# Dfam-consortium/RepeatAfterMe

Measured on AMD Instinct MI355X. Metric: flank_bp_aligned_per_sec (extension columns/s x flanks), higher is better.
Workload: dtype int32

## Files before the change

include/ramx.h:

```cpp
#ifndef RAMX_H
#define RAMX_H

#include <stdint.h>
#include <stdio.h>

#ifdef __cplusplus
extern "C" {
#endif

#ifndef RAMX_USE_REFERENCE_STRUCTS
enum CoreBoundFlag { L_BOUNDARY = 0, SEQ_BOUNDARY = 1, CORE_BOUNDARY = 2, EXT_BOUNDARY = 3 };

struct coreAlignment
{
  struct coreAlignment *next;
  int seqIdx;
  uint64_t leftSeqPos;
  uint64_t rightSeqPos;
  char leftExtendable;
  char rightExtendable;
  uint64_t lowerSeqBound;
  uint64_t upperSeqBound;
  enum CoreBoundFlag lowerSeqBoundFlag;
  enum CoreBoundFlag upperSeqBoundFlag;
  int leftExtensionLen;
  int rightExtensionLen;
  int score;
  char orient;
};

struct sequenceLibrary
{
  char *sequence;
  char **identifiers;
  uint64_t *boundaries;
  uint64_t *offsets;
  uint64_t length;
  int count;
  int markov_chain_order;
  uint32_t **markov_chain_prob_tables;
};

struct scoringSystem
{
  char *name;
  int **matrix;
  int msize;
  char *alphabet;
  double m_lambda;
  double m_bg_freqs[4];
  int gapopen;
  int gapextn;
};
#endif

#define RAMX_SYM_N 99


void ramx_set_runtime(int verbose, int when_to_stop, int l);

int ramx_extend_alignment(int direction, struct coreAlignment *coreAlign, int ****score,
                          struct sequenceLibrary *seqLib, char *master, int BANDWIDTH,
                          int CAPPENALTY, int MINIMPROVEMENT, int L, int N,
                          struct scoringSystem *scoreParams, FILE *pathStringFile);

typedef struct ramx_flat_cores
{
  int32_t n;
  const int64_t *left_pos, *right_pos, *lower, *upper;
  const int8_t *orient, *left_ext, *right_ext;
  int32_t *left_len, *right_len, *score;
} ramx_flat_cores;

typedef struct ramx_params
{
  int32_t bandwidth, cappenalty, minimprovement, L, when_to_stop, l, gapopen, gapextn;
  const int32_t *matrix;
} ramx_params;

typedef struct ramx_run_info
{
  int32_t ret;
  int32_t rows_executed;
  int32_t limit_warning;
  int32_t overflow32;
  int32_t n_extendable;
  int32_t launches;
  double  loop_ms;
  double  kernel_ms_avg;
  int32_t kernel_samples;
  double  prep_ms;
  int32_t persistent;
  int32_t lanes_per_flank;
  int32_t respeculated_rows;
  int32_t packed_rows;
  int32_t lean_rows;
} ramx_run_info;

int ramx_extend_flat(int direction, ramx_flat_cores *cores, const int8_t *sequence, uint64_t seq_len,
                     int8_t *master, const ramx_params *p, ramx_run_info *info);

void ramx_invalidate_library(void);
int ramx_preload_library(const int8_t *sequence, uint64_t seq_len);
struct ramx_packed_library;
int ramx_preload_library_packed(const struct sequenceLibrary *seqLib, const struct ramx_packed_library *pl);

typedef struct ramx_dev ramx_dev;

#define RAMX_OK            0
#define RAMX_ERR_NO_DEVICE (-101)
#define RAMX_ERR_HIP       (-102)
#define RAMX_ERR_ARG       (-103)
#define RAMX_ERR_STATE     (-104)
#define RAMX_ERR_COMM      (-105)
#define RAMX_ERR_UNSUPPORTED (-106)

const char *ramx_last_error(void);
int ramx_device_count(void);
int ramx_dev_create(int device_ordinal, ramx_dev **out);
void ramx_dev_destroy(ramx_dev *d);

int ramx_dev_load_library(ramx_dev *d, const int8_t *sequence, uint64_t length);
struct ramx_packed_library;
int ramx_dev_load_library_packed(ramx_dev *d, const struct ramx_packed_library *pl);

typedef struct ramx_flank
{
  int64_t start;
  int32_t t_lo, t_hi;
  int8_t  step;
  int8_t  compl_;
  int8_t  pad_[6];
} ramx_flank;

int ramx_resolve_flanks(int direction, const ramx_flat_cores *cores, int bandwidth, int L,
                        ramx_flank *flanks, int32_t *core_index);

int ramx_dev_begin_direction(ramx_dev *d, const ramx_flank *flanks, int32_t n_flanks, const ramx_params *p);

int ramx_dev_run_direction(ramx_dev *d, ramx_run_info *info);

int ramx_dev_download(ramx_dev *d, int8_t *cons, int32_t cons_cap, int32_t *trim_high, int32_t *trim_pos);

int ramx_dev_peek_state(ramx_dev *d, int32_t flank, int32_t *cells, int32_t *high, int32_t *pos);

int ramx_dev_peek_family_state(ramx_dev *d, int32_t flank, int32_t *cells);

typedef void (*ramx_row_trace_cb)(int32_t row, int32_t besta, const int8_t *codes ,
                                  const int32_t *best_score, const int32_t *best_idx, void *user);
int ramx_dev_set_row_trace(ramx_dev *d, ramx_row_trace_cb cb, void *user);

int ramx_dev_run_families(ramx_dev *d, const ramx_flank *flanks, int32_t n_padded, const int32_t *fam_first,
                          const int32_t *fam_count, int32_t n_families, const ramx_params *p,
                          ramx_run_info *infos, int8_t *cons, int32_t *trim_high, int32_t *trim_pos);

typedef struct ramx_family
{
  ramx_flat_cores cores;
  const int8_t *sequence;
  uint64_t seq_len;
  int8_t *master;
} ramx_family;
int ramx_extend_batch(int direction, ramx_family *families, int32_t n_families, const ramx_params *p, ramx_run_info *infos);

int ramx_comm_unique_id(uint8_t id[128]);
int ramx_dev_comm_init(ramx_dev *d, const uint8_t id[128], int rank, int nranks);
int ramx_dev_comm_size(ramx_dev *d);
int ramx_dev_peer_export(ramx_dev *d, uint8_t handle[64]);
int ramx_dev_peer_import(ramx_dev *d, const uint8_t *handles , int rank, int nranks);
int ramx_dev_peer_selftest(ramx_dev *d, int phase, unsigned long long token);
int ramx_dev_peer_enable(ramx_dev *d, int on);

int ramx_dev_hostbox_attach(ramx_dev *d, const char *shm_name, int rank, int nranks);
int ramx_hostbox_unlink(const char *shm_name);

typedef void (*ramx_allreduce_cb)(long long *vals4, void *user);
int ramx_dev_set_allreduce_cb(ramx_dev *d, ramx_allreduce_cb cb, void *user);

struct scoringSystem *ramx_get_matrix(const char *matrixName);
struct scoringSystem *ramx_get_matrix_using_gap_penalties(const char *matrixName,
                                                          int gapopen, int gapextn);
struct scoringSystem *ramx_get_repeatscout_matrix(int match, int mismatch, int gap);
void ramx_free_scoring_system(struct scoringSystem *s);
double ramx_calculate_lambda(struct scoringSystem *s);

struct sequenceLibrary *ramx_load_sequence_subset_minimal(const char *twoBitName, const char *rangeBEDName,
                                                          struct coreAlignment **core_align,
                                                          int *num_cores, int max_flanking_bp);
void ramx_free_library(struct sequenceLibrary *lib, struct coreAlignment *cores);

typedef struct ramx_packed_library
{
  uint64_t length;
  int32_t n_windows;
  const uint64_t *win_start;
  const uint64_t *win_byte;
  const uint8_t *win_phase;
  const uint8_t *bytes;
  uint64_t n_bytes;
  const uint64_t *n_start;
  const uint32_t *n_len;
  int32_t n_blocks;
} ramx_packed_library;

struct sequenceLibrary *ramx_load_sequence_subset_packed(const char *twoBitName, const char *rangeBEDName,
                                                         struct coreAlignment **core_align, int *num_cores,
                                                         int max_flanking_bp, const ramx_packed_library **packed);
int ramx_packed_decode(const ramx_packed_library *pl, uint64_t from, uint64_t count, char *out);

void ramx_overlap_avoidance(struct coreAlignment *coreAlign, struct sequenceLibrary *seqLib);

void ramx_print_core_edges(struct coreAlignment *coreAlign, struct sequenceLibrary *seqLib,
                           char omitBlanks, char debug);

int ****ramx_allocate_score(int num_align, int bandwidth);
void ramx_free_score(int num_align, int bandwidth, int ****score);

int ramx_cli_main(int argc, char **argv);

#ifdef __cplusplus
}
#endif
#endif
```

repeatafterme_amd/_lib.py:

```python
from __future__ import annotations

import ctypes as C
import os
import subprocess

_PKG = os.path.dirname(os.path.abspath(__file__))
LIB_PATH = os.environ.get("RAMX_LIB") or os.path.join(_PKG, "libramx.so")
CLI_PATH = os.path.join(_PKG, "RAMExtend")

EXPORTS = [
    "ramx_set_runtime", "ramx_extend_alignment", "ramx_extend_flat", "ramx_invalidate_library", "ramx_preload_library", "ramx_resolve_flanks", "ramx_last_error", "ramx_device_count",
    "ramx_dev_create", "ramx_dev_destroy", "ramx_dev_load_library", "ramx_dev_begin_direction",
    "ramx_dev_run_direction", "ramx_dev_download", "ramx_dev_peek_state", "ramx_dev_peek_family_state", "ramx_dev_set_row_trace", "ramx_dev_run_families", "ramx_extend_batch", "ramx_comm_unique_id",
    "ramx_dev_comm_init", "ramx_dev_comm_size", "ramx_dev_set_allreduce_cb", "ramx_dev_peer_export", "ramx_dev_peer_import",
    "ramx_dev_peer_selftest", "ramx_dev_peer_enable", "ramx_dev_hostbox_attach", "ramx_hostbox_unlink", "ramx_get_matrix", "ramx_get_matrix_using_gap_penalties",
    "ramx_get_repeatscout_matrix", "ramx_free_scoring_system", "ramx_calculate_lambda",
    "ramx_load_sequence_subset_minimal", "ramx_load_sequence_subset_packed", "ramx_packed_decode", "ramx_dev_load_library_packed", "ramx_preload_library_packed", "ramx_free_library", "ramx_overlap_avoidance",
    "ramx_print_core_edges", "ramx_allocate_score", "ramx_free_score", "ramx_cli_main",
]


class RamxError(RuntimeError):
    pass


class FlatCores(C.Structure):
    _fields_ = [("n", C.c_int32)] + [(k, C.c_void_p) for k in
                ("left_pos", "right_pos", "lower", "upper", "orient", "left_ext", "right_ext",
                 "left_len", "right_len", "score")]


class Params(C.Structure):
    _fields_ = [(k, C.c_int32) for k in ("bandwidth", "cappenalty", "minimprovement", "L", "when_to_stop",
                                          "l", "gapopen", "gapextn")] + [("matrix", C.c_void_p)]


class RunInfo(C.Structure):
    _fields_ = [("ret", C.c_int32), ("rows_executed", C.c_int32), ("limit_warning", C.c_int32),
                ("overflow32", C.c_int32), ("n_extendable", C.c_int32), ("launches", C.c_int32),
                ("loop_ms", C.c_double), ("kernel_ms_avg", C.c_double), ("kernel_samples", C.c_int32),
                ("prep_ms", C.c_double), ("persistent", C.c_int32), ("lanes_per_flank", C.c_int32),
                ("respeculated_rows", C.c_int32), ("packed_rows", C.c_int32), ("lean_rows", C.c_int32)]


class Family(C.Structure):
    _fields_ = [("cores", FlatCores), ("sequence", C.c_void_p), ("seq_len", C.c_uint64), ("master", C.c_void_p)]


class Flank(C.Structure):
    _fields_ = [("start", C.c_int64), ("t_lo", C.c_int32), ("t_hi", C.c_int32), ("step", C.c_int8),
                ("compl_", C.c_int8), ("pad_", C.c_int8 * 6)]


ALLREDUCE_CB = C.CFUNCTYPE(None, C.POINTER(C.c_longlong), C.c_void_p)


def build(force: bool = False) -> None:
    if force or not os.path.exists(LIB_PATH) or not os.path.exists(CLI_PATH):
        subprocess.check_call(["make", "-s", "-C", os.path.join(_PKG, "csrc"), "all"])


_lib = None


def lib() -> C.CDLL:
    global _lib
    if _lib is None:
        if not os.path.exists(LIB_PATH):
            raise RamxError(f"{LIB_PATH} is missing: build it with `make -C repeatafterme_amd/csrc` "
                            "(there is no CPU fallback)")
        L = C.CDLL(LIB_PATH)
        L.ramx_last_error.restype = C.c_char_p
        L.ramx_set_runtime.argtypes = [C.c_int, C.c_int, C.c_int]
        L.ramx_set_runtime.restype = None
        L.ramx_extend_flat.argtypes = [C.c_int, C.POINTER(FlatCores), C.c_void_p, C.c_uint64, C.c_void_p,
                                       C.POINTER(Params), C.POINTER(RunInfo)]
        L.ramx_extend_flat.restype = C.c_int
        L.ramx_resolve_flanks.argtypes = [C.c_int, C.POINTER(FlatCores), C.c_int, C.c_int, C.c_void_p, C.c_void_p]
        L.ramx_resolve_flanks.restype = C.c_int
        L.ramx_extend_batch.argtypes = [C.c_int, C.POINTER(Family), C.c_int32, C.POINTER(Params), C.POINTER(RunInfo)]
        L.ramx_extend_batch.restype = C.c_int
        L.ramx_device_count.restype = C.c_int
        L.ramx_dev_create.argtypes = [C.c_int, C.POINTER(C.c_void_p)]
        L.ramx_dev_destroy.argtypes = [C.c_void_p]
        L.ramx_dev_destroy.restype = None
        L.ramx_dev_load_library.argtypes = [C.c_void_p, C.c_void_p, C.c_uint64]
        L.ramx_dev_begin_direction.argtypes = [C.c_void_p, C.c_void_p, C.c_int32, C.POINTER(Params)]
        L.ramx_dev_run_direction.argtypes = [C.c_void_p, C.POINTER(RunInfo)]
        L.ramx_dev_download.argtypes = [C.c_void_p, C.c_void_p, C.c_int32, C.c_void_p, C.c_void_p]
        L.ramx_dev_peek_state.argtypes = [C.c_void_p, C.c_int32, C.c_void_p, C.POINTER(C.c_int32),
                                          C.POINTER(C.c_int32)]
        L.ramx_dev_peek_family_state.argtypes = [C.c_void_p, C.c_int32, C.c_void_p]
        L.ramx_comm_unique_id.argtypes = [C.c_void_p]
        L.ramx_dev_comm_init.argtypes = [C.c_void_p, C.c_void_p, C.c_int, C.c_int]
        L.ramx_dev_comm_size.argtypes = [C.c_void_p]
        L.ramx_dev_set_allreduce_cb.argtypes = [C.c_void_p, ALLREDUCE_CB, C.c_void_p]
        L.ramx_dev_peer_export.argtypes = [C.c_void_p, C.c_void_p]
        L.ramx_dev_peer_import.argtypes = [C.c_void_p, C.c_void_p, C.c_int, C.c_int]
        L.ramx_dev_peer_selftest.argtypes = [C.c_void_p, C.c_int, C.c_uint64]
        L.ramx_dev_peer_enable.argtypes = [C.c_void_p, C.c_int]
        L.ramx_dev_hostbox_attach.argtypes = [C.c_void_p, C.c_char_p, C.c_int, C.c_int]
        L.ramx_hostbox_unlink.argtypes = [C.c_char_p]
        if hasattr(L, "ramx_cli_main"):
            L.ramx_cli_main.argtypes = [C.c_int, C.POINTER(C.c_char_p)]
        _lib = L
    return _lib


def check(rc: int, what: str) -> int:
    if rc < 0:
        raise RamxError(f"{what} failed ({rc}): {lib().ramx_last_error().decode()}")
    return rc
```

repeatafterme_amd/csrc/ramx_device.hip:

```cpp

#include <rccl/rccl.h>
#include <errno.h>
#include <fcntl.h>
#include <sys/mman.h>
#include <unistd.h>
#include <stdarg.h>
#include <stdio.h>
#include <stdlib.h>
#include <string.h>
#include <time.h>
#include <vector>


#include "ramx_kernels_common.h"
#include "ramx_kernels_stream.h"
#include "ramx_kernels_resident.h"
#include "ramx_cp_api.h"
#include "ramx_pk_api.h"

static thread_local char g_err[512];

extern "C" void ramx_set_error(const char *fmt, ...)
{
  va_list ap;
  va_start(ap, fmt);
  vsnprintf(g_err, sizeof(g_err), fmt, ap);
  va_end(ap);
}
extern "C" const char *ramx_last_error(void) { return g_err; }

#define HIPCHK(call)                                                                              \
  do {                                                                                            \
    hipError_t e_ = (call);                                                                       \
    if (e_ != hipSuccess) {                                                                       \
      ramx_set_error("HIP error %s at %s:%d (%s)", hipGetErrorString(e_), __FILE__, __LINE__, #call); \
      return RAMX_ERR_HIP;                                                                        \
    }                                                                                             \
  } while (0)

static double now_ms(void);
static void rt_mark(const char *what)
{
  static double last = 0;
  static int on = -1;
  if (on < 0) on = getenv("RAMX_TIMING") != NULL;
  if (!on) return;
  const double t = now_ms();
  if (what) fprintf(stderr, "RAMX_TIMING       run: %-44s %8.3f ms\n", what, t - last);
  last = t;
}
static double now_ms(void)
{
  struct timespec ts;
  clock_gettime(CLOCK_MONOTONIC, &ts);
  return ts.tv_sec * 1e3 + ts.tv_nsec * 1e-6;
}

#define RAMX_NGROUP (RAMX_CP_NCLASS + 4)

struct ramx_dev
{
  int ordinal;
  hipStream_t stream;
  signed char *d_lib; unsigned long long lib_len; unsigned long long lib_cap;
  int lib_packed;
  unsigned char *d_pk_bytes, *d_pk_phase; unsigned long long *d_pk_wstart, *d_pk_wbyte, *d_pk_nstart; unsigned *d_pk_nlen;
  size_t cap_pk_bytes, cap_pk_phase, cap_pk_wstart, cap_pk_wbyte, cap_pk_nstart, cap_pk_nlen, cap_flank_win;
  int pk_windows, pk_nblocks; int *d_flank_win;
  ramx_flank *d_flanks; unsigned *d_bases; int2 *d_bounds; int4 *d_state[2]; int2 *d_trim;
  long long *d_sums; RamxCtl *d_ctl; signed char *d_cons;
  PShard *d_vote; unsigned *d_err;
  int last_persistent;
  size_t cap_flanks, cap_bases, cap_state, cap_cons, cap_bounds, cap_trim, cap_fam, cap_famctl;
  void *d_fam; RamxCtl *d_famctl;
  RamxCtl *h_ctl;
  void *h_stage; size_t cap_stage;
  hipEvent_t ev_chk[2], ev_begin, ev_end, ev_s0[MAX_SAMPLES], ev_s1[MAX_SAMPLES];
  int Nx, Np, KW;
  ramx_params p; int tab[RAMX_NCLASS][4];
  int ready;
  RamxCtl final_ctl;
  ncclComm_t comm; int rank, nranks;
  ramx_allreduce_cb cb; void *cb_user;
  PeerBox *xbox; PeerBox *peer[RAMX_MAX_RANKS]; PeerBox **d_peer; int peer_ready;
  void *peer_ipc[RAMX_MAX_RANKS];
  void *hostbox_map; size_t hostbox_bytes; PeerBox *hostbox_host; int hostbox_registered;
  PeerBox *hostbox_mirror;
  PeerBox *devbox;
  hipStream_t cls_stream[RAMX_NGROUP]; hipEvent_t cls_ready, cls_done[RAMX_NGROUP]; int cls_init;
  int force_chain;
  ramx_row_trace_cb trace_cb; void *trace_user;
  ramx_row_verbose_cb verbose_cb; void *verbose_user;
  signed char *d_dbg_codes; int2 *d_dbg_best; size_t cap_dbg_codes, cap_dbg_best;
  int *d_dbg_cand; int2 *d_dbg_gap; size_t cap_dbg_cand, cap_dbg_gap;
  int *d_dbg_band; size_t cap_dbg_band; int verbose_band;
  CpDevDesc *d_devdesc; size_t cap_devdesc;
  PShard *d_vote_sets; size_t cap_vote_sets; unsigned *d_err_sets; size_t cap_err_sets;
  int packed_kw;
  hipStream_t pack_stream; hipEvent_t pack_done; int pack_busy;
  int pk_r0;
  int last_packed_r0;
  int cp_flanks_ok;
  int2 *d_cpstate; size_t cap_cpstate; int cpstate_W, cpstate_n;
};

extern "C" int ramx_device_count(void)
{
  int n = 0;
  hipError_t e = hipGetDeviceCount(&n);
  if (e != hipSuccess) { ramx_set_error("hipGetDeviceCount: %s", hipGetErrorString(e)); return RAMX_ERR_NO_DEVICE; }
  return n;
}

extern "C" int ramx_dev_create(int ordinal, ramx_dev **out)
{
  int n = ramx_device_count();
  if (n <= 0) { ramx_set_error("no HIP device visible (libramx has no CPU path)"); return RAMX_ERR_NO_DEVICE; }
  if (ordinal < 0 || ordinal >= n) { ramx_set_error("device ordinal %d out of range (%d devices)", ordinal, n); return RAMX_ERR_ARG; }
  HIPCHK(hipSetDevice(ordinal));
  hipDeviceProp_t prop;
  HIPCHK(hipGetDeviceProperties(&prop, ordinal));
  if (strncmp(prop.gcnArchName, "gfx950", 6) != 0)
  {
    ramx_set_error("device %d is %s; libramx carries gfx950 code objects only", ordinal, prop.gcnArchName);
    return RAMX_ERR_NO_DEVICE;
  }
  ramx_dev *d = (ramx_dev *)calloc(1, sizeof(ramx_dev));
  d->ordinal = ordinal;
#define CRCHK(call) do { hipError_t e_ = (call); if (e_ != hipSuccess) { \
    ramx_set_error("HIP error %s at %s:%d (%s)", hipGetErrorString(e_), __FILE__, __LINE__, #call); ramx_dev_destroy(d); return RAMX_ERR_HIP; } } while (0)
  CRCHK(hipStreamCreateWithFlags(&d->stream, hipStreamNonBlocking));
  CRCHK(hipStreamCreateWithFlags(&d->pack_stream, hipStreamNonBlocking));
  CRCHK(hipEventCreateWithFlags(&d->pack_done, hipEventDisableTiming));
  CRCHK(hipHostMalloc((void **)&d->h_ctl, 4 * sizeof(RamxCtl), hipHostMallocDefault));
  CRCHK(hipHostMalloc(&d->h_stage, (size_t)2 << 20, hipHostMallocDefault));
  d->cap_stage = (size_t)2 << 20;
  CRCHK(hipMalloc((void **)&d->d_sums, (3 * NSHARD * 4 + 8) * sizeof(long long)));
  CRCHK(hipMalloc((void **)&d->d_ctl, 2 * sizeof(RamxCtl)));
  CRCHK(hipMalloc((void **)&d->d_vote, PRK_NSETS * NSHARD * sizeof(PShard)));
  CRCHK(hipMalloc((void **)&d->d_err, 64));

  for (int i = 0; i < 2; i++) CRCHK(hipEventCreate(&d->ev_chk[i]));
  CRCHK(hipEventCreate(&d->ev_begin));
  CRCHK(hipEventCreate(&d->ev_end));
  for (int i = 0; i < MAX_SAMPLES; i++) { CRCHK(hipEventCreate(&d->ev_s0[i])); CRCHK(hipEventCreate(&d->ev_s1[i])); }
#undef CRCHK
  const char *eb = getenv("RAMX_FORCE_CHAIN");
  d->force_chain = (eb && atoi(eb) != 0) ? 1 : 0;
  *out = d;
  return RAMX_OK;
}

extern "C" void ramx_dev_destroy(ramx_dev *d)
{
  if (!d) return;
  (void)hipSetDevice(d->ordinal);
  if (d->stream) (void)hipStreamSynchronize(d->stream);
  if (d->pack_stream) { (void)hipStreamSynchronize(d->pack_stream); (void)hipStreamDestroy(d->pack_stream); }
  if (d->pack_done) (void)hipEventDestroy(d->pack_done);
  if (d->comm) (void)ncclCommDestroy(d->comm);
  for (int q = 0; q < RAMX_MAX_RANKS; q++)
    if (d->peer_ipc[q]) { (void)hipIpcCloseMemHandle(d->peer_ipc[q]); d->peer_ipc[q] = NULL; }
  (void)hipFree(d->d_pk_bytes); (void)hipFree(d->d_pk_phase); (void)hipFree(d->d_pk_wstart); (void)hipFree(d->d_pk_wbyte);
  (void)hipFree(d->d_pk_nstart); (void)hipFree(d->d_pk_nlen); (void)hipFree(d->d_flank_win);
  (void)hipFree(d->d_lib); (void)hipFree(d->d_flanks); (void)hipFree(d->d_bases); (void)hipFree(d->d_bounds);
  (void)hipFree(d->d_state[0]); if (d->d_state[1] != d->d_state[0]) (void)hipFree(d->d_state[1]); (void)hipFree(d->d_trim); (void)hipFree(d->d_sums);
  (void)hipFree(d->d_ctl); (void)hipFree(d->d_cons); (void)hipFree(d->d_vote); (void)hipFree(d->d_err);
  if (d->h_ctl) (void)hipHostFree(d->h_ctl);
  if (d->h_stage) (void)hipHostFree(d->h_stage);
  if (d->hostbox_map)
  {
    if (d->hostbox_registered) (void)hipHostUnregister(d->hostbox_map);
    munmap(d->hostbox_map, d->hostbox_bytes);
  }
  if (d->cls_init)
  {
    for (int c = 0; c < RAMX_NGROUP; c++) { (void)hipStreamDestroy(d->cls_stream[c]); (void)hipEventDestroy(d->cls_done[c]); }
    (void)hipEventDestroy(d->cls_ready);
  }
  if (d->devbox) (void)hipFree(d->devbox);
  (void)hipFree(d->d_fam); (void)hipFree(d->d_famctl); (void)hipFree(d->d_cpstate); (void)hipFree(d->d_dbg_codes); (void)hipFree(d->d_dbg_best); (void)hipFree(d->d_dbg_cand); (void)hipFree(d->d_dbg_gap); (void)hipFree(d->d_dbg_band); (void)hipFree(d->d_devdesc); (void)hipFree(d->d_vote_sets); (void)hipFree(d->d_err_sets);
  if (d->hostbox_mirror) (void)hipFree(d->hostbox_mirror);
  if (d->d_peer) (void)hipFree(d->d_peer);
  for (int i = 0; i < 2; i++) if (d->ev_chk[i]) (void)hipEventDestroy(d->ev_chk[i]);
  if (d->ev_begin) (void)hipEventDestroy(d->ev_begin);
  if (d->ev_end) (void)hipEventDestroy(d->ev_end);
  for (int i = 0; i < MAX_SAMPLES; i++) { if (d->ev_s0[i]) (void)hipEventDestroy(d->ev_s0[i]); if (d->ev_s1[i]) (void)hipEventDestroy(d->ev_s1[i]); }
  if (d->stream) (void)hipStreamDestroy(d->stream);
  free(d);
}

extern "C" int ramx_dev_load_library(ramx_dev *d, const int8_t *sequence, uint64_t length)
{
  if (!d || (!sequence && length)) { ramx_set_error("ramx_dev_load_library: bad argument"); return RAMX_ERR_ARG; }
  HIPCHK(hipSetDevice(d->ordinal));
  if (length > d->lib_cap)
  {
    if (d->d_lib) HIPCHK(hipFree(d->d_lib));
    d->d_lib = NULL;
    HIPCHK(hipMalloc((void **)&d->d_lib, length ? length : 1));
    d->lib_cap = length;
  }
  if (length) HIPCHK(hipMemcpyAsync(d->d_lib, sequence, length, hipMemcpyHostToDevice, d->stream));
  HIPCHK(hipStreamSynchronize(d->stream));
  d->lib_len = length;
  d->lib_packed = 0;
  return RAMX_OK;
}

template <typename T>
static int ensure(T **p, size_t *cap, size_t need_bytes);

extern "C" int ramx_dev_load_library_packed(ramx_dev *d, const struct ramx_packed_library *pl)
{
  if (!d || !pl || pl->n_windows < 0 || (pl->n_windows && (!pl->win_start || !pl->win_byte || !pl->win_phase || !pl->bytes)) ||
      pl->n_blocks < 0 || (pl->n_blocks && (!pl->n_start || !pl->n_len)))
  { ramx_set_error("ramx_dev_load_library_packed: bad argument"); return RAMX_ERR_ARG; }
  HIPCHK(hipSetDevice(d->ordinal));
  const size_t nw = (size_t)pl->n_windows, nb = (size_t)pl->n_blocks;
  int rc;
  if ((rc = ensure(&d->d_pk_bytes, &d->cap_pk_bytes, (size_t)pl->n_bytes + 16))) return rc;
  if ((rc = ensure(&d->d_pk_wstart, &d->cap_pk_wstart, (nw + 1) * sizeof(unsigned long long)))) return rc;
  if ((rc = ensure(&d->d_pk_wbyte, &d->cap_pk_wbyte, (nw + 1) * sizeof(unsigned long long)))) return rc;
  if ((rc = ensure(&d->d_pk_phase, &d->cap_pk_phase, nw + 1))) return rc;
  if ((rc = ensure(&d->d_pk_nstart, &d->cap_pk_nstart, (nb + 1) * sizeof(unsigned long long)))) return rc;
  if ((rc = ensure(&d->d_pk_nlen, &d->cap_pk_nlen, (nb + 1) * sizeof(unsigned)))) return rc;
  if (pl->n_bytes) HIPCHK(hipMemcpyAsync(d->d_pk_bytes, pl->bytes, (size_t)pl->n_bytes, hipMemcpyHostToDevice, d->stream));
  if (nw)
  {
    HIPCHK(hipMemcpyAsync(d->d_pk_wstart, pl->win_start, (nw + 1) * sizeof(unsigned long long), hipMemcpyHostToDevice, d->stream));
    HIPCHK(hipMemcpyAsync(d->d_pk_wbyte, pl->win_byte, (nw + 1) * sizeof(unsigned long long), hipMemcpyHostToDevice, d->stream));
    HIPCHK(hipMemcpyAsync(d->d_pk_phase, pl->win_phase, nw, hipMemcpyHostToDevice, d->stream));
  }
  if (nb)
  {
    HIPCHK(hipMemcpyAsync(d->d_pk_nstart, pl->n_start, nb * sizeof(unsigned long long), hipMemcpyHostToDevice, d->stream));
    HIPCHK(hipMemcpyAsync(d->d_pk_nlen, pl->n_len, nb * sizeof(unsigned), hipMemcpyHostToDevice, d->stream));
  }
  HIPCHK(hipStreamSynchronize(d->stream));
  d->lib_len = pl->length; d->pk_windows = pl->n_windows; d->pk_nblocks = pl->n_blocks;
  d->lib_packed = 1;
  return RAMX_OK;
}

static int launch_pack(ramx_dev *d, int Nx, int Np, int W, int k_lo, int k_hi, hipStream_t st)
{
  if (k_hi <= k_lo) return RAMX_OK;
  if (!d->lib_packed)
  {
    dim3 grid((Np + 255) / 256, k_hi - k_lo);
    hipLaunchKernelGGL(ramx_pack_kernel, grid, dim3(256), 0, st, d->d_lib, (unsigned long long)d->lib_len,
                       d->d_flanks, Nx, Np, W, k_lo, d->d_bases, d->d_bounds);
    HIPCHK(hipGetLastError());
    return RAMX_OK;
  }
  PkLib L;
  L.bytes = d->d_pk_bytes; L.win_start = d->d_pk_wstart; L.win_byte = d->d_pk_wbyte; L.win_phase = d->d_pk_phase;
  L.n_start = d->d_pk_nstart; L.n_len = d->d_pk_nlen; L.length = d->lib_len; L.n_windows = d->pk_windows; L.n_blocks = d->pk_nblocks;
  if (k_lo == 0)
  {
    int rc;
    if ((rc = ensure(&d->d_flank_win, &d->cap_flank_win, (size_t)Np * sizeof(int)))) return rc;
    if (Nx > 0)
    {
      hipLaunchKernelGGL(ramx_flank_window_kernel, dim3((Nx + 255) / 256), dim3(256), 0, st, L, d->d_flanks, Nx, d->d_flank_win);
      HIPCHK(hipGetLastError());
    }
  }
  hipLaunchKernelGGL(ramx_pack2_kernel, dim3((Np + 255) / 256, (k_hi - k_lo + RAMX_PK_WORDS - 1) / RAMX_PK_WORDS), dim3(256), 0, st, L, d->d_flanks,
                     d->d_flank_win, Nx, Np, W, k_lo, k_hi, d->d_bases, d->d_bounds);
  HIPCHK(hipGetLastError());
  return RAMX_OK;
}

static int pack_rest(ramx_dev *d)
{
  if (d->packed_kw >= d->KW) return RAMX_OK;
  if (d->pack_busy) { HIPCHK(hipStreamWaitEvent(d->stream, d->pack_done, 0)); d->pack_busy = 0; }
  const int rc = launch_pack(d, d->Nx, d->Np, d->p.bandwidth, d->packed_kw, d->KW, d->stream);
  d->packed_kw = d->KW;
  return rc;
}
static int pk_segment_columns(int L, int when_to_stop)
{
  const char *e = getenv("RAMX_PK_SEGMENT");
  const int v = e ? atoi(e) : (when_to_stop >= L ? 0 : 2048);
  return v < 0 ? 0 : v;
}

template <typename T>
static int ensure(T **p, size_t *cap, size_t need_bytes)
{
  if (need_bytes <= *cap && *p) return RAMX_OK;
  if (*p) HIPCHK(hipFree(*p));
  *p = NULL;
  HIPCHK(hipMalloc((void **)p, need_bytes ? need_bytes : 16));
  *cap = need_bytes;
  return RAMX_OK;
}

extern "C" int ramx_dev_begin_direction(ramx_dev *d, const ramx_flank *flanks, int32_t n_flanks, const ramx_params *p)
{
  if (!d || !p || n_flanks < 0 || (n_flanks && !flanks)) { ramx_set_error("ramx_dev_begin_direction: bad argument"); return RAMX_ERR_ARG; }
  if (p->bandwidth < 0 || p->L < 0) { ramx_set_error("bandwidth and L must be >= 0"); return RAMX_ERR_ARG; }
  if (!p->matrix) { ramx_set_error("scoring matrix missing"); return RAMX_ERR_ARG; }
  HIPCHK(hipSetDevice(d->ordinal));
  rt_mark(NULL);
  const int W = p->bandwidth, Q = W + 1;
  const int Nx = n_flanks;
  const int Np = ((Nx + 63) / 64) * 64 > 0 ? ((Nx + 63) / 64) * 64 : 64;
  const int KW = (p->L + 2 * W + 2) / 8 + 12;
  d->Nx = Nx; d->Np = Np; d->KW = KW; d->p = *p;
  for (int c = 0; c < RAMX_NCLASS; c++)
  {
    const int code = (c == 8) ? RAMX_SYM_N : c;
    for (int k = 0; k < 4; k++) d->tab[c][k] = p->matrix[k * 100 + code];
  }
  int rc;
  if ((rc = ensure(&d->d_flanks, &d->cap_flanks, (size_t)Np * sizeof(ramx_flank)))) return rc;
  if ((rc = ensure(&d->d_bases, &d->cap_bases, (size_t)KW * Np * sizeof(unsigned)))) return rc;
  if ((rc = ensure(&d->d_bounds, &d->cap_bounds, (size_t)Np * sizeof(int2)))) return rc;
  if ((rc = ensure(&d->d_trim, &d->cap_trim, (size_t)Np * sizeof(int2)))) return rc;
  const size_t state_bytes = (size_t)Np * Q * sizeof(int4);
  if (state_bytes > d->cap_state || !d->d_state[0])
  {
    const bool pingpong = getenv("RAMX_PINGPONG") != NULL;
    if (d->d_state[0]) HIPCHK(hipFree(d->d_state[0]));
    if (d->d_state[1] && d->d_state[1] != d->d_state[0]) HIPCHK(hipFree(d->d_state[1]));
    d->d_state[0] = d->d_state[1] = NULL;
    HIPCHK(hipMalloc((void **)&d->d_state[0], state_bytes));
    if (pingpong) HIPCHK(hipMalloc((void **)&d->d_state[1], state_bytes));
    else d->d_state[1] = d->d_state[0];
    d->cap_state = state_bytes;
  }
  if ((rc = ensure(&d->d_cons, &d->cap_cons, (size_t)p->L + 16))) return rc;
  rt_mark("begin: buffers");
  if (Nx) HIPCHK(hipMemcpyAsync(d->d_flanks, flanks, (size_t)Nx * sizeof(ramx_flank), hipMemcpyHostToDevice, d->stream));
  rt_mark("begin: flanks to the device (enqueued)");
  {
    if (d->pack_busy) { HIPCHK(hipStreamWaitEvent(d->stream, d->pack_done, 0)); d->pack_busy = 0; }
    const int seg = pk_segment_columns(p->L, p->when_to_stop);
    const int first = seg > 0 ? ((seg + 8) >> 3) + 28 : KW;
    d->packed_kw = first < KW ? first : KW;
    if ((rc = launch_pack(d, Nx, Np, W, 0, d->packed_kw, d->stream)) != RAMX_OK) return rc;
  }
  HIPCHK(hipMemsetAsync(d->d_sums, 0, 3 * NSHARD * 4 * sizeof(long long), d->stream));
  HIPCHK(hipMemsetAsync(d->d_cons, 0, (size_t)p->L + 16, d->stream));
  rt_mark("begin: pack of the first piece enqueued");
  HIPCHK(hipStreamSynchronize(d->stream));
  rt_mark("begin: synchronised");
  d->cp_flanks_ok = 1;
  for (int i = 0; i < Nx; i++)
    if (flanks[i].t_lo > 0 && flanks[i].t_lo <= flanks[i].t_hi) { d->cp_flanks_ok = 0; break; }
  d->pk_r0 = d->cp_flanks_ok ? 0 : -1;
  if (d->cp_flanks_ok)
    for (int i = 0; i < Nx; i++)
      if (flanks[i].t_lo <= flanks[i].t_hi && flanks[i].t_lo + W > d->pk_r0) d->pk_r0 = flanks[i].t_lo + W;
  d->ready = 1;
  return RAMX_OK;
}

template <bool INIT>
static void launch_column(ramx_dev *d, const KArgs &a)
{
  const int tiles = d->Np / 64;
  const dim3 grid((tiles + 3) / 4), block(256);
  if (a.go <= 0 && a.ge <= 0 && !d->force_chain)
    hipLaunchKernelGGL((ramx_column_kernel<INIT, false, 256>), grid, block, 0, d->stream, a);
  else
    hipLaunchKernelGGL((ramx_column_kernel<INIT, true, 256>), grid, block, 0, d->stream, a);
}

static void launch_column_trace(ramx_dev *d, const KArgs &a, bool init = false)
{
  const int tiles = d->Np / 64;
  const dim3 grid((tiles + 3) / 4), block(256);
  if (init) { hipLaunchKernelGGL((ramx_column_kernel<true, true, 256, true>), grid, block, 0, d->stream, a); return; }
  if (a.dbg_cand != NULL) { hipLaunchKernelGGL((ramx_column_kernel<false, true, 256, true>), grid, block, 0, d->stream, a); return; }
  if (a.go <= 0 && a.ge <= 0 && !d->force_chain)
    hipLaunchKernelGGL((ramx_column_kernel<false, false, 256, true>), grid, block, 0, d->stream, a);
  else
    hipLaunchKernelGGL((ramx_column_kernel<false, true, 256, true>), grid, block, 0, d->stream, a);
}

static bool dev_is_multi(const ramx_dev *d)
{
  return (d->comm != NULL && (d->nranks > 1 || getenv("RAMX_FORCE_COLLECTIVE") != NULL)) || d->cb != NULL;
}

static int host_allreduce_shards(ramx_dev *d, long long *dptr)
{
  if (d->cb)
  {
    long long h[NSHARD * 4], h4[4] = { 0, 0, 0, 0 };
    HIPCHK(hipMemcpyAsync(h, dptr, sizeof(h), hipMemcpyDeviceToHost, d->stream));
    HIPCHK(hipStreamSynchronize(d->stream));
    for (int i = 0; i < NSHARD * 4; i++) h4[i & 3] += h[i];
    d->cb(h4, d->cb_user);
    memset(h, 0, sizeof(h));
    memcpy(h, h4, sizeof(h4));
    HIPCHK(hipMemcpyAsync(dptr, h, sizeof(h), hipMemcpyHostToDevice, d->stream));
    HIPCHK(hipStreamSynchronize(d->stream));
    return RAMX_OK;
  }
  ncclResult_t nr = ncclAllReduce(dptr, dptr, NSHARD * 4, ncclInt64, ncclSum, d->comm, d->stream);
  if (nr != ncclSuccess) { ramx_set_error("ncclAllReduce: %s", ncclGetErrorString(nr)); return RAMX_ERR_COMM; }
  return RAMX_OK;
}

static int host_allreduce_flag(ramx_dev *d, int *flag)
{
  if (d->cb)
  {
    long long h4[4] = { *flag ? 1 : 0, 0, 0, 0 };
    d->cb(h4, d->cb_user);
    *flag = h4[0] != 0;
    return RAMX_OK;
  }
  long long *tmp = d->d_sums + 3 * NSHARD * 4;
  long long h = *flag ? 1 : 0;
  HIPCHK(hipMemcpyAsync(tmp, &h, sizeof(h), hipMemcpyHostToDevice, d->stream));
  ncclResult_t nr = ncclAllReduce(tmp, tmp, 1, ncclInt64, ncclMax, d->comm, d->stream);
  if (nr != ncclSuccess) { ramx_set_error("ncclAllReduce: %s", ncclGetErrorString(nr)); return RAMX_ERR_COMM; }
  HIPCHK(hipMemcpyAsync(&h, tmp, sizeof(h), hipMemcpyDeviceToHost, d->stream));
  HIPCHK(hipStreamSynchronize(d->stream));
  *flag = h != 0;
  return RAMX_OK;
}

extern "C" int ramx_dev_peer_export(ramx_dev *d, uint8_t handle[64])
{
  if (!d || !handle) { ramx_set_error("ramx_dev_peer_export: bad argument"); return RAMX_ERR_ARG; }
  HIPCHK(hipSetDevice(d->ordinal));
  if (!d->devbox)
  {
    hipError_t e = hipExtMallocWithFlags((void **)&d->devbox, sizeof(PeerBox), hipDeviceMallocFinegrained);
    if (e != hipSuccess) { d->devbox = NULL; ramx_set_error("fine-grained allocation for the peer box failed: %s", hipGetErrorString(e)); return RAMX_ERR_HIP; }
    HIPCHK(hipMemset(d->devbox, 0, sizeof(PeerBox)));
  }
  hipIpcMemHandle_t h;
  HIPCHK(hipIpcGetMemHandle(&h, d->devbox));
  static_assert(sizeof(hipIpcMemHandle_t) <= 64, "ipc handle size");
  memset(handle, 0, 64);
  memcpy(handle, &h, sizeof(h));
  return RAMX_OK;
}

__global__ void ramx_peer_token_kernel(PeerBox *const *peers, int rank, int nranks, unsigned long long token)
{
  if (threadIdx.x < nranks)
    __hip_atomic_store(&peers[threadIdx.x]->token[rank], token, __ATOMIC_RELAXED, __HIP_MEMORY_SCOPE_SYSTEM);
}

extern "C" int ramx_dev_peer_import(ramx_dev *d, const uint8_t *handles, int rank, int nranks)
{
  if (!d || !handles || rank < 0 || rank >= nranks || nranks > RAMX_MAX_RANKS || !d->devbox)
  { ramx_set_error("ramx_dev_peer_import: bad argument (export first; at most %d ranks)", RAMX_MAX_RANKS); return RAMX_ERR_ARG; }
  HIPCHK(hipSetDevice(d->ordinal));
  d->peer_ready = 0;
  d->rank = rank; d->nranks = nranks;
  d->xbox = d->devbox; d->hostbox_host = NULL;
  for (int q = 0; q < RAMX_MAX_RANKS; q++)
    if (d->peer_ipc[q]) { (void)hipIpcCloseMemHandle(d->peer_ipc[q]); d->peer_ipc[q] = NULL; }
  for (int q = 0; q < nranks; q++)
  {
    if (q == rank) { d->peer[q] = d->xbox; continue; }
    hipIpcMemHandle_t h;
    memcpy(&h, handles + 64 * q, sizeof(h));
    void *ptr = NULL;
    hipError_t e = hipIpcOpenMemHandle(&ptr, h, hipIpcMemLazyEnablePeerAccess);
    if (e != hipSuccess) { ramx_set_error("hipIpcOpenMemHandle(rank %d): %s", q, hipGetErrorString(e)); return RAMX_ERR_HIP; }
    d->peer[q] = (PeerBox *)ptr;
    d->peer_ipc[q] = ptr;
  }
  if (!d->d_peer) HIPCHK(hipMalloc((void **)&d->d_peer, RAMX_MAX_RANKS * sizeof(PeerBox *)));
  HIPCHK(hipMemcpy(d->d_peer, d->peer, nranks * sizeof(PeerBox *), hipMemcpyHostToDevice));
  return RAMX_OK;
}

extern "C" int ramx_dev_hostbox_attach(ramx_dev *d, const char *shm_name, int rank, int nranks)
{
  if (!d || !shm_name || rank < 0 || rank >= nranks || nranks > RAMX_MAX_RANKS)
  { ramx_set_error("ramx_dev_hostbox_attach: bad argument (at most %d ranks)", RAMX_MAX_RANKS); return RAMX_ERR_ARG; }
  HIPCHK(hipSetDevice(d->ordinal));
  d->peer_ready = 0;
  const size_t bytes = (((size_t)nranks * sizeof(PeerBox)) + 4095) & ~(size_t)4095;
  int fd = rank == 0 ? shm_open(shm_name, O_CREAT | O_EXCL | O_RDWR, 0600) : shm_open(shm_name, O_RDWR, 0600);
  if (fd < 0) { ramx_set_error("shm_open(%s): %s", shm_name, strerror(errno)); return RAMX_ERR_COMM; }
  if (rank == 0 && ftruncate(fd, (off_t)bytes) != 0) { ramx_set_error("ftruncate(%s): %s", shm_name, strerror(errno)); close(fd); shm_unlink(shm_name); return RAMX_ERR_COMM; }
  void *map = mmap(NULL, bytes, PROT_READ | PROT_WRITE, MAP_SHARED, fd, 0);
  close(fd);
  if (map == MAP_FAILED) { ramx_set_error("mmap(%s): %s", shm_name, strerror(errno)); return RAMX_ERR_COMM; }
  hipError_t e = hipHostRegister(map, bytes, hipHostRegisterMapped | hipHostRegisterPortable);
  if (e != hipSuccess) { munmap(map, bytes); ramx_set_error("hipHostRegister(shared boxes): %s", hipGetErrorString(e)); return RAMX_ERR_HIP; }
  void *dptr = NULL;
  e = hipHostGetDevicePointer(&dptr, map, 0);
  if (e != hipSuccess) { (void)hipHostUnregister(map); munmap(map, bytes); ramx_set_error("hipHostGetDevicePointer: %s", hipGetErrorString(e)); return RAMX_ERR_HIP; }
  if (d->hostbox_map) { if (d->hostbox_registered) (void)hipHostUnregister(d->hostbox_map); munmap(d->hostbox_map, d->hostbox_bytes); }
  d->hostbox_map = map; d->hostbox_bytes = bytes; d->hostbox_registered = 1;
  d->hostbox_host = (PeerBox *)map + rank;
  memset(d->hostbox_host, 0, sizeof(PeerBox));
  d->rank = rank; d->nranks = nranks;
  d->xbox = (PeerBox *)dptr + rank;
  for (int q = 0; q < nranks; q++) d->peer[q] = (PeerBox *)dptr + q;
  if (!d->d_peer) HIPCHK(hipMalloc((void **)&d->d_peer, RAMX_MAX_RANKS * sizeof(PeerBox *)));
  HIPCHK(hipMemcpy(d->d_peer, d->peer, nranks * sizeof(PeerBox *), hipMemcpyHostToDevice));
  return RAMX_OK;
}

extern "C" int ramx_hostbox_unlink(const char *shm_name)
{
  if (!shm_name) return RAMX_ERR_ARG;
  return shm_unlink(shm_name) == 0 ? RAMX_OK : RAMX_ERR_COMM;
}

extern "C" int ramx_dev_peer_selftest(ramx_dev *d, int phase, unsigned long long token)
{
  if (!d || !d->d_peer) { ramx_set_error("ramx_dev_peer_selftest: import first"); return RAMX_ERR_ARG; }
  HIPCHK(hipSetDevice(d->ordinal));
  if (phase == 0)
  {
    hipLaunchKernelGGL(ramx_peer_token_kernel, dim3(1), dim3(64), 0, d->stream, (PeerBox *const *)d->d_peer, d->rank, d->nranks, token);
    HIPCHK(hipGetLastError());
    HIPCHK(hipStreamSynchronize(d->stream));
    return RAMX_OK;
  }
  PeerBox h;
  for (int tries = 0; tries < 200; tries++)
  {
    if (d->hostbox_host) memcpy(&h, (const void *)d->hostbox_host, sizeof(h));
    else HIPCHK(hipMemcpy(&h, d->xbox, sizeof(h), hipMemcpyDeviceToHost));
    int ok = 1;
    for (int q = 0; q < d->nranks; q++) ok &= (h.token[q] == token);
    if (ok) return 1;
    struct timespec ts = { 0, 1000000 };
    nanosleep(&ts, NULL);
  }
  return 0;
}

extern "C" int ramx_dev_peer_enable(ramx_dev *d, int on)
{
  if (!d) return RAMX_ERR_ARG;
  d->peer_ready = (on && d->d_peer && d->xbox) ? 1 : 0;
  return RAMX_OK;
}

static int fast_pack_ok(const int (&tab)[RAMX_NCLASS][4], int go, int ge, int L, int W)
{
  long long mx = (long long)(go < 0 ? -go : go) + (long long)(ge < 0 ? -ge : ge);
  for (int c = 0; c < RAMX_NCLASS; c++)
    for (int k = 0; k < 4; k++)
    {
      const long long v = tab[c][k] < 0 ? -(long long)tab[c][k] : (long long)tab[c][k];
      if (v > mx) mx = v;
    }
  for (int c = 0; c < RAMX_NCLASS; c++)
    for (int k = 0; k < 4; k++)
      if (tab[c][k] < -128 || tab[c][k] > 127) return 0;
  return ((long long)L + 2LL * W + 4) * mx < (1LL << 27) ? 1 : 0;
}

static int lean_p_of(const int (&tab)[RAMX_NCLASS][4], int go, int ge)
{
  if (getenv("RAMX_NO_LEAN") != NULL || go > 0 || ge > 0) return -1;
  int mx = 0;
  for (int c = 0; c < RAMX_NCLASS; c++)
    for (int k = 0; k < 4; k++) if (tab[c][k] > mx) mx = tab[c][k];
  return mx;
}

template <int W, int BLOCK>
static int prk_capacity_blocks(int *out)
{
  static int cached = -1;
  if (cached >= 0) { *out = cached; return RAMX_OK; }
  int per_cu = 0, dev = 0, cus = 0;
  HIPCHK(hipGetDevice(&dev));
  HIPCHK(hipDeviceGetAttribute(&cus, hipDeviceAttributeMultiprocessorCount, dev));
  HIPCHK(hipOccupancyMaxActiveBlocksPerMultiprocessor(&per_cu, ramx_persistent_kernel<W, BLOCK>, BLOCK, 0));
  if (per_cu > 1) per_cu = 1;
  *out = per_cu * cus;
  cached = *out;
  return RAMX_OK;
}

static void test_delay_rank(const ramx_dev *d)
{
  const char *e = getenv("RAMX_TEST_DELAY_RANK");
  int r = -1, ms = 0;
  if (e && sscanf(e, "%d:%d", &r, &ms) == 2 && r == d->rank && ms > 0) usleep((useconds_t)ms * 1000);
}

template <int W, int BLOCK>
static int prk_launch(ramx_dev *d, PArgs &pa, int blocks)
{
  if (pa.nranks > 1) test_delay_rank(d);
  if (getenv("RAMX_COOP_LAUNCH") != NULL)
  {
    void *args[] = { (void *)&pa };
    HIPCHK(hipLaunchCooperativeKernel((const void *)ramx_persistent_kernel<W, BLOCK>, dim3(blocks), dim3(BLOCK), args, 0, d->stream));
    return RAMX_OK;
  }
  hipLaunchKernelGGL((ramx_persistent_kernel<W, BLOCK>), dim3(blocks), dim3(BLOCK), 0, d->stream, pa);
  HIPCHK(hipGetLastError());
  return RAMX_OK;
}

template <int W>
static int prk_plan(int tiles, int *block, int *blocks)
{
  int cap = 0, rc;
  *block = 0; *blocks = 0;
  if ((rc = prk_capacity_blocks<W, 256>(&cap)) != RAMX_OK) return rc;
  if ((tiles + 3) / 4 <= cap)
  {
    *block = 256; *blocks = (tiles + 3) / 4;
    return RAMX_OK;
  }
  if constexpr (W <= 40)
  {
    if ((rc = prk_capacity_blocks<W, 512>(&cap)) != RAMX_OK) return rc;
    if ((tiles + 7) / 8 <= cap) { *block = 512; *blocks = (tiles + 7) / 8; }
  }
  return RAMX_OK;
}

static bool prk_has_width(int W) { return W == 14 || W == 20 || W == 40 || W == 80; }
static bool fam_has_width(int W) { return W == 14 || W == 20 || W == 40; }

static int d2h_small(ramx_dev *d, void *dst, const void *src, size_t bytes)
{
  const size_t off = d->cap_stage - ((size_t)64 << 10);
  if (bytes == 0) return RAMX_OK;
  if (bytes > ((size_t)64 << 10) || d->h_stage == NULL || d->cap_stage < ((size_t)128 << 10) || getenv("RAMX_DOWNLOAD_DMA") != NULL)
  {
    HIPCHK(hipStreamSynchronize(d->stream));
    HIPCHK(hipMemcpy(dst, src, bytes, hipMemcpyDeviceToHost));
    return RAMX_OK;
  }
  int2 *stage = (int2 *)((char *)d->h_stage + off);
  const int n = (int)((bytes + 7) / 8);
  hipLaunchKernelGGL(ramx_to_host_kernel, dim3((n + 255) / 256), dim3(256), 0, d->stream, (const int2 *)src, stage, n);
  HIPCHK(hipGetLastError());
  HIPCHK(hipStreamSynchronize(d->stream));
  memcpy(dst, stage, bytes);
  return RAMX_OK;
}

#define RAMX_CP_MIN_K_OVER_PACKED 4
static int prk_local_can(ramx_dev *d, const KArgs &a, int L, bool multi, bool *can_out, int *block, int *blocks)
{
  const int W = a.W;
  const int tiles = d->Np / 64;
  int rc;
  *block = 0; *blocks = 0;
  bool can = !(getenv("RAMX_NO_PERSISTENT") != NULL || d->force_chain || a.go > 0 || a.ge > 0 || a.go + a.ge < -32768 ||
               !prk_has_width(W) || L <= 0);
  if (multi && (!d->peer_ready || d->nranks < 2 || L >= 65536 || getenv("RAMX_NO_PEER") != NULL)) can = false;
  if (can)
  {
    rc = (W == 14) ? prk_plan<14>(tiles, block, blocks) : (W == 20) ? prk_plan<20>(tiles, block, blocks) :
         (W == 40) ? prk_plan<40>(tiles, block, blocks) : prk_plan<80>(tiles, block, blocks);
    if (rc != RAMX_OK) return rc;
    if (*block == 0) can = false;
  }
  *can_out = can;
  return RAMX_OK;
}

static int pk_route(ramx_dev *d, const KArgs &a, int L, bool multi, bool int32_can, bool *pk_out, int *spread, int *rebase, int *pk_block, int *pk_blocks)
{
  *pk_out = false; *pk_block = 0; *pk_blocks = 0;
  const int pk_r0 = (getenv("RAMX_NO_PERSISTENT") != NULL || d->force_chain || L <= 0) ? -1 : d->pk_r0;
  bool pk = pk_r0 >= 0 && pk_r0 < L && ramx_pk_plan(a.W, a.go, a.ge, a.tab, spread, rebase) != 0;
  if (multi && (!d->peer_ready || d->nranks < 2 || L >= 65536 || getenv("RAMX_NO_PEER") != NULL || getenv("RAMX_NO_PK_MULTI") != NULL)) pk = false;
  if (pk)
  {
    if (ramx_pk_shape(a.W, d->Np / 64, pk_block, pk_blocks) != RAMX_OK) { ramx_set_error("packed-row kernel: occupancy query failed"); return RAMX_ERR_HIP; }
    if (*pk_block == 0 || (pk_r0 > 0 && !int32_can)) pk = false;
  }
  *pk_out = pk;
  return RAMX_OK;
}

static int prk_run(ramx_dev *d, const KArgs &a, int L, bool *used)
{
  *used = false;
  const int W = a.W;
  const bool multi = dev_is_multi(d);
  int block = 0, blocks = 0, rc;
  bool can = false;
  if ((rc = prk_local_can(d, a, L, multi, &can, &block, &blocks)) != RAMX_OK) return rc;
  if (multi)
  {
    int cannot = can ? 0 : 1;
    if ((rc = host_allreduce_flag(d, &cannot)) != RAMX_OK) return rc;
    can = !cannot;
  }
  const bool int32_can = can;
  const int pk_r0 = (getenv("RAMX_NO_PERSISTENT") != NULL || d->force_chain || L <= 0) ? -1 : d->pk_r0;
  if (!can && (multi || pk_r0 < 0)) return RAMX_OK;
  *used = true;
  PArgs pa;
  memset(&pa, 0, sizeof(pa));
  pa.S = d->d_state[0]; pa.bases = d->d_bases; pa.bounds = d->d_bounds; pa.trim = d->d_trim;
  pa.sums0 = d->d_sums; pa.vote = d->d_vote; pa.ctl_out = d->d_ctl; pa.cons_out = d->d_cons; pa.err = d->d_err;
  pa.Np = d->Np; pa.Nx = d->Nx; pa.r0 = 0; pa.L = L; pa.go = a.go; pa.ge = a.ge; pa.cap = a.cap; pa.minimp = a.minimp;
  pa.when_to_stop = a.when_to_stop; pa.nblocks = blocks;
  pa.nranks = 1; pa.rank = 0; pa.peers = NULL; pa.box = NULL;
  if (multi)
  {
    pa.nranks = d->nranks; pa.rank = d->rank; pa.peers = (PeerBox *const *)d->d_peer; pa.box = d->xbox;
    pa.mirror = NULL;
    auto local_prep = [&]() -> int
    {
      if (d->hostbox_host)
      {
        if (!d->hostbox_mirror) HIPCHK(hipMalloc((void **)&d->hostbox_mirror, sizeof(PeerBox)));
        HIPCHK(hipMemsetAsync(d->hostbox_mirror, 0, sizeof(PeerBox), d->stream));
        pa.mirror = d->hostbox_mirror;
      }
      if (d->hostbox_host)
      {
        HIPCHK(hipStreamSynchronize(d->stream));
        memset((void *)d->hostbox_host, 0, sizeof(PeerBox));
        __sync_synchronize();
      }
      else
      {
        HIPCHK(hipMemsetAsync(d->xbox, 0, sizeof(PeerBox), d->stream));
        HIPCHK(hipStreamSynchronize(d->stream));
      }
      return RAMX_OK;
    };
    const int lrc = local_prep();
    if ((rc = host_allreduce_shards(d, d->d_sums)) != RAMX_OK) return rc;
    if (lrc != RAMX_OK) return lrc;
    const char *tf = getenv("RAMX_TEST_FAIL_PRK_RANK");
    if (tf && atoi(tf) == d->rank) { ramx_set_error("test hook: forced failure of the persistent launch on rank %d", d->rank); return RAMX_ERR_HIP; }
  }
  memcpy(pa.tab, a.tab, sizeof(pa.tab));
  pa.pack_ok = getenv("RAMX_NO_FASTPACK") ? 0 : fast_pack_ok(pa.tab, a.go, a.ge, L, W);
  if (pa.pack_ok && getenv("RAMX_NO_MASKHI") == NULL) pa.pack_ok = 2;
  pa.lean_p = lean_p_of(pa.tab, a.go, a.ge);
  { const char *lm = getenv("RAMX_LEADER_MAX"); pa.leader_max = lm ? atoi(lm) : 3; if (pa.leader_max < 0) pa.leader_max = 0; if (pa.leader_max > 64) pa.leader_max = 64; }
  PKArgs ka;
  memset(&ka, 0, sizeof(ka));
  int pk_block = 0, pk_blocks = 0;
  bool pk = false;
  if ((rc = pk_route(d, a, L, multi, int32_can, &pk, &ka.spread, &ka.rebase, &pk_block, &pk_blocks)) != RAMX_OK) return rc;
  if (!pk && !int32_can) { *used = false; return RAMX_OK; }
  if (!pk && (rc = pack_rest(d)) != RAMX_OK) return rc;
  HIPCHK(hipMemsetAsync(d->d_vote, 0, PRK_NSETS * NSHARD * sizeof(PShard), d->stream));
  HIPCHK(hipMemsetAsync(d->d_err, 0, 64, d->stream));
  long long *sums_next = d->d_sums + (size_t)NSHARD * 4;
  const bool head = !pk || pk_r0 > 0;
  if (pk && pk_r0 > 0) { pa.L = pk_r0; pa.sums_next = sums_next; }
#ifdef RAMX_PRK_TIMING
  const size_t nw = pk ? (size_t)pk_blocks * (pk_block / 64) : (size_t)blocks * (block / 64);
  unsigned long long *dbgbuf = NULL;
  HIPCHK(hipMalloc((void **)&dbgbuf, nw * 8 * sizeof(unsigned long long)));
  HIPCHK(hipMemset(dbgbuf, 0, nw * 8 * sizeof(unsigned long long)));
  if (pk) ka.dbg = dbgbuf; else pa.dbg = dbgbuf;
#endif
  rc = RAMX_OK;
  const bool tmarks = getenv("RAMX_TIMING") != NULL;
  const double tm0 = now_ms();
  rt_mark("persistent route, memsets");
  if (head)
  {
    if (block == 256)
      rc = (W == 14) ? prk_launch<14, 256>(d, pa, blocks) : (W == 20) ? prk_launch<20, 256>(d, pa, blocks) :
           (W == 40) ? prk_launch<40, 256>(d, pa, blocks) : prk_launch<80, 256>(d, pa, blocks);
    else
      rc = (W == 14) ? prk_launch<14, 512>(d, pa, blocks) : (W == 20) ? prk_launch<20, 512>(d, pa, blocks) : prk_launch<40, 512>(d, pa, blocks);
  }
  rt_mark("first rows launched (int32 kernel)");
  if (rc == RAMX_OK && pk)
  {
    ka.S = d->d_state[0]; ka.bases = d->d_bases; ka.bounds = d->d_bounds; ka.trim = d->d_trim;
    ka.vote = d->d_vote; ka.cons_out = d->d_cons; ka.err = d->d_err;
    ka.peers = pa.peers; ka.box = pa.box; ka.mirror = pa.mirror; ka.rank = pa.rank; ka.nranks = pa.nranks;
    ka.xblock = 0;
    if (ka.nranks > 1 && getenv("RAMX_NO_PK_EXCHANGER") == NULL)
    {
      int cap = 0;
      if (ramx_pk_capacity(W, pk_block, &cap) == RAMX_OK && pk_blocks + 1 <= cap) ka.xblock = pk_blocks;
    }
    ka.Np = d->Np; ka.Nx = d->Nx; ka.L = L; ka.go = a.go; ka.ge = a.ge; ka.cap = a.cap; ka.minimp = a.minimp;
    ka.when_to_stop = a.when_to_stop; ka.nblocks = pk_blocks;
    memcpy(ka.tab, a.tab, sizeof(ka.tab));
    ka.lean_p = pa.lean_p; ka.leader_max = pa.leader_max;
    ka.spec_on = getenv("RAMX_NO_PK_SPEC") == NULL ? 1 : 0;
    { const char *we = getenv("RAMX_TEST_PK_WRONG_EVERY"); ka.test_wrong_every = we ? atoi(we) : 0; }
    { const char *ts = getenv("RAMX_TEST_PK_SPREAD"); if (ts) ka.spread = atoi(ts); }
    ka.spread_rows = ka.spread;
    { const char *ts = getenv("RAMX_TEST_PK_SPREAD_ROWS"); if (ts) ka.spread_rows = atoi(ts); }
    d->last_packed_r0 = pk_r0;
    const int seg = pk_segment_columns(L, a.when_to_stop);
    const int NWw = (2 * W + 1 + 8) / 8 + 2;
    long long *sbuf[2] = { d->d_sums + (size_t)NSHARD * 4, d->d_sums + (size_t)2 * NSHARD * 4 };
    const long long *sums_in = pk_r0 > 0 ? sbuf[0] : d->d_sums;
    int nextbuf = pk_r0 > 0 ? 1 : 0;
    int ctl_i = 0;
    auto words_for = [&](int r_end) { int wn = ((r_end + 7) >> 3) + NWw + 2; return wn < d->KW ? wn : d->KW; };
    if (ka.nranks > 1 && !head) test_delay_rank(d);
    for (int r = pk_r0, s_i = 0; r < L && rc == RAMX_OK; s_i++)
    {
      const int r1 = seg > 0 ? std::min(L, (r / seg + 1) * seg) : L;
      if (d->pack_busy) { HIPCHK(hipStreamWaitEvent(d->stream, d->pack_done, 0)); d->pack_busy = 0; }
      if (d->packed_kw < words_for(r1))
      {
        if ((rc = launch_pack(d, d->Nx, d->Np, W, d->packed_kw, words_for(r1), d->stream)) != RAMX_OK) break;
        d->packed_kw = words_for(r1);
      }
      HIPCHK(hipMemsetAsync(d->d_vote, 0, PRK_NSETS * NSHARD * sizeof(PShard), d->stream));
      ka.r0 = r; ka.Lseg = r1; ka.sums_in = sums_in;
      ka.sums_next = r1 < L ? sbuf[nextbuf] : NULL;
      if (r1 < L) HIPCHK(hipMemsetAsync(sbuf[nextbuf], 0, (size_t)NSHARD * 4 * sizeof(long long), d->stream));
      ka.ctl_in = d->d_ctl + ctl_i; ka.ctl_out = d->d_ctl + (ctl_i ^ 1);
      if (r == 0) ka.ctl_out = d->d_ctl;
      const double tm1 = now_ms();
      rc = ramx_pk_launch(d->stream, W, pk_block, pk_blocks, ka);
      if (rc != RAMX_OK) { ramx_set_error("packed-row kernel: launch failed (W %d, %d workgroups of %d threads)", W, pk_blocks, pk_block); break; }
      if (tmarks) fprintf(stderr, "RAMX_TIMING       run: piece %d (rows %d..%d, %d x %d threads) launched %.3f ms after the first launch (launch call %.3f ms)\n", s_i, r, r1, pk_blocks, pk_block, now_ms() - tm0, now_ms() - tm1);
      const int out_i = (r == 0) ? 0 : (ctl_i ^ 1);
      if (r1 >= L) break;
      const int r2 = std::min(L, (r1 / seg + 1) * seg);
      if (d->packed_kw < words_for(r2))
      {
        if ((rc = launch_pack(d, d->Nx, d->Np, W, d->packed_kw, words_for(r2), d->pack_stream)) != RAMX_OK) break;
        HIPCHK(hipEventRecord(d->pack_done, d->pack_stream));
        d->pack_busy = 1;
        d->packed_kw = words_for(r2);
      }
      RamxCtl hc;
      unsigned errw = 0;
      HIPCHK(hipStreamSynchronize(d->stream));
      if (tmarks) fprintf(stderr, "RAMX_TIMING       run: piece %d complete %.3f ms after the first launch\n", s_i, now_ms() - tm0);
      {
        unsigned long long ew = 0;
        if ((rc = d2h_small(d, &hc, d->d_ctl + out_i, sizeof(hc))) != RAMX_OK) break;
        if ((rc = d2h_small(d, &ew, d->d_err, sizeof(ew))) != RAMX_OK) break;
        errw = (unsigned)ew;
      }
      rt_mark("piece: control block and error word read");
      if (hc.stopped || hc.pad != 0 || errw != 0 || hc.rows_done < r1) break;
      sums_in = sbuf[nextbuf]; nextbuf ^= 1; ctl_i = out_i; r = r1;
    }
    if (pk) { block = pk_block; blocks = pk_blocks; }
  }
  else d->last_packed_r0 = -1;
#ifdef RAMX_PRK_TIMING
  if (rc == RAMX_OK)
  {
    HIPCHK(hipStreamSynchronize(d->stream));
    unsigned long long *h = (unsigned long long *)malloc(nw * 8 * sizeof(unsigned long long));
    HIPCHK(hipMemcpy(h, dbgbuf, nw * 8 * sizeof(unsigned long long), hipMemcpyDeviceToHost));
    static const char *nm[6] = { "wait vote", "block barrier 1", "band", pk ? "early arrival" : "reduce+barrier 2", pk ? "late arrival" : "issue atomics", "loop top" };
    const int wpb = block / 64;
    fprintf(stderr, "PRK_TIMING %s blocks %d x %d threads, L %d, first row %d (ns per column)\n", pk ? "packed rows" : "int32 rows", blocks, block, L, pk ? pk_r0 : 0);
    for (int k = 0; k < 6; k++)
    {
      double s0 = 0, sO = 0, mx = 0, mn = 1e30;
      for (size_t i = 0; i < nw; i++)
      {
        const double v = 10.0 * (double)h[i * 8 + k] / L;
        if ((int)(i % wpb) == 0) s0 += v; else sO += v;
        if (v > mx) mx = v;
        if (v < mn) mn = v;
      }
      fprintf(stderr, "PRK_TIMING %-18s wave0 avg %8.1f  other waves avg %8.1f  min %8.1f  max %8.1f\n", nm[k], s0 / blocks,
              wpb > 1 ? sO / (double)(nw - blocks) : 0.0, mn, mx);
    }
    fprintf(stderr, "PRK_TIMING band by wave index:");
    for (int wv = 0; wv < wpb; wv++)
    {
      double sw = 0;
      for (int b = 0; b < blocks - 1; b++) sw += 10.0 * (double)h[((size_t)b * wpb + wv) * 8 + 2] / L;
      fprintf(stderr, " w%d %.0f", wv, sw / (blocks > 1 ? blocks - 1 : 1));
    }
    fprintf(stderr, "\n");
    {
      int gb = 0;
      for (int b = 1; b < blocks; b++) if (h[(size_t)b * wpb * 8 + 0] < h[(size_t)gb * wpb * 8 + 0]) gb = b;
      fprintf(stderr, "PRK_TIMING workgroup %d (shortest vote wait), per wave: wait vote | barrier | band | early | late | top\n", gb);
      for (int wv = 0; wv < wpb; wv++)
      {
        const unsigned long long *q = h + ((size_t)gb * wpb + wv) * 8;
        fprintf(stderr, "PRK_TIMING   w%d %7.0f %7.0f %7.0f %7.0f %7.0f %7.0f   rows full %llu lean %llu\n", wv, 10.0 * q[0] / L, 10.0 * q[1] / L, 10.0 * q[2] / L,
                10.0 * q[3] / L, 10.0 * q[4] / L, 10.0 * q[5] / L, q[6], q[7]);
      }
    }
    {
      const double half = L - L / 2;
      size_t never = 0, always = 0, wg_any = 0;
      double lanes = 0, cols = 0;
      int hist[6] = { 0, 0, 0, 0, 0, 0 };
      for (int b = 0; b < blocks; b++)
      {
        bool any = false;
        for (int wv = 0; wv < wpb; wv++)
        {
          const size_t i = (size_t)b * wpb + wv;
          const double c = (double)h[i * 8 + 6], l = (double)h[i * 8 + 7];
          if (c == 0) { never++; continue; }
          any = any || c > 0.5 * half;
          if (c > 0.9 * half) always++;
          lanes += l; cols += c;
          const double avg = l / c;
          hist[avg <= 1 ? 0 : avg <= 2 ? 1 : avg <= 4 ? 2 : avg <= 8 ? 3 : avg <= 16 ? 4 : 5]++;
        }
        if (any) wg_any++;
      }
      fprintf(stderr, "PRK_LEANSTAT second half (%.0f columns): %zu of %zu waves always LEAN, %zu non-LEAN in > 90 %% of the columns; workgroups with a wave "
              "non-LEAN in > 50 %%: %zu of %d; lanes per non-LEAN wave-column %.2f; waves by that average <=1: %d <=2: %d <=4: %d <=8: %d <=16: %d more: %d\n",
              half, never, nw, always, wg_any, blocks, cols > 0 ? lanes / cols : 0.0, hist[0], hist[1], hist[2], hist[3], hist[4], hist[5]);
    }
    free(h);
    (void)hipFree(dbgbuf);
  }
#endif
  return rc;
}

static void cp_test_hooks(CPArgs &ca)
{
  const char *we = getenv("RAMX_TEST_CP_WRONG_EVERY"), *vd = getenv("RAMX_TEST_CP_VOTE_DELAY");
  ca.test_wrong_every = we ? atoi(we) : 0;
  ca.test_vote_delay = vd ? atoi(vd) : 0;
  ca.lean_p = lean_p_of(ca.tab, ca.go, ca.ge);
}

template <int W, int BLOCK>
static int fam_launch(ramx_dev *d, const FArgs &fa, int F, hipStream_t st)
{
  (void)d;
  hipLaunchKernelGGL((ramx_family_kernel<W, BLOCK>), dim3(F), dim3(BLOCK), 0, st, fa);
  HIPCHK(hipGetLastError());
  return RAMX_OK;
}

static int run_families_pass(ramx_dev *d, const ramx_flank *flanks, int32_t n_padded, const int32_t *fam_first,
                             const int32_t *fam_count, int32_t n_families, const ramx_params *p,
                             ramx_run_info *infos, int8_t *cons, int32_t *trim_high, int32_t *trim_pos,
                             bool allow_dev, unsigned char *timed_out)
{
  if (!d || !p || !p->matrix || n_families < 0 || n_padded < 0 || (n_padded & 63) || (n_families && (!fam_first || !fam_count || !flanks)))
  { ramx_set_error("ramx_dev_run_families: bad argument"); return RAMX_ERR_ARG; }
  HIPCHK(hipSetDevice(d->ordinal));
  const int W = p->bandwidth, L = p->L;
  if (W < 1 || L < 0) { ramx_set_error("ramx_dev_run_families: bad bandwidth / L"); return RAMX_ERR_ARG; }
  const bool resident = fam_has_width(W) && p->gapopen <= 0 && p->gapextn <= 0 && p->gapopen + p->gapextn >= -32768 &&
                        !d->force_chain && getenv("RAMX_NO_PERSISTENT") == NULL;
  int maxn = 0;
  for (int f = 0; f < n_families; f++)
  {
    if (fam_count[f] < 0 || fam_first[f] < 0 || (fam_first[f] & 63) || (long long)fam_first[f] + fam_count[f] > n_padded) { ramx_set_error("ramx_dev_run_families: bad family layout"); return RAMX_ERR_ARG; }
    if (fam_count[f] > maxn) maxn = fam_count[f];
  }
  if (maxn > 512) { ramx_set_error("batch mode: a family has more than 512 flanks"); return RAMX_ERR_UNSUPPORTED; }
  if (n_families == 0) return RAMX_OK;
  const int Np = n_padded > 0 ? n_padded : 64;
  const int KW = (L + 2 * W + 2) / 8 + 12;
  int rc;
  if ((rc = ensure(&d->d_flanks, &d->cap_flanks, (size_t)Np * sizeof(ramx_flank)))) return rc;
  if ((rc = ensure(&d->d_bases, &d->cap_bases, (size_t)KW * Np * sizeof(unsigned)))) return rc;
  if ((rc = ensure(&d->d_bounds, &d->cap_bounds, (size_t)Np * sizeof(int2)))) return rc;
  if ((rc = ensure(&d->d_trim, &d->cap_trim, (size_t)Np * sizeof(int2)))) return rc;
  if ((rc = ensure(&d->d_cons, &d->cap_cons, (size_t)n_families * (L > 0 ? L : 1) + 16))) return rc;
  int tab9[RAMX_NCLASS][4];
  for (int c = 0; c < RAMX_NCLASS; c++)
  {
    const int code = (c == 8) ? RAMX_SYM_N : c;
    for (int k = 0; k < 4; k++) tab9[c][k] = p->matrix[k * 100 + code];
  }
  const int cp_max = d->force_chain ? 0 : ramx_cp_max_family(W, p->gapopen, p->gapextn, tab9, L);
  FamDesc *hfd = (FamDesc *)malloc(sizeof(FamDesc) * n_families);
  int *grp = (int *)malloc(sizeof(int) * n_families);
  int cls_first[RAMX_NGROUP + 1], cls_count[RAMX_NGROUP], cp_k[RAMX_CP_NCLASS], cp_threads[RAMX_CP_NCLASS];
  memset(cls_count, 0, sizeof(cls_count));
  memset(cp_k, 0, sizeof(cp_k)); memset(cp_threads, 0, sizeof(cp_threads));
  auto cls_of = [](int nx) { return nx <= 64 ? 0 : nx <= 128 ? 1 : nx <= 256 ? 2 : 3; };
  int n_cp = 0, n_dev = 0, dev_k = 0, dev_threads = 0, dev_vw = 0, cus = 0;
  std::vector<CpDevDesc> hdev;
  std::vector<int> dev_round_first, dev_round_blocks;
  {
    int devo = 0;
    if (hipGetDevice(&devo) != hipSuccess || hipDeviceGetAttribute(&cus, hipDeviceAttributeMultiprocessorCount, devo) != hipSuccess) cus = 0;
  }
  const bool dev_route = allow_dev && cp_max > 0 && cus > 0 && getenv("RAMX_NO_CP_DEVICE") == NULL && getenv("RAMX_NO_PERSISTENT") == NULL;
  int dev_wide = 0;
  if (dev_route)
  {
    long long need = 0;
    for (int f = 0; f < n_families; f++)
    {
      if (fam_count[f] <= cp_max) continue;
      int k = 0, th = 0, nb = 0;
      int vwf = 0;
      ramx_cp_device_plan(W, fam_count[f], cus, 0, &k, &th, &nb, &vwf);
      need += k > 0 ? nb : 0;
    }
    dev_wide = need > cus;
  }
  for (int f = 0; f < n_families; f++)
  {
    int g = RAMX_CP_NCLASS + cls_of(fam_count[f]);
    if (fam_count[f] > 0 && cp_max > 0)
    {
      bool ok = true;
      for (int i = 0; i < fam_count[f] && ok; i++)
      {
        const ramx_flank &x = flanks[fam_first[f] + i];
        ok = (x.t_lo <= 0) || (x.t_lo > x.t_hi);
      }
      int k = 0, th = 0;
      const int c = (ok && fam_count[f] <= cp_max) ? ramx_cp_class(W, fam_count[f], &k, &th) : -1;
      if (c >= 0) { g = c; cp_k[c] = k; cp_threads[c] = th; n_cp++; }
      else if (ok && dev_route)
      {
        int nb = 0;
        int vwf = 0;
        ramx_cp_device_plan(W, fam_count[f], cus, dev_wide, &k, &th, &nb, &vwf);
        if (k > 0 && nb <= cus && (dev_k == 0 || (k == dev_k && th == dev_threads && vwf == dev_vw)))
        {
          dev_k = k; dev_threads = th; dev_vw = vwf;
          if (dev_round_first.empty() || dev_round_blocks.back() + nb > cus)
          {
            dev_round_first.push_back((int)hdev.size());
            dev_round_blocks.push_back(0);
          }
          dev_round_blocks.back() += nb;
          for (int b = 0; b < nb; b++)
          {
            CpDevDesc x;
            memset(&x, 0, sizeof(x));
            x.first = fam_first[f]; x.nx = fam_count[f]; x.b = b; x.nb = nb; x.id = f; x.vs = n_dev;
            hdev.push_back(x);
          }
          n_dev++;
          g = -1;
        }
      }
    }
    grp[f] = g;
    if (g >= 0) cls_count[g]++;
  }
  cls_first[0] = 0;
  for (int c = 0; c < RAMX_NGROUP; c++) cls_first[c + 1] = cls_first[c] + cls_count[c];
  {
    int fill[RAMX_NGROUP];
    for (int c = 0; c < RAMX_NGROUP; c++) fill[c] = cls_first[c];
    for (int f = 0; f < n_families; f++)
    {
      if (grp[f] < 0) continue;
      FamDesc &x = hfd[fill[grp[f]]++];
      x.tile0 = fam_first[f] / 64; x.ntiles = (fam_count[f] + 63) / 64; x.nx = fam_count[f]; x.id = f;
    }
  }
  RamxCtl *hctl = NULL;
  int2 *tmp = NULL;
  float ms = 0;
  unsigned long long *cp_dbg = NULL;
#define FAMCHK(call) do { hipError_t e_ = (call); if (e_ != hipSuccess) { \
    ramx_set_error("HIP error %s at %s:%d (%s)", hipGetErrorString(e_), __FILE__, __LINE__, #call); rc = RAMX_ERR_HIP; goto done; } } while (0)
  FamDesc *dfd; RamxCtl *dctl;
  FArgs fa;
  const bool legacy_any = n_cp + n_dev < n_families;
  if ((rc = ensure(&d->d_fam, &d->cap_fam, sizeof(FamDesc) * (size_t)n_families))) goto done;
  if ((rc = ensure(&d->d_famctl, &d->cap_famctl, sizeof(RamxCtl) * (size_t)n_families))) goto done;
  dfd = (FamDesc *)d->d_fam; dctl = d->d_famctl;
  FAMCHK(hipMemcpyAsync(dfd, hfd, sizeof(FamDesc) * n_families, hipMemcpyHostToDevice, d->stream));
  if (n_padded) FAMCHK(hipMemcpyAsync(d->d_flanks, flanks, (size_t)n_padded * sizeof(ramx_flank), hipMemcpyHostToDevice, d->stream));
  if ((rc = launch_pack(d, n_padded, Np, W, 0, KW, d->stream)) != RAMX_OK) goto done;
  d->packed_kw = KW;
  FAMCHK(hipMemsetAsync(d->d_cons, 0, (size_t)n_families * (L > 0 ? L : 1) + 16, d->stream));
  memset(&fa, 0, sizeof(fa));
  fa.bases = d->d_bases; fa.bounds = d->d_bounds; fa.fam = dfd; fa.trim = d->d_trim; fa.ctl_out = dctl; fa.cons_out = d->d_cons;
  fa.Np = Np; fa.L = L; fa.go = p->gapopen; fa.ge = p->gapextn; fa.cap = p->cappenalty; fa.minimp = p->minimprovement;
  fa.when_to_stop = p->when_to_stop;
  memcpy(fa.tab, tab9, sizeof(fa.tab));
  fa.pack_ok = getenv("RAMX_NO_FASTPACK") ? 0 : fast_pack_ok(fa.tab, fa.go, fa.ge, L, W);
  if (fa.pack_ok && getenv("RAMX_NO_MASKHI") == NULL) fa.pack_ok = 2;
  fa.lean_p = lean_p_of(fa.tab, fa.go, fa.ge);
#ifdef RAMX_PRK_TIMING
  FAMCHK(hipMalloc((void **)&fa.dbg, 8 * 8 * sizeof(unsigned long long)));
  FAMCHK(hipMemset(fa.dbg, 0, 8 * 8 * sizeof(unsigned long long)));
#endif
  FAMCHK(hipEventRecord(d->ev_begin, d->stream));
  if (!d->cls_init)
  {
    for (int c = 0; c < RAMX_NGROUP; c++)
    {
      FAMCHK(hipStreamCreateWithFlags(&d->cls_stream[c], hipStreamNonBlocking));
      FAMCHK(hipEventCreateWithFlags(&d->cls_done[c], hipEventDisableTiming));
    }
    FAMCHK(hipEventCreateWithFlags(&d->cls_ready, hipEventDisableTiming));
    d->cls_init = 1;
  }
  if (n_dev > 0)
  {
    if ((rc = ensure(&d->d_devdesc, &d->cap_devdesc, sizeof(CpDevDesc) * hdev.size()))) goto done;
    if ((rc = ensure(&d->d_vote_sets, &d->cap_vote_sets, sizeof(PShard) * RAMX_CP_NSETS * NSHARD * (size_t)n_dev))) goto done;
    if ((rc = ensure(&d->d_err_sets, &d->cap_err_sets, 64 * (size_t)n_dev))) goto done;
    FAMCHK(hipMemcpyAsync(d->d_devdesc, hdev.data(), sizeof(CpDevDesc) * hdev.size(), hipMemcpyHostToDevice, d->stream));
    FAMCHK(hipMemsetAsync(d->d_vote_sets, 0, sizeof(PShard) * RAMX_CP_NSETS * NSHARD * (size_t)n_dev, d->stream));
    FAMCHK(hipMemsetAsync(d->d_err_sets, 0, 64 * (size_t)n_dev, d->stream));
  }
  FAMCHK(hipEventRecord(d->cls_ready, d->stream));
  for (int c = 0; c < RAMX_NGROUP; c++) FAMCHK(hipStreamWaitEvent(d->cls_stream[c], d->cls_ready, 0));
  if (n_dev > 0)
  {
    CPArgs ca;
    memset(&ca, 0, sizeof(ca));
    ca.bases = d->d_bases; ca.bounds = d->d_bounds; ca.trim = d->d_trim; ca.ctl_out = dctl; ca.cons_out = d->d_cons;
    ca.Np = Np; ca.KW = KW; ca.L = L; ca.go = p->gapopen; ca.ge = p->gapextn; ca.cap = p->cappenalty; ca.minimp = p->minimprovement;
    ca.when_to_stop = p->when_to_stop;
    memcpy(ca.tab, tab9, sizeof(ca.tab));
    ca.nranks = 1; ca.rank = 0;
    {
      hipStream_t st = d->cls_stream[RAMX_NGROUP - 1];
      ca.dev = d->d_devdesc; ca.vote = d->d_vote_sets; ca.err = d->d_err_sets; ca.vote_wave = dev_vw;
      { const char *td = getenv("RAMX_TEST_CP_DROP_TICKET"), *tf = getenv("RAMX_TEST_CP_DROP_FAMILY");
        ca.test_drop_row = td ? atoi(td) : 0; ca.test_drop_id = tf ? atoi(tf) : -1; }
      cp_test_hooks(ca);
#ifdef RAMX_CP_TIMING
      if (n_cp == 0)
      {
        FAMCHK(hipMalloc((void **)&ca.dbg, (16 * 16 + 8) * sizeof(unsigned long long)));
        FAMCHK(hipMemset(ca.dbg, 0, (16 * 16 + 8) * sizeof(unsigned long long)));
        cp_dbg = ca.dbg;
      }
#endif
      for (size_t ro = 0; ro < dev_round_first.size(); ro++)
      {
        ca.dev = d->d_devdesc + dev_round_first[ro];
        rc = ramx_cp_launch_device(st, W, dev_k, dev_threads, dev_round_blocks[ro], ca);
        if (rc != RAMX_OK) { ramx_set_error("cell-parallel multi-family device launch failed (W %d, %d workgroups)", W, dev_round_blocks[ro]); goto done; }
      }
    }
  }
  if (n_cp > 0)
  {
    CPArgs ca;
    memset(&ca, 0, sizeof(ca));
    ca.bases = d->d_bases; ca.bounds = d->d_bounds; ca.trim = d->d_trim; ca.ctl_out = dctl; ca.cons_out = d->d_cons;
    ca.state_out = NULL;
    ca.Np = Np; ca.KW = KW; ca.L = L; ca.go = p->gapopen; ca.ge = p->gapextn; ca.cap = p->cappenalty; ca.minimp = p->minimprovement;
    ca.when_to_stop = p->when_to_stop;
    memcpy(ca.tab, tab9, sizeof(ca.tab));
    ca.lean_p = lean_p_of(ca.tab, ca.go, ca.ge);
    if (getenv("RAMX_CP_PEEK") != NULL)
    {
      const size_t need = (size_t)Np * (2 * W + 1) * sizeof(int2);
      if ((rc = ensure(&d->d_cpstate, &d->cap_cpstate, need))) goto done;
      FAMCHK(hipMemsetAsync(d->d_cpstate, 0, need, d->stream));
      FAMCHK(hipEventRecord(d->cls_ready, d->stream));
      for (int c = 0; c < RAMX_CP_NCLASS; c++) FAMCHK(hipStreamWaitEvent(d->cls_stream[c], d->cls_ready, 0));
      ca.state_out = (int2 *)d->d_cpstate;
      d->cpstate_W = W; d->cpstate_n = Np;
    }
#ifdef RAMX_CP_TIMING
    FAMCHK(hipMalloc((void **)&ca.dbg, (16 * 16 + 8) * sizeof(unsigned long long)));
    FAMCHK(hipMemset(ca.dbg, 0, (16 * 16 + 8) * sizeof(unsigned long long)));
    cp_dbg = ca.dbg;
#endif
    for (int c = 0; c < RAMX_CP_NCLASS; c++)
    {
      if (cls_count[c] == 0) continue;
      ca.fam = dfd + cls_first[c];
      rc = ramx_cp_launch_families(d->cls_stream[c], W, cp_k[c], cp_threads[c], cls_count[c], ca);
      if (rc != RAMX_OK) { ramx_set_error("cell-parallel family kernel launch failed (W %d, %d lanes per flank)", W, cp_k[c]); goto done; }
    }
  }
  if (legacy_any && !resident)
  {
    const size_t state_bytes = (size_t)Np * (W + 1) * sizeof(int4);
    if (state_bytes > d->cap_state || !d->d_state[0])
    {
      if (d->d_state[0]) FAMCHK(hipFree(d->d_state[0]));
      if (d->d_state[1] && d->d_state[1] != d->d_state[0]) FAMCHK(hipFree(d->d_state[1]));
      d->d_state[0] = d->d_state[1] = NULL; d->cap_state = 0;
      FAMCHK(hipMalloc((void **)&d->d_state[0], state_bytes));
      d->d_state[1] = d->d_state[0];
      d->cap_state = state_bytes;
    }
    FSArgs fs;
    memset(&fs, 0, sizeof(fs));
    fs.k.bases = d->d_bases; fs.k.bounds = d->d_bounds; fs.k.trim = d->d_trim; fs.k.S_in = d->d_state[0]; fs.k.S_out = d->d_state[0];
    fs.k.Np = Np; fs.k.Nx = Np; fs.k.W = W; fs.k.go = p->gapopen; fs.k.ge = p->gapextn; fs.k.cap = p->cappenalty;
    fs.k.minimp = p->minimprovement; fs.k.when_to_stop = p->when_to_stop;
    memcpy(fs.k.tab, fa.tab, sizeof(fs.k.tab));
    fs.fam = dfd; fs.ctl_out = dctl; fs.cons_out = d->d_cons; fs.L = L;
    const bool chain = p->gapopen > 0 || p->gapextn > 0 || d->force_chain;
#define RAMX_FS_LAUNCH(CH, BL, C) do { const int g_ = RAMX_CP_NCLASS + (C); if (cls_count[g_] > 0) { fs.fam = dfd + cls_first[g_]; \
      hipLaunchKernelGGL((ramx_family_stream_kernel<CH, BL>), dim3(cls_count[g_]), dim3(BL), 0, d->cls_stream[g_], fs); } } while (0)
    if (chain) { RAMX_FS_LAUNCH(true, 64, 0); RAMX_FS_LAUNCH(true, 128, 1); RAMX_FS_LAUNCH(true, 256, 2); RAMX_FS_LAUNCH(true, 512, 3); }
    else { RAMX_FS_LAUNCH(false, 64, 0); RAMX_FS_LAUNCH(false, 128, 1); RAMX_FS_LAUNCH(false, 256, 2); RAMX_FS_LAUNCH(false, 512, 3); }
#undef RAMX_FS_LAUNCH
    FAMCHK(hipGetLastError());
  }
  else if (legacy_any)
  {
    const int g0 = RAMX_CP_NCLASS;
    const int n256 = cls_count[g0] + cls_count[g0 + 1] + cls_count[g0 + 2], n512 = cls_count[g0 + 3];
    if (n256 > 0)
    {
      fa.fam = dfd + cls_first[g0];
      hipStream_t st = d->cls_stream[g0 + 2];
      rc = (W == 14) ? fam_launch<14, 256>(d, fa, n256, st) : (W == 20) ? fam_launch<20, 256>(d, fa, n256, st) : fam_launch<40, 256>(d, fa, n256, st);
      if (rc != RAMX_OK) goto done;
      cls_count[g0 + 2] = n256; cls_count[g0] = cls_count[g0 + 1] = 0;
    }
    if (n512 > 0)
    {
      fa.fam = dfd + cls_first[g0 + 3];
      hipStream_t st = d->cls_stream[g0 + 3];
      rc = (W == 14) ? fam_launch<14, 512>(d, fa, n512, st) : (W == 20) ? fam_launch<20, 512>(d, fa, n512, st) : fam_launch<40, 512>(d, fa, n512, st);
      if (rc != RAMX_OK) goto done;
    }
  }
  for (int c = 0; c < RAMX_NGROUP; c++)
    if (cls_count[c] > 0 || (c == RAMX_NGROUP - 1 && n_dev > 0))
    { FAMCHK(hipEventRecord(d->cls_done[c], d->cls_stream[c])); FAMCHK(hipStreamWaitEvent(d->stream, d->cls_done[c], 0)); }
  FAMCHK(hipEventRecord(d->ev_end, d->stream));
  FAMCHK(hipStreamSynchronize(d->stream));
  FAMCHK(hipEventElapsedTime(&ms, d->ev_begin, d->ev_end));
#ifdef RAMX_PRK_TIMING
  if (resident && legacy_any)
  {
    unsigned long long h[64];
    FAMCHK(hipMemcpy(h, fa.dbg, sizeof(h), hipMemcpyDeviceToHost));
    static const char *nm[6] = { "vote + stop rule", "winner table+barrier", "band + contrib", "wave reduce", "end barrier", "loop top" };
    const double cols = h[6] ? (double)h[6] : 1.0;
    fprintf(stderr, "FAM_TIMING family 0 (block 0), %.0f columns, ns per column per wave:\n", cols);
    for (int k = 0; k < 6; k++)
      fprintf(stderr, "FAM_TIMING %-22s w0 %7.1f  w1 %7.1f  w2 %7.1f  w3 %7.1f\n", nm[k], 10.0 * h[k] / cols, 10.0 * h[8 + k] / cols,
              10.0 * h[16 + k] / cols, 10.0 * h[24 + k] / cols);
  }
  if (fa.dbg) (void)hipFree(fa.dbg);
#endif
#ifdef RAMX_CP_TIMING
  if (cp_dbg)
  {
    unsigned long long h[16 * 16 + 8];
    FAMCHK(hipMemcpy(h, cp_dbg, sizeof(h), hipMemcpyDeviceToHost));
    static const char *nm[12] = { "vote read + stop rule", "(after speculative band)", "row update", "reductions", "records/slide/window",
                                  "sum+atomics+barrier", "-", "loop top", "wait: drain", "wait: samples + polling", "wait: fold",
                                  "wait: LDS + barrier" };
    const double cols = h[16 * 16] ? (double)h[16 * 16] : 1.0;
    fprintf(stderr, "CP_TIMING block 0, %.0f columns, shader clocks per column (waves 0, 1, last two):\n", cols);
    int nw = 0;
    for (int w = 0; w < 16; w++) if (h[w * 16 + 0]) nw = w + 1;
    for (int k = 0; k < 12; k++)
      if (k == 6) fprintf(stderr, "CP_TIMING mispredicted columns: %.0f of %.0f\n", (double)h[6], cols);
      else fprintf(stderr, "CP_TIMING %-24s w0 %7.1f  w1 %7.1f  w%d %7.1f  w%d %7.1f\n", nm[k], h[k] / cols, h[16 + k] / cols,
                          nw > 1 ? nw - 2 : 0, h[(nw > 1 ? nw - 2 : 0) * 16 + k] / cols, nw > 0 ? nw - 1 : 0, h[(nw > 0 ? nw - 1 : 0) * 16 + k] / cols);
  }
#endif
  hctl = (RamxCtl *)malloc(sizeof(RamxCtl) * n_families);
  FAMCHK(hipMemcpy(hctl, dctl, sizeof(RamxCtl) * n_families, hipMemcpyDeviceToHost));
  if (cons && L > 0) FAMCHK(hipMemcpy(cons, d->d_cons, (size_t)n_families * L, hipMemcpyDeviceToHost));
  if ((trim_high || trim_pos) && n_padded)
  {
    tmp = (int2 *)malloc((size_t)n_padded * sizeof(int2));
    FAMCHK(hipMemcpy(tmp, d->d_trim, (size_t)n_padded * sizeof(int2), hipMemcpyDeviceToHost));
    for (int i = 0; i < n_padded; i++) { if (trim_high) trim_high[i] = tmp[i].x; if (trim_pos) trim_pos[i] = tmp[i].y; }
  }
  for (int f = 0; f < n_families; f++)
  {
    const bool gave_up = grp[f] < 0 && hctl[f].pad != 0;
    if (timed_out) timed_out[f] = gave_up ? 1 : 0;
    if (gave_up && !timed_out) { ramx_set_error("batch mode: the vote of a multi-workgroup family timed out (bounded spin gave up)"); rc = RAMX_ERR_STATE; goto done; }
    if (!infos) continue;
    memset(&infos[f], 0, sizeof(ramx_run_info));
    infos[f].ret = hctl[f].max_row + 1;
    infos[f].rows_executed = hctl[f].rows_done;
    infos[f].limit_warning = (hctl[f].stopped && hctl[f].rows_done - 1 == L - 1) ? 1 : 0;
    infos[f].overflow32 = hctl[f].overflow;
    infos[f].n_extendable = fam_count[f];
    infos[f].launches = 1;
    infos[f].loop_ms = ms;
    infos[f].persistent = grp[f] < RAMX_CP_NCLASS ? 1 : (resident ? 1 : 2);
    infos[f].lanes_per_flank = grp[f] < 0 ? dev_k : (grp[f] < RAMX_CP_NCLASS ? cp_k[grp[f]] : 1);
    infos[f].respeculated_rows = grp[f] < 0 ? hctl[f].besta : 0;
  }
  rc = RAMX_OK;
done:
#undef FAMCHK
  if (cp_dbg) (void)hipFree(cp_dbg);
  free(hctl); free(tmp); free(hfd); free(grp);
  d->ready = 0;
  return rc;
}

extern "C" int ramx_dev_run_families(ramx_dev *d, const ramx_flank *flanks, int32_t n_padded, const int32_t *fam_first,
                                     const int32_t *fam_count, int32_t n_families, const ramx_params *p,
                                     ramx_run_info *infos, int8_t *cons, int32_t *trim_high, int32_t *trim_pos)
{
  std::vector<unsigned char> to((size_t)(n_families > 0 ? n_families : 1), 0);
  int rc = run_families_pass(d, flanks, n_padded, fam_first, fam_count, n_families, p, infos, cons, trim_high, trim_pos, true, to.data());
  if (rc != RAMX_OK) return rc;
  std::vector<int> redo;
  for (int f = 0; f < n_families; f++) if (to[f]) redo.push_back(f);
  if (redo.empty()) return RAMX_OK;
  fprintf(stderr, "ramx: batch mode: the device-wide vote of %zu multi-workgroup famil%s timed out (bounded spin); repeating "
                  "%s on the lane-per-flank route\n", redo.size(), redo.size() == 1 ? "y" : "ies", redo.size() == 1 ? "it" : "them");
  const int L = p->L;
  std::vector<ramx_flank> fl2;
  std::vector<int32_t> first2, count2;
  for (int f : redo)
  {
    first2.push_back((int32_t)fl2.size());
    count2.push_back(fam_count[f]);
    const int padded = ((fam_count[f] + 63) / 64) * 64;
    for (int i = 0; i < padded; i++)
    {
      ramx_flank x;
      if (i < fam_count[f]) x = flanks[fam_first[f] + i];
      else { memset(&x, 0, sizeof(x)); x.t_lo = 1; x.t_hi = 0; x.step = 1; }
      fl2.push_back(x);
    }
  }
  const int n2 = (int)redo.size(), np2 = (int)fl2.size();
  std::vector<ramx_run_info> inf2((size_t)n2);
  std::vector<int8_t> cons2((size_t)n2 * (L > 0 ? L : 1));
  std::vector<int32_t> th2((size_t)np2 + 1), tp2((size_t)np2 + 1);
  rc = run_families_pass(d, fl2.data(), np2, first2.data(), count2.data(), n2, p, inf2.data(), cons2.data(), th2.data(), tp2.data(), false, NULL);
  if (rc != RAMX_OK) return rc;
  for (int k = 0; k < n2; k++)
  {
    const int f = redo[k];
    if (infos) infos[f] = inf2[k];
    if (cons && L > 0) memcpy(cons + (size_t)f * L, cons2.data() + (size_t)k * L, (size_t)L);
    for (int i = 0; i < fam_count[f]; i++)
    {
      if (trim_high) trim_high[fam_first[f] + i] = th2[first2[k] + i];
      if (trim_pos) trim_pos[fam_first[f] + i] = tp2[first2[k] + i];
    }
  }
  return RAMX_OK;
}

extern "C" int ramx_dev_run_direction(ramx_dev *d, ramx_run_info *info)
{
  if (!d || !d->ready) { ramx_set_error("ramx_dev_run_direction: begin_direction has not been called"); return RAMX_ERR_STATE; }
  HIPCHK(hipSetDevice(d->ordinal));
  const ramx_params &p = d->p;
  const int L = p.L;
  KArgs a;
  memset(&a, 0, sizeof(a));
  a.bases = d->d_bases; a.bounds = d->d_bounds; a.trim = d->d_trim; a.cons_out = d->d_cons;
  a.Np = d->Np; a.Nx = d->Nx; a.W = p.bandwidth; a.go = p.gapopen; a.ge = p.gapextn; a.cap = p.cappenalty;
  a.minimp = p.minimprovement; a.when_to_stop = p.when_to_stop;
  memcpy(a.tab, d->tab, sizeof(a.tab));
  const bool multi = dev_is_multi(d);

  auto slot = [&](int r) { return d->d_sums + (size_t)(((r % 3) + 3) % 3) * NSHARD * 4; };
  int launches = 0, nsamp = 0, pending = -1, chk = 0, lanes = 1, prk_local_rc = RAMX_OK;
  bool persistent = false;
  const bool tracing = d->trace_cb != NULL || d->verbose_cb != NULL;
  const bool verbose_trace = d->verbose_cb != NULL;
  const int Bt = 2 * p.bandwidth + 1;
  auto deliver_trace = [&](int r, int besta) -> int
  {
    std::vector<int8_t> codes;
    std::vector<int2> best((size_t)d->Nx + 1), gaps((size_t)d->Nx + 1);
    std::vector<int32_t> bs((size_t)d->Nx + 1), bi((size_t)d->Nx + 1), gfl(2 * (size_t)d->Nx + 2), cand(16 * (size_t)d->Nx + 16);
    if (d->Nx && r >= 0) HIPCHK(hipMemcpy(best.data(), d->d_dbg_best, (size_t)d->Nx * sizeof(int2), hipMemcpyDeviceToHost));
    for (int i = 0; i < d->Nx; i++) { bs[i] = best[i].x; bi[i] = best[i].y; }
    if (d->trace_cb && r >= 0)
    {
      codes.resize((size_t)d->Nx * Bt + 1);
      if (d->Nx) HIPCHK(hipMemcpy(codes.data(), d->d_dbg_codes, (size_t)d->Nx * Bt, hipMemcpyDeviceToHost));
      d->trace_cb(r, besta, codes.data(), bs.data(), bi.data(), d->trace_user);
    }
    if (d->verbose_cb)
    {
      if (d->Nx)
      {
        HIPCHK(hipMemcpy(cand.data(), d->d_dbg_cand, (size_t)d->Nx * 16 * sizeof(int), hipMemcpyDeviceToHost));
        HIPCHK(hipMemcpy(gaps.data(), d->d_dbg_gap, (size_t)d->Nx * sizeof(int2), hipMemcpyDeviceToHost));
      }
      for (int i = 0; i < d->Nx; i++) { gfl[2 * i] = gaps[i].x; gfl[2 * i + 1] = gaps[i].y; }
      std::vector<int32_t> band;
      if (d->verbose_band && d->Nx)
      {
        band.resize((size_t)d->Nx * 8 * Bt);
        HIPCHK(hipMemcpy(band.data(), d->d_dbg_band, band.size() * sizeof(int32_t), hipMemcpyDeviceToHost));
      }
      d->verbose_cb(r, besta, d->Nx, bs.data(), bi.data(), gfl.data(), cand.data(), band.empty() ? NULL : band.data(), d->verbose_user);
    }
    return RAMX_OK;
  };
  auto trace_buffers = [&](KArgs &ka) -> int
  {
    int trc;
    if ((trc = ensure(&d->d_dbg_best, &d->cap_dbg_best, (size_t)d->Np * sizeof(int2))) != RAMX_OK) return trc;
    ka.dbg_best = d->d_dbg_best;
    ka.dbg_codes = NULL; ka.dbg_cand = NULL; ka.dbg_gap = NULL; ka.dbg_band = NULL;
    if (d->trace_cb)
    {
      if ((trc = ensure(&d->d_dbg_codes, &d->cap_dbg_codes, (size_t)d->Np * Bt)) != RAMX_OK) return trc;
      ka.dbg_codes = d->d_dbg_codes;
    }
    if (verbose_trace)
    {
      if ((trc = ensure(&d->d_dbg_cand, &d->cap_dbg_cand, (size_t)d->Np * 16 * sizeof(int))) != RAMX_OK) return trc;
      if ((trc = ensure(&d->d_dbg_gap, &d->cap_dbg_gap, (size_t)d->Np * sizeof(int2))) != RAMX_OK) return trc;
      ka.dbg_cand = d->d_dbg_cand; ka.dbg_gap = d->d_dbg_gap;
      if (d->verbose_band)
      {
        if ((trc = ensure(&d->d_dbg_band, &d->cap_dbg_band, (size_t)d->Np * 8 * Bt * sizeof(int))) != RAMX_OK) return trc;
        ka.dbg_band = d->d_dbg_band;
      }
    }
    return RAMX_OK;
  };
  rt_mark(NULL);
  {
    bool lazy = false;
    if (!tracing && d->Nx > 0)
    {
      int blk = 0, blks = 0, sp = 0, rb = 0, pb = 0, pbs = 0;
      bool can32 = false;
      int lrc = prk_local_can(d, a, L, multi, &can32, &blk, &blks);
      if (lrc != RAMX_OK) return lrc;
      if ((lrc = pk_route(d, a, L, multi, can32, &lazy, &sp, &rb, &pb, &pbs)) != RAMX_OK) return lrc;
      if (lazy && !multi && d->cp_flanks_ok && getenv("RAMX_NO_CP_DEVICE") == NULL && ramx_cp_max_family(a.W, a.go, a.ge, d->tab, L) > 0)
      {
        int dev = 0, cus = 0, k = 0, th = 0, nb = 0, vwf = 0;
        HIPCHK(hipGetDevice(&dev));
        HIPCHK(hipDeviceGetAttribute(&cus, hipDeviceAttributeMultiprocessorCount, dev));
        const char *mx = getenv("RAMX_CP_DEVICE_MAXN");
        if (mx == NULL || d->Nx <= atoi(mx)) ramx_cp_device_plan(a.W, d->Nx, cus, 0, &k, &th, &nb, &vwf);
        if (k > 0 && k < RAMX_CP_MIN_K_OVER_PACKED && getenv("RAMX_CP_K") == NULL) k = 0;
        if (k > 0) lazy = false;
      }
    }
    if (!lazy) { const int prc = pack_rest(d); if (prc != RAMX_OK) return prc; }
  }
  rt_mark("route (occupancy answers)");
  const bool cp_multi_ok = !multi || (d->peer_ready && d->nranks >= 2 && L < 65536 && getenv("RAMX_NO_PEER") == NULL);
  if (!tracing && cp_multi_ok && !d->force_chain && L > 0 && getenv("RAMX_NO_PERSISTENT") == NULL && getenv("RAMX_NO_CP_DEVICE") == NULL &&
      (multi || d->Nx > 0))
  {
    int dev = 0, cus = 0, k = 0, th = 0, nb = 0, vwf = 0;
    HIPCHK(hipGetDevice(&dev));
    HIPCHK(hipDeviceGetAttribute(&cus, hipDeviceAttributeMultiprocessorCount, dev));
    const char *mx = getenv("RAMX_CP_DEVICE_MAXN");
    if (d->cp_flanks_ok && ramx_cp_max_family(a.W, a.go, a.ge, d->tab, L) > 0 && (mx == NULL || d->Nx <= atoi(mx)))
      ramx_cp_device_plan(a.W, d->Nx > 0 ? d->Nx : 1, cus, 0, &k, &th, &nb, &vwf);
    if (k > 0 && k < RAMX_CP_MIN_K_OVER_PACKED && getenv("RAMX_CP_K") == NULL)
    {
      int blk = 0, blks = 0, sp = 0, rb = 0, pb = 0, pbs = 0;
      bool can32 = false, pkq = false;
      int lrc = prk_local_can(d, a, L, multi, &can32, &blk, &blks);
      if (lrc != RAMX_OK) return lrc;
      if ((lrc = pk_route(d, a, L, multi, can32, &pkq, &sp, &rb, &pb, &pbs)) != RAMX_OK) return lrc;
      if (pkq) k = 0;
    }
    if (multi)
    {
      if (d->hostbox_host)
      {
        HIPCHK(hipStreamSynchronize(d->stream));
        memset((void *)d->hostbox_host, 0, sizeof(PeerBox));
        __sync_synchronize();
      }
      else
      {
        HIPCHK(hipMemsetAsync(d->xbox, 0, sizeof(PeerBox), d->stream));
        HIPCHK(hipStreamSynchronize(d->stream));
      }
      int cannot = k > 0 ? 0 : 1;
      int arc = host_allreduce_flag(d, &cannot);
      if (arc != RAMX_OK) return arc;
      if (cannot) k = 0;
    }
    if (k > 0)
    {
      int lrc = RAMX_OK;
      bool accepted = false;
      auto launch = [&]() -> int
      {
        { const int prc = pack_rest(d); if (prc != RAMX_OK) return prc; }
        CPArgs ca;
        memset(&ca, 0, sizeof(ca));
        ca.bases = d->d_bases; ca.bounds = d->d_bounds; ca.trim = d->d_trim; ca.ctl_out = d->d_ctl; ca.cons_out = d->d_cons;
        ca.Np = d->Np; ca.KW = d->KW; ca.L = L; ca.go = a.go; ca.ge = a.ge; ca.cap = a.cap; ca.minimp = a.minimp; ca.when_to_stop = a.when_to_stop;
        memcpy(ca.tab, d->tab, sizeof(ca.tab));
        {
          std::vector<CpDevDesc> hd((size_t)nb);
          for (int i = 0; i < nb; i++) { memset(&hd[i], 0, sizeof(CpDevDesc)); hd[i].first = 0; hd[i].nx = d->Nx; hd[i].b = i; hd[i].nb = nb; hd[i].id = 0; }
          int drc = ensure(&d->d_devdesc, &d->cap_devdesc, sizeof(CpDevDesc) * (size_t)nb);
          if (drc != RAMX_OK) return drc;
          HIPCHK(hipMemcpyAsync(d->d_devdesc, hd.data(), sizeof(CpDevDesc) * (size_t)nb, hipMemcpyHostToDevice, d->stream));
          HIPCHK(hipStreamSynchronize(d->stream));
        }
        ca.dev = d->d_devdesc; ca.vote = d->d_vote; ca.err = d->d_err; ca.S = d->d_state[0]; ca.vote_wave = vwf;
        { const char *td = getenv("RAMX_TEST_CP_DROP_TICKET"); ca.test_drop_row = td ? atoi(td) : 0; ca.test_drop_id = -1; }
        cp_test_hooks(ca);
        ca.nranks = 1; ca.rank = 0;
        if (multi)
        {
          ca.nranks = d->nranks; ca.rank = d->rank; ca.peers = (PeerBox *const *)d->d_peer; ca.box = d->xbox; ca.mirror = NULL;
          if (d->hostbox_host)
          {
            if (!d->hostbox_mirror) HIPCHK(hipMalloc((void **)&d->hostbox_mirror, sizeof(PeerBox)));
            HIPCHK(hipMemsetAsync(d->hostbox_mirror, 0, sizeof(PeerBox), d->stream));
            ca.mirror = d->hostbox_mirror;
          }
          const char *tf = getenv("RAMX_TEST_FAIL_PRK_RANK");
          if (tf && atoi(tf) == d->rank) { ramx_set_error("test hook: forced failure of the cell-parallel launch on rank %d", d->rank); return RAMX_ERR_HIP; }
        }
        HIPCHK(hipMemsetAsync(d->d_vote, 0, RAMX_CP_NSETS * NSHARD * sizeof(PShard), d->stream));
        HIPCHK(hipMemsetAsync(d->d_err, 0, 64, d->stream));
        HIPCHK(hipMemsetAsync(d->d_ctl, 0, 2 * sizeof(RamxCtl), d->stream));
#ifdef RAMX_CP_TIMING
        HIPCHK(hipMalloc((void **)&ca.dbg, (16 * 16 + 8) * sizeof(unsigned long long)));
        HIPCHK(hipMemset(ca.dbg, 0, (16 * 16 + 8) * sizeof(unsigned long long)));
#endif
        HIPCHK(hipEventRecord(d->ev_begin, d->stream));
        if (multi) test_delay_rank(d);
        int crc = ramx_cp_launch_device(d->stream, a.W, k, th, nb, ca);
        if (crc != RAMX_OK)
        {
#ifdef RAMX_CP_TIMING
          (void)hipFree(ca.dbg);
#endif
          ramx_set_error("cell-parallel device launch failed (W %d, %d lanes per flank, %d workgroups)", a.W, k, nb);
          return crc;
        }
        accepted = true;
        HIPCHK(hipEventRecord(d->ev_end, d->stream));
        HIPCHK(hipStreamSynchronize(d->stream));
#ifdef RAMX_CP_TIMING
        if (vwf)
        {
          unsigned long long h[16 * 16 + 8];
          HIPCHK(hipMemcpy(h, ca.dbg, sizeof(h), hipMemcpyDeviceToHost));
          const double cols = h[16 * 16] ? (double)h[16 * 16] : 1.0;
          fprintf(stderr, "SP_TIMING workgroup 0, %d workgroups x %d threads, K %d, %.0f rows; shader clocks (100 MHz) per row\n", nb, th, k, cols);
          fprintf(stderr, "SP_TIMING vote wave: tickets wait+fold %.1f | winner+forward %.1f | stop rule, decision %.1f | loop %.1f | waiting for band sums %.1f | forwarded at once %.0f %%\n",
                  h[0] / cols, h[1] / cols, h[2] / cols, h[3] / cols, h[4] / cols, 100.0 * h[5] / cols);
          for (int wv = 1; wv < th / 64; wv++)
            fprintf(stderr, "SP_TIMING band wave %d: idle %.1f | planning %.1f | rows %.1f\n", wv, h[wv * 16 + 0] / cols, h[wv * 16 + 1] / cols, h[wv * 16 + 2] / cols);
        }
        (void)hipFree(ca.dbg);
#endif
        return RAMX_OK;
      };
      lrc = launch();
      RamxCtl c0;
      memset(&c0, 0, sizeof(c0));
      int bad = lrc != RAMX_OK;
      if (!bad && hipMemcpy(&c0, d->d_ctl, sizeof(c0), hipMemcpyDeviceToHost) != hipSuccess) bad = 1;
      bad = bad || c0.pad != 0;
      if (multi)
      {
        if (lrc != RAMX_OK) (void)hipStreamSynchronize(d->stream);
        int frc = host_allreduce_flag(d, &bad);
        if (frc != RAMX_OK) return frc;
        if (bad)
        {
          fprintf(stderr, "ramx: cross-device cell-parallel launch gave up or failed on some rank; repeating the direction with per-column "
                          "launches and leaving the mailbox path off for the rest of this process\n");
          d->peer_ready = 0;
        }
      }
      else if (lrc != RAMX_OK && accepted)
        return lrc;
      else if (lrc != RAMX_OK)
      {
        (void)hipStreamSynchronize(d->stream);
        (void)hipGetLastError();
        fprintf(stderr, "ramx: cell-parallel device launch not possible (%s); continuing on the lane-per-flank route\n", ramx_last_error());
      }
      else if (bad)
        fprintf(stderr, "ramx: device-wide vote of the cell-parallel launch timed out (bounded spin); repeating the direction with "
                        "per-column launches\n");
      if (!bad) { persistent = true; lanes = k; launches = 1; }
    }
  }
  const bool cp_done = persistent;
  rt_mark("cell-parallel plan / launch");
  if (!cp_done)
  {
  HIPCHK(hipMemsetAsync(d->d_sums, 0, 3 * NSHARD * 4 * sizeof(long long), d->stream));
  HIPCHK(hipEventRecord(d->ev_begin, d->stream));
  a.r = -1; a.S_in = d->d_state[0]; a.S_out = d->d_state[1]; a.ctl_in = d->d_ctl; a.ctl_out = d->d_ctl + 1;
  a.sums_in = slot(0); a.sums_out = slot(0); a.sums_zero = slot(1); a.nshards_in = NSHARD;
  if (verbose_trace)
  {
    int trc = trace_buffers(a);
    if (trc != RAMX_OK) return trc;
    launch_column_trace(d, a, true);
    HIPCHK(hipGetLastError());
    HIPCHK(hipStreamSynchronize(d->stream));
    if ((trc = deliver_trace(-1, 0)) != RAMX_OK) return trc;
  }
  else launch_column<true>(d, a);
  HIPCHK(hipGetLastError());
  rt_mark("boundary row launched");
  {
    if (d->d_state[0] != d->d_state[1]) { ramx_set_error("persistent path needs the in-place row buffer"); }
    else if (!tracing)
    {
      prk_local_rc = prk_run(d, a, L, &persistent);
      if (prk_local_rc != RAMX_OK && !(multi && persistent)) return prk_local_rc;
    }
  }
  if (persistent && multi)
  {
    int bad = prk_local_rc != RAMX_OK;
    RamxCtl c0[2];
    unsigned errw = 0;
    memset(c0, 0, sizeof(c0));
    if (!bad)
    {
      if (hipStreamSynchronize(d->stream) != hipSuccess || hipMemcpy(c0, d->d_ctl, sizeof(c0), hipMemcpyDeviceToHost) != hipSuccess ||
          hipMemcpy(&errw, d->d_err, sizeof(errw), hipMemcpyDeviceToHost) != hipSuccess) bad = 1;
    }
    else (void)hipStreamSynchronize(d->stream);
    bad = bad || c0[0].pad != 0 || c0[1].pad != 0 || errw != 0;
    int frc = host_allreduce_flag(d, &bad);
    if (frc != RAMX_OK) return frc;
    if (bad)
    {
      fprintf(stderr, "ramx: cross-device persistent launch gave up on some rank; repeating the direction with per-column launches "
                      "and leaving the mailbox path off for the rest of this process\n");
      persistent = false;
      d->peer_ready = 0;
      HIPCHK(hipMemsetAsync(d->d_sums, 0, 3 * NSHARD * 4 * sizeof(long long), d->stream));
      a.r = -1; a.S_in = d->d_state[0]; a.S_out = d->d_state[1]; a.ctl_in = d->d_ctl; a.ctl_out = d->d_ctl + 1;
      a.sums_in = slot(0); a.sums_out = slot(0); a.sums_zero = slot(1); a.nshards_in = NSHARD;
      launch_column<true>(d, a);
      HIPCHK(hipMemsetAsync(d->d_ctl, 0, sizeof(RamxCtl), d->stream));
    }
  }
  else if (persistent)
  {
    HIPCHK(hipStreamSynchronize(d->stream));
    RamxCtl c0[2];
    unsigned errw = 0;
    {
      unsigned long long ew = 0;
      int drc;
      if ((drc = d2h_small(d, c0, d->d_ctl, sizeof(c0))) != RAMX_OK) return drc;
      if ((drc = d2h_small(d, &ew, d->d_err, sizeof(ew))) != RAMX_OK) return drc;
      errw = (unsigned)ew;
    }
    rt_mark("after the launch: control blocks, error word");
    if (c0[0].pad != 0 || c0[1].pad != 0 || errw != 0)
    {
      if (errw == 2 || errw == 3)
        fprintf(stderr, "ramx: the packed-row kernel refused %s (a cell outside the span computed for this scoring system); repeating "
                        "the direction with per-column launches\n", errw == 3 ? "the rows it was handed" : "a row it computed");
      else
      fprintf(stderr, "ramx: device-wide barrier of the persistent launch timed out (bounded spin); repeating the direction with "
                      "per-column launches\n");
      persistent = false;
      HIPCHK(hipMemsetAsync(d->d_sums, 0, 3 * NSHARD * 4 * sizeof(long long), d->stream));
      a.r = -1; a.S_in = d->d_state[0]; a.S_out = d->d_state[1]; a.ctl_in = d->d_ctl; a.ctl_out = d->d_ctl + 1;
      a.sums_in = slot(0); a.sums_out = slot(0); a.sums_zero = slot(1); a.nshards_in = NSHARD;
      launch_column<true>(d, a);
      HIPCHK(hipMemsetAsync(d->d_ctl, 0, sizeof(RamxCtl), d->stream));
    }
  }
  }
  d->last_persistent = persistent ? 1 : 0;
  if (!persistent) { const int prc = pack_rest(d); if (prc != RAMX_OK) return prc; }
  const int CHUNK = 64;
  const int stride = L > MAX_SAMPLES * 4 ? L / MAX_SAMPLES : 4;
  bool stopped = false;
  memset(d->h_ctl, 0, 4 * sizeof(RamxCtl));
  for (int r = 0; r < L && !stopped && !persistent; r++)
  {
    if (multi)
    {
      int hrc = host_allreduce_shards(d, slot(r));
      if (hrc != RAMX_OK) return hrc;
    }
    a.sums_in = slot(r); a.nshards_in = NSHARD;
    a.r = r; a.S_in = d->d_state[(r + 1) & 1]; a.S_out = d->d_state[r & 1];
    a.ctl_in = d->d_ctl + ((r + 1) & 1); a.ctl_out = d->d_ctl + (r & 1);
    a.sums_out = slot(r + 1); a.sums_zero = slot(r + 2);
    if (tracing)
    {
      int trc = trace_buffers(a);
      if (trc != RAMX_OK) return trc;
      launch_column_trace(d, a);
      launches++;
      HIPCHK(hipGetLastError());
      HIPCHK(hipStreamSynchronize(d->stream));
      RamxCtl c;
      HIPCHK(hipMemcpy(&c, a.ctl_out, sizeof(c), hipMemcpyDeviceToHost));
      if (c.rows_done == r + 1)
        if ((trc = deliver_trace(r, c.besta)) != RAMX_OK) return trc;
      if (c.stopped) stopped = true;
      continue;
    }
    const bool sample = (r % stride) == (stride / 2) && nsamp < MAX_SAMPLES;
    if (sample) HIPCHK(hipEventRecord(d->ev_s0[nsamp], d->stream));
    launch_column<false>(d, a);
    if (sample) { HIPCHK(hipEventRecord(d->ev_s1[nsamp], d->stream)); nsamp++; }
    launches++;
    if (((r + 1) % CHUNK) == 0 || r == L - 1)
    {
      HIPCHK(hipGetLastError());
      HIPCHK(hipMemcpyAsync(d->h_ctl + 2 * chk, d->d_ctl, 2 * sizeof(RamxCtl), hipMemcpyDeviceToHost, d->stream));
      HIPCHK(hipEventRecord(d->ev_chk[chk], d->stream));
      if (pending >= 0)
      {
        HIPCHK(hipEventSynchronize(d->ev_chk[pending]));
        const RamxCtl *h = d->h_ctl + 2 * pending;
        if (h[0].stopped || h[1].stopped) stopped = true;
      }
      pending = chk;
      chk ^= 1;
    }
  }
  if (!cp_done) HIPCHK(hipEventRecord(d->ev_end, d->stream));
  rt_mark("loop enqueued / pieces run");
  HIPCHK(hipStreamSynchronize(d->stream));
  RamxCtl h[2];
  { const int drc = d2h_small(d, h, d->d_ctl, sizeof(h)); if (drc != RAMX_OK) return drc; }
  rt_mark("final synchronisation, control blocks");
  const RamxCtl &f = (L == 0) ? h[1] : ((h[0].rows_done > h[1].rows_done) ? h[0] : h[1]);
  d->final_ctl = f;
  if (persistent)
  {
    launches = 1;
    if (f.pad != 0) { ramx_set_error("persistent kernel: device-wide barrier timed out (bounded spin gave up)"); return RAMX_ERR_STATE; }
  }
  if (info)
  {
    info->ret = f.max_row + 1;
    info->rows_executed = f.rows_done;
    info->limit_warning = (f.stopped && f.rows_done - 1 == L - 1) ? 1 : 0;
    info->overflow32 = f.overflow;
    info->n_extendable = d->Nx;
    info->launches = launches;
    float ms = 0;
    HIPCHK(hipEventElapsedTime(&ms, d->ev_begin, d->ev_end));
    info->loop_ms = ms;
    double acc = 0; int cnt = 0;
    for (int i = 0; i < nsamp; i++)
    {
      float t = 0;
      if (hipEventElapsedTime(&t, d->ev_s0[i], d->ev_s1[i]) == hipSuccess) { acc += t; cnt++; }
    }
    info->kernel_ms_avg = cnt ? acc / cnt : 0.0;
    info->kernel_samples = cnt;
    info->persistent = persistent ? 1 : 0;
    info->lanes_per_flank = lanes;
    info->respeculated_rows = cp_done ? f.besta : 0;
    info->packed_rows = (persistent && !cp_done && d->last_packed_r0 >= 0 && f.rows_done > d->last_packed_r0) ? f.rows_done - d->last_packed_r0 : 0;
    info->lean_rows = (persistent && !cp_done && d->last_packed_r0 >= 0) ? (f.besta & 0xffff) : 0;
    if (persistent && !cp_done && d->last_packed_r0 >= 0) info->respeculated_rows = (f.besta >> 16) & 0xffff;
  }
  return RAMX_OK;
}

extern "C" int ramx_dev_download(ramx_dev *d, int8_t *cons, int32_t cons_cap, int32_t *trim_high, int32_t *trim_pos)
{
  if (!d || !d->ready) { ramx_set_error("ramx_dev_download: nothing to download"); return RAMX_ERR_STATE; }
  HIPCHK(hipSetDevice(d->ordinal));
  const int rows = d->final_ctl.rows_done;
  const bool timing = getenv("RAMX_TIMING") != NULL;
  const double td0 = now_ms();
  if (cons)
  {
    if (cons_cap < rows) { ramx_set_error("cons buffer too small (%d < %d)", cons_cap, rows); return RAMX_ERR_ARG; }
    if (rows) { const int drc = d2h_small(d, cons, d->d_cons, (size_t)rows); if (drc != RAMX_OK) return drc; }
  }
  if ((trim_high || trim_pos) && d->Nx)
  {
    const size_t need = (size_t)d->Nx * sizeof(int2);
    if (need > d->cap_stage)
    {
      if (d->h_stage) HIPCHK(hipHostFree(d->h_stage));
      d->h_stage = NULL; d->cap_stage = 0;
      HIPCHK(hipHostMalloc(&d->h_stage, need + need / 2, hipHostMallocDefault));
      d->cap_stage = need + need / 2;
    }
    int2 *tmp = (int2 *)d->h_stage;
    const double td1 = now_ms();
    if (getenv("RAMX_DOWNLOAD_DMA"))
      HIPCHK(hipMemcpyAsync(tmp, d->d_trim, need, hipMemcpyDeviceToHost, d->stream));
    else
    {
      hipLaunchKernelGGL(ramx_to_host_kernel, dim3((d->Nx + 255) / 256), dim3(256), 0, d->stream, (const int2 *)d->d_trim, tmp, d->Nx);
      HIPCHK(hipGetLastError());
    }
    HIPCHK(hipStreamSynchronize(d->stream));
    if (timing) fprintf(stderr, "RAMX_TIMING       download: consensus %.3f ms, trim copy %.3f ms\n", td1 - td0, now_ms() - td1);
    for (int i = 0; i < d->Nx; i++)
    {
      if (trim_high) trim_high[i] = tmp[i].x;
      if (trim_pos) trim_pos[i] = tmp[i].y;
    }
  }
  return RAMX_OK;
}

extern "C" int ramx_dev_peek_state(ramx_dev *d, int32_t flank, int32_t *cells, int32_t *high, int32_t *pos)
{
  if (!d || !d->ready || flank < 0 || flank >= d->Nx) { ramx_set_error("ramx_dev_peek_state: bad argument"); return RAMX_ERR_ARG; }
  HIPCHK(hipSetDevice(d->ordinal));
  const int W = d->p.bandwidth, Q = W + 1, B = 2 * W + 1;
  const int rows = d->final_ctl.rows_done;
  const int4 *S = d->d_state[(rows - 1) & 1];
  const int tile = flank / 64, lane = flank % 64;
  for (int q = 0; q < Q; q++)
  {
    int4 v;
    HIPCHK(hipMemcpy(&v, S + ((size_t)tile * Q + q) * 64 + lane, sizeof(v), hipMemcpyDeviceToHost));
    cells[4 * q] = v.x; cells[4 * q + 1] = v.y;
    if (2 * q + 1 < B) { cells[4 * q + 2] = v.z; cells[4 * q + 3] = v.w; }
    else { if (high) *high = v.z; if (pos) *pos = v.w; }
  }
  return RAMX_OK;
}

extern "C" int ramx_dev_peek_family_state(ramx_dev *d, int32_t flank, int32_t *cells)
{
  if (!d) d = ramx_default_device();
  if (!d || !d->d_cpstate || flank < 0 || flank >= d->cpstate_n || !cells)
  { ramx_set_error("ramx_dev_peek_family_state: nothing kept (set RAMX_CP_PEEK=1 before the batch call)"); return RAMX_ERR_ARG; }
  HIPCHK(hipSetDevice(d->ordinal));
  const int B = 2 * d->cpstate_W + 1;
  HIPCHK(hipMemcpy(cells, d->d_cpstate + (size_t)flank * B, (size_t)B * sizeof(int2), hipMemcpyDeviceToHost));
  return RAMX_OK;
}

extern "C" int ramx_dev_family_route_max(ramx_dev *d, const ramx_params *p)
{
  if (!d || !p || !p->matrix) return 512;
  int tab9[RAMX_NCLASS][4];
  for (int c = 0; c < RAMX_NCLASS; c++)
  {
    const int code = (c == 8) ? RAMX_SYM_N : c;
    for (int k = 0; k < 4; k++) tab9[c][k] = p->matrix[k * 100 + code];
  }
  if (d->force_chain || getenv("RAMX_NO_CP_DEVICE") != NULL || getenv("RAMX_NO_PERSISTENT") != NULL) return 512;
  const int m = ramx_cp_max_family(p->bandwidth, p->gapopen, p->gapextn, tab9, p->L);
  if (m <= 0) return 512;
  const int s1 = ramx_cp_single_family_max(p->bandwidth);
  return s1 < m ? s1 : m;
}

extern "C" int ramx_dev_set_row_trace(ramx_dev *d, ramx_row_trace_cb cb, void *user)
{
  if (!d) d = ramx_default_device();
  if (!d) return RAMX_ERR_NO_DEVICE;
  d->trace_cb = cb;
  d->trace_user = user;
  return RAMX_OK;
}

extern "C" int ramx_dev_set_row_verbose(ramx_dev *d, ramx_row_verbose_cb cb, void *user)
{
  if (!d) d = ramx_default_device();
  if (!d) return RAMX_ERR_NO_DEVICE;
  d->verbose_cb = cb;
  d->verbose_user = user;
  return RAMX_OK;
}

extern "C" int ramx_dev_set_verbose_band(ramx_dev *d, int on)
{
  if (!d) d = ramx_default_device();
  if (!d) return RAMX_ERR_NO_DEVICE;
  d->verbose_band = on ? 1 : 0;
  return RAMX_OK;
}

extern "C" int ramx_dev_set_allreduce_cb(ramx_dev *d, ramx_allreduce_cb cb, void *user)
{
  if (!d) { ramx_set_error("ramx_dev_set_allreduce_cb: bad argument"); return RAMX_ERR_ARG; }
  d->cb = cb;
  d->cb_user = user;
  return RAMX_OK;
}

extern "C" int ramx_comm_unique_id(uint8_t id[128])
{
  ncclUniqueId u;
  ncclResult_t r = ncclGetUniqueId(&u);
  if (r != ncclSuccess) { ramx_set_error("ncclGetUniqueId: %s", ncclGetErrorString(r)); return RAMX_ERR_COMM; }
  memcpy(id, &u, 128);
  return RAMX_OK;
}

extern "C" int ramx_dev_comm_init(ramx_dev *d, const uint8_t id[128], int rank, int nranks)
{
  if (!d || rank < 0 || rank >= nranks) { ramx_set_error("ramx_dev_comm_init: bad argument"); return RAMX_ERR_ARG; }
  HIPCHK(hipSetDevice(d->ordinal));
  d->rank = rank; d->nranks = nranks;
  if (nranks == 1 && getenv("RAMX_COMM_SINGLE") == NULL) return RAMX_OK;
  ncclUniqueId u;
  memcpy(&u, id, 128);
  ncclResult_t r = ncclCommInitRank(&d->comm, nranks, u, rank);
  if (r != ncclSuccess) { ramx_set_error("ncclCommInitRank: %s", ncclGetErrorString(r)); d->comm = NULL; return RAMX_ERR_COMM; }
  return RAMX_OK;
}

extern "C" int ramx_dev_comm_size(ramx_dev *d)
{
  if (!d) { ramx_set_error("ramx_dev_comm_size: bad argument"); return RAMX_ERR_ARG; }
  if (!d->comm) return 1;
  int n = 0;
  ncclResult_t r = ncclCommCount(d->comm, &n);
  if (r != ncclSuccess) { ramx_set_error("ncclCommCount: %s", ncclGetErrorString(r)); return RAMX_ERR_COMM; }
  return n;
}
```

repeatafterme_amd/csrc/ramx_kernels_packed.h:

```cpp
#pragma once

#include "ramx_kernels_vote.h"
#include "ramx_pk_api.h"

template <int W>
struct PkCfg
{
  static constexpr int B = 2 * W + 1, NP = W + 1, NW = (B + 8) / 8 + 2, NG = (B + 31) / 32, Q = W + 1;
};

#define PKB_NEG2 ((int)0x80008000u)
#ifndef PKB_GROUP
#define PKB_GROUP 2
#endif
#ifndef PKB_PT
#define PKB_PT 2
#endif

__device__ __forceinline__ int pkb_add_sat(int a, int b) { return pk_i(__builtin_elementwise_add_sat(pk_v(a), pk_v(b))); }
__device__ __forceinline__ int pkb_sub_sat(int a, int b) { return pk_i(__builtin_elementwise_sub_sat(pk_v(a), pk_v(b))); }
__device__ __forceinline__ int pkb_max(int a, int b) { return pk_i(__builtin_elementwise_max(pk_v(a), pk_v(b))); }
__device__ __forceinline__ void pkb_add_to_hi(int &dst, int a, int b) { asm("v_add_i16 %0, %1, %2 op_sel:[0,0,1] clamp" : "+v"(dst) : "v"(a), "v"(b)); }
__device__ __forceinline__ int pkb_add_lo(int a, int b) { int d; asm("v_add_i16 %0, %1, %2 clamp" : "=v"(d) : "v"(a), "v"(b)); return d; }
__device__ __forceinline__ int pkb_hmax(int p) { const pk_s2 q = pk_v(p); return q.x > q.y ? (int)q.x : (int)q.y; }
__device__ __forceinline__ unsigned pkb_lds_off(const void *p) { return (unsigned)(size_t)(__attribute__((address_space(3))) const void *)p; }

__device__ __forceinline__ unsigned pkb_mask_word(unsigned wv, int kb, int bdy9x4 )
{
  int s = bdy9x4 - 32 * kb;
  s = s < 0 ? 0 : s;
  const unsigned m = s >= 32 ? 0u : (0xffffffffu << s);
  return wv | m;
}

struct PkTabs
{
  int4 t4[4][256];
  int tp[4][256];
};

template <int BLOCK>
__device__ __forceinline__ void pkb_tabs_init(PkTabs &pt, const int (&tab)[RAMX_NCLASS][4])
{
  for (int i = threadIdx.x; i < 256; i += BLOCK)
  {
    const int hi = i >> 4, lo = (i & 15) ^ ((hi & 3) << 2);
    int q[4];
#pragma unroll
    for (int c = 0; c < 4; c++)
    {
      const int sl = lo < RAMX_NCLASS ? tab[lo][c] : (lo == 15 ? -32768 : 0);
      const int sh = hi < RAMX_NCLASS ? tab[hi][c] : (hi == 15 ? -32768 : 0);
      q[c] = (sl & 0xffff) | (sh << 16);
      pt.tp[c][i] = q[c];
    }
#pragma unroll
    for (int wv = 0; wv < 4; wv++) pt.t4[wv][i] = make_int4(q[wv], q[(wv + 1) & 3], q[(wv + 2) & 3], q[(wv + 3) & 3]);
  }
}

template <int W, int BLOCK, bool FULL>
__device__ __forceinline__ void pkb_band(const int go2, const int ge2, const PkTabs &pt, const int wsel, const int ph4, const unsigned (&w)[PkCfg<W>::NW],
                                         int (&R)[PkCfg<W>::NP], int (&E)[PkCfg<W>::NP], int &best, int (&kg)[PkCfg<W>::NG], int (&bA)[4], int &maxE)
{
  constexpr int B = PkCfg<W>::B, NP = PkCfg<W>::NP, NG = PkCfg<W>::NG, PT = PKB_PT;
  const char *tb = FULL ? reinterpret_cast<const char *>(&pt.t4[0][0]) : reinterpret_cast<const char *>(&pt.tp[0][0]);
  const unsigned wrep = (unsigned)wsel * 0x01010101u;
  const int hmask = (int)0xffff0000u;
  int C = PKB_NEG2, Rprev = PKB_NEG2;
  best = PKB_NEG2; maxE = PKB_NEG2;
#pragma unroll
  for (int c = 0; c < 4; c++) bA[c] = PKB_NEG2;
#pragma unroll
  for (int g = 0; g < NG; g++) kg[g] = -2147483647 - 1;
  unsigned Alo = 0, Ahi = 0;
  int tQ[PT];
  int cQ[FULL ? PT : 1][4];
  auto lookup = [&](auto kc, auto qc) __attribute__((always_inline))
  {
    constexpr int k = decltype(kc)::value, qi = decltype(qc)::value;
    if constexpr ((k & 3) == 0)
    {
      unsigned A = __builtin_amdgcn_alignbit(w[(k >> 2) + 1], w[k >> 2], ph4);
      A ^= (A >> 2) & 0x0c0c0c0cu;
      Alo = __builtin_amdgcn_perm(wrep, A, 0x04010400u);
      Ahi = __builtin_amdgcn_perm(wrep, A, 0x04030402u);
    }
    const unsigned Aw = (k & 2) ? Ahi : Alo;
    if constexpr (FULL)
    {
      const int4 v4 = *reinterpret_cast<const int4 *>(tb + pk_word_shl<(k & 1), 4>(Aw));
      cQ[qi][0] = v4.x; cQ[qi][1] = v4.y; cQ[qi][2] = v4.z; cQ[qi][3] = v4.w;
      tQ[qi] = v4.x;
    }
    else tQ[qi] = *reinterpret_cast<const int *>(tb + pk_word_shl<(k & 1), 2>(Aw));
  };
  static_for([&](auto kc) __attribute__((always_inline)) { lookup(kc, kc); }, std::make_integer_sequence<int, PT>{});
  static_for([&](auto kc) __attribute__((always_inline))
  {
    constexpr int k = decltype(kc)::value;
    if constexpr ((k % PKB_GROUP) == 0)
    {
      if constexpr (FULL) asm volatile("" ::"v"(C), "v"(bA[0]), "v"(bA[1]), "v"(bA[2]), "v"(bA[3]), "v"(maxE), "v"(kg[(k > 0 ? 2 * k - 1 : 0) >> 5]));
      else asm volatile("" ::"v"(best), "v"(C));
      __builtin_amdgcn_sched_barrier(0);
    }
    const int S = tQ[0];
    int sc[4] = { 0, 0, 0, 0 };
    if constexpr (FULL) { sc[0] = cQ[0][0]; sc[1] = cQ[0][1]; sc[2] = cQ[0][2]; sc[3] = cQ[0][3]; }
#pragma unroll
    for (int q = 0; q + 1 < PT; q++)
    {
      tQ[q] = tQ[q + 1];
      if constexpr (FULL) { cQ[q][0] = cQ[q + 1][0]; cQ[q][1] = cQ[q + 1][1]; cQ[q][2] = cQ[q + 1][2]; cQ[q][3] = cQ[q + 1][3]; }
    }
    if constexpr (k + PT < NP) lookup(std::integral_constant<int, (k + PT < NP ? k + PT : 0)>{}, std::integral_constant<int, PT - 1>{});
    const int PeP = k + 1 < NP ? E[k + 1 < NP ? k + 1 : 0] : PKB_NEG2;
    const int sub = pkb_add_sat(R[k], S);
    const int sg = pkb_add_sat(sub, go2);
    const int t = pk_max3_lll(sg, PeP, C);
    pkb_add_to_hi(C, t, ge2);
    int m = pkb_max(pkb_max(sub, PeP), C);
    E[k] = C;
    if constexpr (FULL) { if constexpr (k > 0) maxE = pkb_max(maxE, C); }
    if constexpr (2 * k + 1 < B)
    {
      const int t2 = pk_max3_hhh(sg, PeP, C);
      C = pkb_add_lo(t2, ge2);
    }
    else m = (m & 0xffff) | (int)0x80000000u;
    R[k] = m;
    if constexpr (FULL)
    {
      constexpr int g = (2 * k) >> 5;
      const int klo = (int)(((unsigned)m << 16) | (unsigned)(31 - ((2 * k) & 31)));
      if constexpr (2 * k + 1 < B)
      {
        const int khi = (m & hmask) | (31 - ((2 * k + 1) & 31));
        kg[g] = imax3(kg[g], klo, khi);
      }
      else kg[g] = imax(kg[g], klo);
      const int ms = (int)__builtin_amdgcn_alignbit((unsigned)m, (unsigned)Rprev, 16);
#pragma unroll
      for (int c = 0; c < 4; c++) bA[c] = pkb_max(bA[c], pkb_add_sat(ms, sc[c]));
      Rprev = m;
    }
    else best = pkb_max(best, m);
  }, std::make_integer_sequence<int, NP>{});
}

template <int W, int BLOCK>
__device__ __forceinline__ void pkb_leader_rows(const PkTabs &pt, int *scr , const int ph, const int leader,
                                                const int pbase, const int jhi, const int bestF,
                                                const unsigned (&w)[PkCfg<W>::NW], const int (&R)[PkCfg<W>::NP], const int (&E)[PkCfg<W>::NP],
                                                int (&bestA)[4], int &jbest)
{
  constexpr int B = PkCfg<W>::B, NW = PkCfg<W>::NW, NP = PkCfg<W>::NP;
  constexpr int NH = (B + 63) / 64;
  const int lane = threadIdx.x & 63;
  if (lane == leader)
  {
    static_for([&](auto kc) __attribute__((always_inline)) { constexpr int k = decltype(kc)::value; scr[k] = R[k]; scr[NP + k] = E[k]; },
               std::make_integer_sequence<int, NP>{});
    static_for([&](auto kc) __attribute__((always_inline)) { constexpr int k = decltype(kc)::value; scr[2 * NP + k] = (int)w[k]; },
               std::make_integer_sequence<int, NW>{});
  }
  __builtin_amdgcn_wave_barrier();
  const int bf = __builtin_amdgcn_readlane(bestF, leader);
  const int lbase = __builtin_amdgcn_readlane(pbase, leader);
  const int ljhi = __builtin_amdgcn_readlane(jhi, leader);
  int ta[4] = { NEG, NEG, NEG, NEG }, me = NEG;
  unsigned long long hit[NH];
#pragma unroll
  for (int h = 0; h < NH; h++)
  {
    const int k = lane + 64 * h;
    const bool ok = k < B && k <= ljhi;
    const int kk = k < B ? k : 0;
    const int mw = scr[kk >> 1];
    const int m = lbase + ((kk & 1) ? (mw >> 16) : (int)(short)mw);
    const int g = kk + 1 + ph;
    const unsigned cls = ((unsigned)scr[2 * NP + (g >> 3)] >> (4 * (g & 7))) & 15u;
    if (ok && k + 1 <= ljhi)
    {
#pragma unroll
      for (int c = 0; c < 4; c++) ta[c] = imax(ta[c], m + (int)(short)pt.tp[c][cls]);
    }
    if (ok && k >= 1)
    {
      const int cw = scr[NP + ((kk + 1) >> 1)];
      me = imax(me, lbase + ((kk & 1) ? (int)(short)cw : (cw >> 16)));
    }
    hit[h] = __ballot(ok && m == bf);
  }
  const int mx = wave_max_i32_dpp(me);
  int best[4];
#pragma unroll
  for (int c = 0; c < 4; c++) best[c] = imax(wave_max_i32_dpp(ta[c]), mx);
  int jb = 0;
#pragma unroll
  for (int h = NH - 1; h >= 0; h--)
    if (hit[h]) jb = 64 * h + __builtin_ctzll(hit[h]);
  if (lane == leader)
  {
#pragma unroll
    for (int c = 0; c < 4; c++) bestA[c] = best[c];
    jbest = jb;
  }
}

template <class A>
__device__ __forceinline__ int pkb_stop_rule(const A &a, const int r, const long long (&v)[4], const int fl, int *st, const int lane)
{
  long long mx = ((long long)__builtin_amdgcn_readfirstlane(st[1]) << 32) | (long long)(unsigned)__builtin_amdgcn_readfirstlane(st[0]);
  int mr = __builtin_amdgcn_readfirstlane(st[2]), ov = __builtin_amdgcn_readfirstlane(st[3]);
  long long cw = 0;
  int bw = 0;
#pragma unroll
  for (int k = 0; k < 4; k++)
  {
    const long long vk = ((long long)__builtin_amdgcn_readfirstlane((int)(v[k] >> 32)) << 32) |
                         (long long)(unsigned)__builtin_amdgcn_readfirstlane((int)v[k]);
    if (vk > 2147483647LL || vk < -2147483648LL) ov = 1;
    if (vk > cw) { cw = vk; bw = k; }
  }
  int dist = mr - r;
  dist = dist < 0 ? -dist : dist;
  const int nm = cw >= mx + (long long)dist * a.minimp ? 1 : 0;
  if (nm && !fl) { mr = r; mx = cw; }
  int d2 = r - mr;
  d2 = d2 < 0 ? -d2 : d2;
  const int stp = d2 >= a.when_to_stop ? 1 : 0;
  if (lane == 0) { st[0] = (int)mx; st[1] = (int)(mx >> 32); st[2] = mr; st[3] = ov; }
  return bw | (nm << 2) | (stp << 3) | (fl << 4);
}

#ifdef RAMX_PRK_TIMING
#ifdef RAMX_PRK_TIMING_TAIL
#define PKB_TICK_ON (2 * r >= a.L)
#else
#define PKB_TICK_ON true
#endif
#define PKB_TICK(k) do { const unsigned long long t_ = wall_clock64(); if (PKB_TICK_ON) tsum[k] += t_ - tlast; tlast = t_; } while (0)
#else
#define PKB_TICK(k) do { } while (0)
#endif

template <int W, int BLOCK>
__global__ __launch_bounds__(BLOCK, BLOCK / 256) void ramx_packed_kernel(const PKArgs a)
{
  constexpr int NP = PkCfg<W>::NP, NW = PkCfg<W>::NW, NG = PkCfg<W>::NG, Q = PkCfg<W>::Q, WPB = BLOCK / 64;
  constexpr bool VW = (BLOCK % 256) != 0;
  constexpr int BW = VW ? WPB - 1 : WPB, VOTER = VW ? BW : 0;
  constexpr bool SPEC = W <= 40;
  struct Smem
  {
    PkTabs pt;
    long long tot[2][2][4];
    int word[2][2];
    int cnt[2][2];
    int st[4];
    int lead[WPB][2 * NP + NW + 1];
    int eb[SPEC ? BLOCK * NP : 1];
  };
  __shared__ __attribute__((aligned(16))) Smem sm;
  const int lane = threadIdx.x & 63, wave = threadIdx.x >> 6;
  const int tile = blockIdx.x * BW + wave;
  const bool live = wave < BW && tile < (a.Np >> 6);
  const int n = (live ? tile : 0) * 64 + lane;
  int4 *S = a.S + (size_t)(live ? tile : 0) * Q * 64 + lane;
  const int2 bd = a.bounds[n];
  const int bdy = (n >= a.Nx) ? 0x3fffffff : (bd.x > bd.y ? -0x40000000 : bd.y);
#define PKB_BDY9X4(b) ((b) > 0x07ffffff ? 0x3fffffff : ((b) < -0x08000000 ? -0x40000000 : 4 * ((b) + 9)))
  const int shard = blockIdx.x % NSHARD;
  const int go2 = pk_two(a.go), ge2 = pk_two(a.ge);

  pkb_tabs_init<BLOCK>(sm.pt, a.tab);
  if (threadIdx.x < 16) (&sm.tot[0][0][0])[threadIdx.x] = 0;
  if (threadIdx.x < 4) (&sm.cnt[0][0])[threadIdx.x] = 0;
  if (threadIdx.x < 4) (&sm.word[0][0])[threadIdx.x] = 0;

  long long max_ext = 0;
  int max_row = -1, rows_done = a.r0, ovf = 0, stopped = 0, failed = 0, carried = 0;
  if (a.r0 > 0)
  {
    const RamxCtl *cp = a.ctl_in;
    const long long me = cp->max_ext;
    max_ext = ((long long)__builtin_amdgcn_readfirstlane((int)(me >> 32)) << 32) | (long long)(unsigned)__builtin_amdgcn_readfirstlane((int)me);
    max_row = __builtin_amdgcn_readfirstlane(cp->max_row);
    rows_done = __builtin_amdgcn_readfirstlane(cp->rows_done);
    ovf = __builtin_amdgcn_readfirstlane(cp->overflow);
    stopped = (__builtin_amdgcn_readfirstlane(cp->stopped) || rows_done < a.r0) ? 1 : 0;
    const int cpad = __builtin_amdgcn_readfirstlane(cp->pad);
    failed = cpad;
    carried = __builtin_amdgcn_readfirstlane(cp->besta);
  }
  else if (live) a.trim[n] = make_int2(0, 0);
  stopped = __builtin_amdgcn_readfirstlane(stopped); max_row = __builtin_amdgcn_readfirstlane(max_row);
  rows_done = __builtin_amdgcn_readfirstlane(rows_done); carried = __builtin_amdgcn_readfirstlane(carried);
  const bool skip = stopped || failed || a.r0 >= a.Lseg;
  if (threadIdx.x == 0) { sm.st[0] = (int)max_ext; sm.st[1] = (int)(max_ext >> 32); sm.st[2] = max_row; sm.st[3] = ovf; }

  if (blockIdx.x == a.nblocks)
  {
    if (wave != 0 || stopped || failed || a.r0 >= a.Lseg) return;
    for (int r = a.r0; r < a.Lseg; r++)
    {
      PShard *vb = a.vote;
      asm volatile("" : "+s"(vb));
      long long v[4];
      prk_wait_vote(a, vb, a.sums_in, r == a.r0 ? (a.r0 == 0 ? 1 : 2) : 0, r, lane, (a.nblocks - (lane & (NSHARD - 1)) + NSHARD - 1) / NSHARD, failed, v, true);
      const int fl = __any(failed) ? 1 : 0;
      const int dword = pkb_stop_rule(a, r, v, fl, sm.st, lane);
      if (fl) { if (lane == 0) __hip_atomic_fetch_max(a.err, 1u, __ATOMIC_RELAXED, __HIP_MEMORY_SCOPE_AGENT); break; }
      if (lane == 0) a.cons_out[r] = (signed char)(dword & 3);
      if (lane < NSHARD)
      {
        PShard *z = vb + (size_t)((r + 3) & (PRK_NSETS - 1)) * NSHARD + lane;
#pragma unroll
        for (int k = 0; k < 4; k++) __hip_atomic_store(&z->word[k], 0ULL, __ATOMIC_RELAXED, __HIP_MEMORY_SCOPE_AGENT);
      }
      if ((dword & 8) || r == a.L - 1) break;
    }
    return;
  }

  int R[NP], E[NP];
  int high, pos, pbase = 0;
  {
    const int jcut = bdy - (a.r0 - 1);
    int bmax = -2147483647 - 1, bmin = 2147483647;
    const int4 *S1 = S;
    asm volatile("" : "+v"(S1));
    static_for([&](auto qc) __attribute__((always_inline))
    {
      constexpr int q = decltype(qc)::value;
      if constexpr ((q & 7) == 0) __builtin_amdgcn_sched_barrier(0);
      const int4 v = S1[(size_t)q * 64];
      const int x0 = 2 * q <= jcut ? v.x : -2147483647 - 1, n0 = 2 * q <= jcut ? v.x : 2147483647;
      bmax = imax(bmax, x0); bmin = n0 < bmin ? n0 : bmin;
      if constexpr (q < W)
      {
        const int x1 = 2 * q + 1 <= jcut ? v.z : -2147483647 - 1, n1 = 2 * q + 1 <= jcut ? v.z : 2147483647;
        bmax = imax(bmax, x1); bmin = n1 < bmin ? n1 : bmin;
      }
      asm volatile("" : "+v"(bmax), "+v"(bmin));
    }, std::make_integer_sequence<int, Q>{});
    __builtin_amdgcn_sched_barrier(0);
    const bool none = bmax == -2147483647 - 1;
    pbase = none ? 0 : bmax;
    if (live && !skip && n < a.Nx && !none && (long long)bmax - (long long)bmin > (long long)a.spread)
      __hip_atomic_fetch_max(a.err, 3u, __ATOMIC_RELAXED, __HIP_MEMORY_SCOPE_AGENT);
    int jcut2 = jcut;
    const int4 *S2 = S;
    asm volatile("" : "+v"(jcut2), "+v"(S2));
    auto rel16 = [&](int x, bool inb) __attribute__((always_inline)) -> int
    {
      int d = x - pbase;
      d = d < -32768 ? -32768 : (d > 32767 ? 32767 : d);
      return inb ? d : -32768;
    };
    int eprev = -32768;
    static_for([&](auto qc) __attribute__((always_inline))
    {
      constexpr int q = decltype(qc)::value;
      if constexpr ((q & 7) == 0) __builtin_amdgcn_sched_barrier(0);
      const int4 v = S2[(size_t)q * 64];
      const bool in0 = 2 * q <= jcut2, in1 = q < W && 2 * q + 1 <= jcut2;
      const int m0 = rel16(v.x, in0), e0 = rel16(v.y, in0);
      const int m1 = q < W ? rel16(v.z, in1) : -32768, e1 = q < W ? rel16(v.w, in1) : -32768;
      R[q] = (m0 & 0xffff) | (m1 << 16);
      E[q] = (eprev & 0xffff) | (e0 << 16);
      eprev = e1;
      if constexpr (q == W) { high = v.z; pos = v.w; }
    }, std::make_integer_sequence<int, Q>{});
    __builtin_amdgcn_sched_barrier(0);
  }
  if (skip)
  {
    if (blockIdx.x == 0 && threadIdx.x == 0)
    {
      RamxCtl o;
      o.max_ext = max_ext; o.max_row = max_row; o.stopped = stopped; o.rows_done = rows_done; o.overflow = ovf; o.besta = carried; o.pad = failed;
      *a.ctl_out = o;
    }
    return;
  }

  unsigned w[NW], wnext;
  {
    const int k0 = (a.r0 + 8) >> 3;
    const unsigned *bp = a.bases + (size_t)k0 * a.Np + n;
    static_for([&](auto kc) __attribute__((always_inline)) { constexpr int k = decltype(kc)::value; w[k] = pkb_mask_word(bp[(size_t)k * a.Np], k0 + k, PKB_BDY9X4(bdy)); },
               std::make_integer_sequence<int, NW>{});
    wnext = bp[(size_t)NW * a.Np];
  }
  __syncthreads();

  int prevBest = 0x3fffffff;
  int full_rows = 0, lean_rows = 0, wrong_rows = 0;
#ifdef RAMX_PRK_TIMING
  unsigned long long tsum[6] = { 0, 0, 0, 0, 0, 0 }, tlast = wall_clock64();
#endif
  int spec = 0, guess = 0;
  for (int r = a.r0; r < a.Lseg; r++)
  {
    PKB_TICK(5);
    PShard *vb = a.vote;
    asm volatile("" : "+s"(vb));
    if (((r + 8) & 7) == 0 && r > a.r0)
    {
      static_for([&](auto kc) __attribute__((always_inline)) { constexpr int k = decltype(kc)::value; w[k] = w[k + 1]; }, std::make_integer_sequence<int, NW - 1>{});
      const int kn = ((r + 8) >> 3) + NW;
      int nn = n, bb = bdy;
      asm volatile("" : "+v"(nn), "+v"(bb));
      w[NW - 1] = pkb_mask_word(wnext, kn - 1, PKB_BDY9X4(bb));
      wnext = a.bases[(size_t)kn * a.Np + nn];
    }
    const int par = r & 1, npar = (r + 1) & 1;
    const bool hand_over = r == a.Lseg - 1 && a.Lseg < a.L;
    int besta = 0, next_guess = 0;
    long long dgw = 0;
    bool new_max = false, last_col = false;

    auto decide = [&]() __attribute__((always_inline)) -> bool
    {
      if (wave == VOTER)
      {
        long long v[4];
        int lv = lane;
        asm volatile("" : "+v"(lv));
        prk_wait_vote(a, vb, a.sums_in, r == a.r0 ? (a.r0 == 0 ? 1 : 2) : 0, r, lv, (a.nblocks - (lv & (NSHARD - 1)) + NSHARD - 1) / NSHARD, failed, v, blockIdx.x == a.xblock);
        const int fl = __any(failed) ? 1 : 0;
        const int dword = pkb_stop_rule(a, r, v, fl, sm.st, lane);
        const int bw = dword & 3;
        if (lane == 0)
        {
          sm.word[par][0] = dword;
          if (fl) __hip_atomic_fetch_max(a.err, 1u, __ATOMIC_RELAXED, __HIP_MEMORY_SCOPE_AGENT);
        }
        if (blockIdx.x == a.xblock && !fl)
        {
          if (lane == 0) a.cons_out[r] = (signed char)bw;
          if (lane < NSHARD)
          {
            PShard *z = vb + (size_t)((r + 3) & (PRK_NSETS - 1)) * NSHARD + lane;
#pragma unroll
            for (int k = 0; k < 4; k++) __hip_atomic_store(&z->word[k], 0ULL, __ATOMIC_RELAXED, __HIP_MEMORY_SCOPE_AGENT);
          }
        }
      }
      PKB_TICK(0);
      asm volatile("s_waitcnt lgkmcnt(0)\n\ts_barrier" ::: "memory");
      PKB_TICK(1);
      int dw, gw;
      asm volatile("ds_read_b64 %0, %1\n\ts_waitcnt lgkmcnt(0)" : "=v"(dgw) : "v"(pkb_lds_off(&sm.word[par][0])) : "memory");
      dw = __builtin_amdgcn_readfirstlane((int)dgw); gw = __builtin_amdgcn_readfirstlane((int)(dgw >> 32));
      next_guess = gw;
      if (dw & 16) { failed = 1; return false; }
      besta = dw & 3;
      new_max = (dw & 4) != 0;
      stopped = (dw >> 3) & 1;
      rows_done = r + 1;
      last_col = stopped || r == a.L - 1;
      return true;
    };

    auto arrive = [&](const int set, const long long t0, const long long t1, const long long t2, const long long t3) __attribute__((always_inline))
    {
      const long long mine = lane == 0 ? t0 : lane == 1 ? t1 : lane == 2 ? t2 : t3;
      int old = 0;
      if (lane < 4) asm volatile("ds_add_u64 %0, %1" : : "v"(pkb_lds_off(&sm.tot[set][npar][lane])), "v"(mine) : "memory");
      if (lane == 0) asm volatile("ds_add_rtn_u32 %0, %1, %2\n\ts_waitcnt lgkmcnt(0)" : "=v"(old) : "v"(pkb_lds_off(&sm.cnt[set][npar])), "v"(1) : "memory");
      old = __builtin_amdgcn_readfirstlane(old);
      if (old == WPB - 1)
      {
        long long t = 0;
        if (lane < 4)
        {
          asm volatile("ds_read_b64 %0, %1\n\ts_waitcnt lgkmcnt(0)" : "=v"(t) : "v"(pkb_lds_off(&sm.tot[set][npar][lane])) : "memory");
          if (set == 1)
          {
            asm volatile("ds_write_b64 %0, %1" : : "v"(pkb_lds_off(&sm.tot[set][npar][lane])), "v"(0LL) : "memory");
            if (hand_over)
            {
              int lq = lane;
              asm volatile("" : "+v"(lq));
              __hip_atomic_fetch_add(&a.sums_next[shard * 4 + lq], t, __ATOMIC_RELAXED, __HIP_MEMORY_SCOPE_AGENT);
            }
            else
            {
              PShard *sh = vb + (size_t)((r + 1) & (PRK_NSETS - 1)) * NSHARD + shard;
              __hip_atomic_fetch_add(&sh->word[lane], (unsigned long long)t + PRK_BIAS + PRK_TICKET, __ATOMIC_RELAXED, __HIP_MEMORY_SCOPE_AGENT);
            }
          }
        }
        if (set == 1 && lane == 0) asm volatile("ds_write_b32 %0, %1" : : "v"(pkb_lds_off(&sm.cnt[set][npar])), "v"(0) : "memory");
        if constexpr (SPEC)
        {
          const long long q0 = prk_readlane_u64((unsigned long long)t, 0), q1 = prk_readlane_u64((unsigned long long)t, 1);
          const long long q2 = prk_readlane_u64((unsigned long long)t, 2), q3 = prk_readlane_u64((unsigned long long)t, 3);
          long long c = 0;
          int g = 0;
          if (q0 > c) { c = q0; g = 0; }
          if (q1 > c) { c = q1; g = 1; }
          if (q2 > c) { c = q2; g = 2; }
          if (q3 > c) { c = q3; g = 3; }
          const int informative = !(q0 == q1 && q1 == q2 && q2 == q3) && a.spec_on;
          if (lane == 0) sm.word[par][1] = (informative << 8) | g;
        }
      }
    };

    int Rb[SPEC ? NP : 1], high_b = 0, pos_b = 0, prev_b = 0, pbase_b = 0;
    int *myEb = sm.eb + (SPEC ? threadIdx.x * NP : 0);
    bool pass_spec = false;
    int wsel = 0;
    if (spec)
    {
      if constexpr (SPEC)
      {
#ifndef PKB_PROBE_NO_BACKUP
        if (live)
        static_for([&](auto kc) __attribute__((always_inline)) { constexpr int k = decltype(kc)::value; Rb[k] = R[k]; myEb[k] = E[k]; }, std::make_integer_sequence<int, NP>{});
#else
        Rb[0] = R[0];
#endif
        high_b = high; pos_b = pos; prev_b = prevBest; pbase_b = pbase;
      }
      pass_spec = true;
      wsel = guess;
      if (a.test_wrong_every > 0 && (r % a.test_wrong_every) == 0) wsel = (guess + 1) & 3;
    }
    else
    {
      if (!decide()) break;
      wsel = besta;
    }
    bool confirmed_arrival = false;
    bool gave_up = false;
    for (;;)
    {
      const int set = pass_spec ? 0 : 1;
      const int jhi = bdy - r;
      const int capfloor = (high + a.cap) > 0 ? (high + a.cap) : 0;
      bool lean = false, early = false;
      unsigned long long leaders = 0;
      if (live && a.lean_p >= 0)
      {
        const unsigned long long keep = __ballot((n < a.Nx) && !((prevBest + 2 * a.lean_p <= capfloor) && (prevBest + a.lean_p <= high)));
        if (keep == 0) { lean = true; early = true; }
        else if (__popcll(keep) <= a.leader_max) { lean = true; leaders = keep; }
      }
      if (!live) early = true;
      const bool send = pass_spec || !last_col;
      if (early && send)
      {
        const long long t = wave_sum_nonneg31((live && n < a.Nx) ? capfloor : 0);
        arrive(set, t, t, t, t);
      }
      PKB_TICK(3);
      if (__builtin_amdgcn_readfirstlane(early ? 1 : 0) == 0) __builtin_amdgcn_s_setprio(2);

      int contrib[4] = { 0, 0, 0, 0 };
      if (live)
      {
        const int ph4 = 4 * ((r + 8) & 7);
        int best, kg[NG], bA[4], maxE;
        if (lean) pkb_band<W, BLOCK, false>(go2, ge2, sm.pt, wsel, ph4, w, R, E, best, kg, bA, maxE);
        else pkb_band<W, BLOCK, true>(go2, ge2, sm.pt, wsel, ph4, w, R, E, best, kg, bA, maxE);
        int rel, jbest = 0, bestA[4] = { NEG, NEG, NEG, NEG };
        if (lean) rel = pkb_hmax(best);
        else
        {
          int bkey = kg[NG - 1], bg = NG - 1;
          rel = kg[NG - 1] >> 16;
#pragma unroll
          for (int g = NG - 2; g >= 0; g--)
          {
            const int v = kg[g] >> 16;
            const bool take = v >= rel;
            rel = take ? v : rel;
            bkey = take ? kg[g] : bkey;
            bg = take ? g : bg;
          }
          jbest = 32 * bg + 31 - (bkey & 31);
          const int mE = pkb_hmax(maxE);
          int rot[4];
#pragma unroll
          for (int i = 0; i < 4; i++) rot[i] = jhi < 1 ? NEG : pbase + imax(pkb_hmax(bA[i]), mE);
#pragma unroll
          for (int c = 0; c < 4; c++)
          {
            const int i = (c - wsel) & 3;
            bestA[c] = i == 0 ? rot[0] : i == 1 ? rot[1] : i == 2 ? rot[2] : rot[3];
          }
        }
        const int bestF = jhi < 0 ? SENT : pbase + rel;
        for (unsigned long long rest = leaders; rest != 0; rest &= rest - 1)
          pkb_leader_rows<W, BLOCK>(sm.pt, sm.lead[wave], (r + 8) & 7, __builtin_ctzll(rest), pbase, jhi, bestF, w, R, E, bestA, jbest);
        if ((r & 63) == 63)
        {
          int mn = 0x7fff7fff, jj = jhi;
          asm volatile("" : "+v"(jj));
          static_for([&](auto kc) __attribute__((always_inline))
          {
            constexpr int k = decltype(kc)::value;
            int v = R[k];
            const bool in_hi = 2 * k + 1 < PkCfg<W>::B && 2 * k + 1 <= jj;
            v = in_hi ? v : ((v & 0xffff) | 0x7fff0000);
            v = 2 * k <= jj ? v : 0x7fff7fff;
            mn = pk_i(__builtin_elementwise_min(pk_v(mn), pk_v(v)));
          }, std::make_integer_sequence<int, NP>{});
          const pk_s2 q = pk_v(mn);
          const int lowest = q.x < q.y ? (int)q.x : (int)q.y;
          if (n < a.Nx && jhi >= 0 && rel - lowest > a.spread_rows) __hip_atomic_fetch_max(a.err, 2u, __ATOMIC_RELAXED, __HIP_MEMORY_SCOPE_AGENT);
        }
        if ((r & 15) == 15 && __any(jhi >= 0 && (rel > a.rebase || rel < -a.rebase)))
        {
          const int mv = jhi >= 0 ? rel : 0;
          const int bb = pk_two(mv);
          static_for([&](auto kc) __attribute__((always_inline)) { constexpr int k = decltype(kc)::value; R[k] = pkb_sub_sat(R[k], bb); E[k] = pkb_sub_sat(E[k], bb); },
                     std::make_integer_sequence<int, NP>{});
          pbase += mv;
        }
        prevBest = bestF;
        if (bestF > high) { high = bestF; pos = r + jbest - W; }
        if (n < a.Nx)
        {
          const int capv = high + a.cap;
#pragma unroll
          for (int c = 0; c < 4; c++)
          {
            const int b = bestA[c] < 0 ? 0 : bestA[c];
            contrib[c] = (b >= capv) ? b : capv;
          }
        }
        if (!pass_spec) { if (lean) lean_rows++; else full_rows++; }
      }
      PKB_TICK(2);
      if (!early && send)
      {
#ifndef PKB_PROBE_NO_REDUCE
        const long long t0 = wave_sum_nonneg31(contrib[0]), t1 = wave_sum_nonneg31(contrib[1]);
        const long long t2 = wave_sum_nonneg31(contrib[2]), t3 = wave_sum_nonneg31(contrib[3]);
#else
        const long long t0 = __builtin_amdgcn_readfirstlane(contrib[0]), t1 = __builtin_amdgcn_readfirstlane(contrib[1]);
        const long long t2 = __builtin_amdgcn_readfirstlane(contrib[2]), t3 = __builtin_amdgcn_readfirstlane(contrib[3]);
#endif
        arrive(set, t0, t1, t2, t3);
      }
      PKB_TICK(4);
      __builtin_amdgcn_s_setprio(0);
      if (!pass_spec) { confirmed_arrival = send; break; }
      if (!decide()) { gave_up = true; break; }
      const bool right = besta == wsel;
      if (wave == VOTER)
      {
        if (lane < 4)
        {
          long long t;
          asm volatile("ds_read_b64 %0, %1\n\ts_waitcnt lgkmcnt(0)" : "=v"(t) : "v"(pkb_lds_off(&sm.tot[0][npar][lane])) : "memory");
          asm volatile("ds_write_b64 %0, %1" : : "v"(pkb_lds_off(&sm.tot[0][npar][lane])), "v"(0LL) : "memory");
          if (right && !last_col)
          {
            if (hand_over)
            {
              int lq = lane;
              asm volatile("" : "+v"(lq));
              __hip_atomic_fetch_add(&a.sums_next[shard * 4 + lq], t, __ATOMIC_RELAXED, __HIP_MEMORY_SCOPE_AGENT);
            }
            else
            {
              PShard *sh = vb + (size_t)((r + 1) & (PRK_NSETS - 1)) * NSHARD + shard;
              __hip_atomic_fetch_add(&sh->word[lane], (unsigned long long)t + PRK_BIAS + PRK_TICKET, __ATOMIC_RELAXED, __HIP_MEMORY_SCOPE_AGENT);
            }
          }
        }
        if (lane == 0) asm volatile("ds_write_b32 %0, %1" : : "v"(pkb_lds_off(&sm.cnt[0][npar])), "v"(0) : "memory");
      }
      if (right) break;
      if constexpr (SPEC)
      {
        if (live)
        static_for([&](auto kc) __attribute__((always_inline)) { constexpr int k = decltype(kc)::value; R[k] = Rb[k]; E[k] = myEb[k]; }, std::make_integer_sequence<int, NP>{});
        high = high_b; pos = pos_b; prevBest = prev_b; pbase = pbase_b;
      }
      wrong_rows++;
      pass_spec = false;
      wsel = besta;
    }
    if (gave_up) break;
#ifndef PKB_PROBE_NO_TRIM
    if (new_max && live)
#else
    if (new_max && live && r < 0)
#endif
    {
      int nn = n;
      asm volatile("" : "+v"(nn));
      a.trim[nn] = make_int2(high, pos);
    }
    if (last_col || hand_over) break;
    if constexpr (SPEC)
    {
      if (confirmed_arrival)
      {
        asm volatile("s_waitcnt lgkmcnt(0)\n\ts_barrier" ::: "memory");
        int gw;
        asm volatile("ds_read_b32 %0, %1\n\ts_waitcnt lgkmcnt(0)" : "=v"(gw) : "v"(pkb_lds_off(&sm.word[par][1])) : "memory");
        next_guess = __builtin_amdgcn_readfirstlane(gw);
      }
      spec = next_guess >> 8; guess = next_guess & 3;
    }
  }
#ifdef RAMX_PRK_TIMING
  if (a.dbg != NULL && (threadIdx.x & 63) == 0)
  {
#pragma unroll
    for (int k = 0; k < 6; k++) a.dbg[((size_t)blockIdx.x * WPB + wave) * 8 + k] += tsum[k];
    a.dbg[((size_t)blockIdx.x * WPB + wave) * 8 + 6] += (unsigned long long)full_rows;
    a.dbg[((size_t)blockIdx.x * WPB + wave) * 8 + 7] += (unsigned long long)lean_rows;
  }
#endif

  if (live && rows_done > a.r0)
  {
    int bz = bdy;
    asm volatile("" : "+v"(bz));
    const int rl = rows_done - 1, jh = bz - rl;
    const int edge = rl < W ? a.go + (rl + 1) * a.ge : SENT;
    int tid = threadIdx.x;
    asm volatile("" : "+v"(tid));
    int4 *S3 = a.S + (size_t)(blockIdx.x * BW + (tid >> 6)) * Q * 64 + (tid & 63);
    auto val = [&](int half, int j, bool is_e) __attribute__((always_inline)) -> int
    {
      if (j > jh) { const int f = j < W ? edge : SENT; return is_e ? f + a.ge : f; }
      return pbase + half;
    };
    static_for([&](auto qc) __attribute__((always_inline))
    {
      constexpr int q = decltype(qc)::value;
      const int m0 = val((int)(short)R[q], 2 * q, false), e0 = val(E[q] >> 16, 2 * q, true);
      if constexpr (q < W)
      {
        const int m1 = val(R[q] >> 16, 2 * q + 1, false), e1 = val((int)(short)E[q + 1 < NP ? q + 1 : 0], 2 * q + 1, true);
        S3[(size_t)q * 64] = make_int4(m0, e0, m1, e1);
      }
      else S3[(size_t)q * 64] = make_int4(m0, e0, high, pos);
    }, std::make_integer_sequence<int, Q>{});
  }
  if (blockIdx.x == 0 && threadIdx.x == 0)
  {
    RamxCtl o;
    o.max_ext = ((long long)sm.st[1] << 32) | (long long)(unsigned)sm.st[0]; o.max_row = sm.st[2]; o.stopped = stopped; o.rows_done = rows_done;
    o.overflow = sm.st[3];
    o.besta = ((carried & 0xffff) + lean_rows) | ((((carried >> 16) & 0xffff) + wrong_rows) << 16);
    o.pad = failed;
    *a.ctl_out = o;
  }
}
```

repeatafterme_amd/csrc/ramx_packed.hip:

```cpp
#define RAMX_SECONDARY_TU 1
#include "ramx_kernels_packed.h"

#include <stdlib.h>

#define PK_REBASE 6000

int ramx_pk_plan(int W, int go, int ge, const int (&tab)[RAMX_NCLASS][4], int *spread, int *rebase)
{
  *spread = 0; *rebase = 0;
  if (!(W == 14 || W == 20 || W == 40 || W == 80) || go > 0 || ge > 0 || getenv("RAMX_NO_PK") != NULL) return 0;
  long long P = 0, mn = 0;
  for (int c = 0; c < RAMX_NCLASS; c++)
    for (int k = 0; k < 4; k++)
    {
      if (tab[c][k] > P) P = tab[c][k];
      if (-(long long)tab[c][k] > mn) mn = -(long long)tab[c][k];
    }
  const long long GO = -(long long)go, GE = -(long long)ge;
  const long long sp = 3LL * W * (P + mn + GE) + GO + (long long)W * GE;
  const long long lag = PK_REBASE + 16 * (P > mn ? P : mn);
  if (sp + lag + mn + GO + GE + 64 > 32000) return 0;
  if (lag + P + 64 > 32000) return 0;
  *spread = (int)sp; *rebase = PK_REBASE;
  return 1;
}

template <int W, int BLOCK>
static int pk_capacity(int *out)
{
  static int cached = -1;
  if (cached >= 0) { *out = cached; return RAMX_OK; }
  int per_cu = 0, dev = 0, cus = 0;
  if (hipGetDevice(&dev) != hipSuccess) return RAMX_ERR_HIP;
  if (hipDeviceGetAttribute(&cus, hipDeviceAttributeMultiprocessorCount, dev) != hipSuccess) return RAMX_ERR_HIP;
  if (hipOccupancyMaxActiveBlocksPerMultiprocessor(&per_cu, ramx_packed_kernel<W, BLOCK>, BLOCK, 0) != hipSuccess) return RAMX_ERR_HIP;
  int lim = 1;
  if (const char *e = getenv("RAMX_PK_WG_PER_CU")) lim = atoi(e) >= 2 && BLOCK == 256 ? 2 : 1;
  if (per_cu > lim) per_cu = lim;
  *out = per_cu * cus;
  cached = *out;
  return RAMX_OK;
}

template <int W>
static int pk_shape(int tiles, int *block, int *blocks)
{
  int cap = 0, rc;
  *block = 0; *blocks = 0;
  const bool vw = W <= 40 && getenv("RAMX_PK_NO_VW") == NULL;
  if constexpr (W <= 40) rc = vw ? pk_capacity<W, 320>(&cap) : pk_capacity<W, 256>(&cap);
  else rc = pk_capacity<W, 256>(&cap);
  if (rc != RAMX_OK) return rc;
  if (getenv("RAMX_PK_NO_256") != NULL) cap = 0;
  if ((tiles + 3) / 4 <= cap) { *block = vw ? 320 : 256; *blocks = (tiles + 3) / 4; return RAMX_OK; }
  if constexpr (W <= 40)
  {
    if ((rc = pk_capacity<W, 512>(&cap)) != RAMX_OK) return rc;
    if ((tiles + 7) / 8 <= cap) { *block = 512; *blocks = (tiles + 7) / 8; }
  }
  return RAMX_OK;
}

int ramx_pk_capacity(int W, int block, int *cap)
{
  *cap = 0;
  if (block == 256)
    switch (W) { case 14: return pk_capacity<14, 256>(cap); case 20: return pk_capacity<20, 256>(cap); case 40: return pk_capacity<40, 256>(cap); case 80: return pk_capacity<80, 256>(cap); }
  if (block == 320)
    switch (W) { case 14: return pk_capacity<14, 320>(cap); case 20: return pk_capacity<20, 320>(cap); case 40: return pk_capacity<40, 320>(cap); }
  if (block == 512)
    switch (W) { case 14: return pk_capacity<14, 512>(cap); case 20: return pk_capacity<20, 512>(cap); case 40: return pk_capacity<40, 512>(cap); }
  return RAMX_OK;
}

int ramx_pk_shape(int W, int tiles, int *block, int *blocks)
{
  switch (W)
  {
    case 14: return pk_shape<14>(tiles, block, blocks);
    case 20: return pk_shape<20>(tiles, block, blocks);
    case 40: return pk_shape<40>(tiles, block, blocks);
    case 80: return pk_shape<80>(tiles, block, blocks);
  }
  *block = 0; *blocks = 0;
  return RAMX_OK;
}

template <int W>
static int pk_launch(hipStream_t st, int block, int blocks, const PKArgs &a)
{
  const int grid = blocks + (a.xblock != 0 ? 1 : 0);
  if (block == 256) hipLaunchKernelGGL((ramx_packed_kernel<W, 256>), dim3(grid), dim3(256), 0, st, a);
  else if (block == 320)
  {
    if constexpr (W <= 40) hipLaunchKernelGGL((ramx_packed_kernel<W, 320>), dim3(grid), dim3(320), 0, st, a);
    else return RAMX_ERR_ARG;
  }
  else if (block == 512)
  {
    if constexpr (W <= 40) hipLaunchKernelGGL((ramx_packed_kernel<W, 512>), dim3(grid), dim3(512), 0, st, a);
    else return RAMX_ERR_ARG;
  }
  else return RAMX_ERR_ARG;
  return hipGetLastError() == hipSuccess ? RAMX_OK : RAMX_ERR_HIP;
}

int ramx_pk_launch(hipStream_t st, int W, int block, int blocks, const PKArgs &a)
{
  switch (W)
  {
    case 14: return pk_launch<14>(st, block, blocks, a);
    case 20: return pk_launch<20>(st, block, blocks, a);
    case 40: return pk_launch<40>(st, block, blocks, a);
    case 80: return pk_launch<80>(st, block, blocks, a);
  }
  return RAMX_ERR_UNSUPPORTED;
}
```

repeatafterme_amd/csrc/ramx_pk_api.h:

```cpp
#pragma once

#include <hip/hip_runtime.h>

#include "ramx_kernels_common.h"

struct PShard;
struct PeerBox;

struct PKArgs
{
  int4 *S;
  const unsigned *bases;
  const int2 *bounds;
  int2 *trim;
  const long long *sums_in;
  PShard *vote;
  const RamxCtl *ctl_in;
  RamxCtl *ctl_out;
  signed char *cons_out;
  unsigned *err;
  PeerBox *const *peers;
  PeerBox *box;
  PeerBox *mirror;
  int rank, nranks;
  int xblock;
  long long *sums_next;
  int Np, Nx, r0, Lseg, L, go, ge, cap, minimp, when_to_stop, nblocks;
  int tab[RAMX_NCLASS][4];
  int lean_p;
  int leader_max;
  int spread;
  int spread_rows;
  int rebase;
  int spec_on;
  int test_wrong_every;
  unsigned long long *dbg;
};

int ramx_pk_plan(int W, int go, int ge, const int (&tab)[RAMX_NCLASS][4], int *spread, int *rebase);
int ramx_pk_capacity(int W, int block, int *cap);
int ramx_pk_shape(int W, int tiles, int *block, int *blocks);
int ramx_pk_launch(hipStream_t st, int W, int block, int blocks, const PKArgs &a);
```

repeatafterme_amd/device.py:

```python
from __future__ import annotations

import ctypes as C

import numpy as np

from . import _lib
from .datamodel import CoreSet, ExtendParams
from .extend import RunInfo, _info, _params


def resolve_flanks(direction: int, cores: CoreSet, bandwidth: int, L: int):
    L_ = _lib.lib()
    fc = _lib.FlatCores(cores.n, *[getattr(cores, k).ctypes.data for k in
                                   ("left_pos", "right_pos", "lower", "upper", "orient", "left_ext",
                                    "right_ext", "left_len", "right_len", "score")])
    flanks = (_lib.Flank * max(cores.n, 1))()
    idx = np.zeros(max(cores.n, 1), np.int32)
    nx = L_.ramx_resolve_flanks(int(direction), C.byref(fc), bandwidth, L, flanks, idx.ctypes.data)
    return (flanks, nx), idx[:nx].copy()


class Device:
    def __init__(self, ordinal: int = 0):
        self._L = _lib.lib()
        h = C.c_void_p()
        _lib.check(self._L.ramx_dev_create(ordinal, C.byref(h)), "ramx_dev_create")
        self._h = h
        self._keep = None
        self.nx = 0
        self.p = None

    def close(self):
        if self._h:
            self._L.ramx_dev_destroy(self._h)
            self._h = None

    def __del__(self):
        try:
            self.close()
        except Exception:
            pass

    def load_library(self, sequence: np.ndarray):
        assert sequence.dtype == np.int8 and sequence.flags.c_contiguous
        _lib.check(self._L.ramx_dev_load_library(self._h, sequence.ctypes.data, len(sequence)), "ramx_dev_load_library")

    def begin_direction(self, flanks, p: ExtendParams):
        arr, nx = flanks
        cp, keep = _params(p)
        self._keep = keep
        _lib.check(self._L.ramx_dev_begin_direction(self._h, arr, nx, C.byref(cp)), "ramx_dev_begin_direction")
        self.nx, self.p = nx, p

    def run_direction(self) -> RunInfo:
        ci = _lib.RunInfo()
        _lib.check(self._L.ramx_dev_run_direction(self._h, C.byref(ci)), "ramx_dev_run_direction")
        self.last = _info(ci)
        return self.last

    def download(self):
        rows = self.last.rows_executed
        cons = np.zeros(max(rows, 1), np.int8)
        th = np.zeros(max(self.nx, 1), np.int32)
        tp = np.zeros(max(self.nx, 1), np.int32)
        _lib.check(self._L.ramx_dev_download(self._h, cons.ctypes.data, len(cons), th.ctypes.data, tp.ctypes.data),
                   "ramx_dev_download")
        return cons[:rows], th[:self.nx], tp[:self.nx]

    def peek_state(self, flank: int):
        B = 2 * self.p.bandwidth + 1
        cells = np.zeros(4 * (self.p.bandwidth + 1), np.int32)
        hi, po = C.c_int32(), C.c_int32()
        _lib.check(self._L.ramx_dev_peek_state(self._h, flank, cells.ctypes.data, C.byref(hi), C.byref(po)),
                   "ramx_dev_peek_state")
        return cells[:2 * B].reshape(B, 2).copy(), hi.value, po.value

    def unique_id(self) -> np.ndarray:
        uid = np.zeros(128, np.uint8)
        _lib.check(self._L.ramx_comm_unique_id(uid.ctypes.data), "ramx_comm_unique_id")
        return uid

    def comm_init(self, uid: np.ndarray, rank: int, nranks: int):
        uid = np.ascontiguousarray(uid, dtype=np.uint8)
        _lib.check(self._L.ramx_dev_comm_init(self._h, uid.ctypes.data, rank, nranks), "ramx_dev_comm_init")

    def comm_size(self) -> int:
        return _lib.check(self._L.ramx_dev_comm_size(self._h), "ramx_dev_comm_size")

    def set_allreduce_callback(self, fn):
        def _cb(ptr, _user):
            vals = fn([ptr[i] for i in range(4)])
            for i in range(4):
                ptr[i] = int(vals[i])
        self._cb = _lib.ALLREDUCE_CB(_cb)
        _lib.check(self._L.ramx_dev_set_allreduce_cb(self._h, self._cb, None), "ramx_dev_set_allreduce_cb")

    def peer_setup(self, rank: int, world: int, all_gather_bytes, all_reduce_min, barrier) -> bool:
        import os
        only = os.environ.get("RAMX_PEER_KIND", "")
        token = 0x52414D58000000 + world
        self.peer_kind = None

        def selftest(ok):
            if all_reduce_min(ok) == 1:
                if self._L.ramx_dev_peer_selftest(self._h, 0, token) < 0:
                    ok = 0
                barrier()
                if ok and self._L.ramx_dev_peer_selftest(self._h, 1, token) != 1:
                    ok = 0
            return all_reduce_min(ok)

        if only in ("", "device"):
            ok = 1
            h = np.zeros(64, np.uint8)
            if self._L.ramx_dev_peer_export(self._h, h.ctypes.data) < 0:
                ok = 0
            handles = all_gather_bytes(h.tobytes())
            if all_reduce_min(ok) == 1:
                allh = np.frombuffer(b"".join(handles), np.uint8).copy()
                if self._L.ramx_dev_peer_import(self._h, allh.ctypes.data, rank, world) < 0:
                    ok = 0
            if selftest(ok) == 1:
                self._L.ramx_dev_peer_enable(self._h, 1)
                self.peer_kind = "device"
                return True
        if only in ("", "host"):
            mine = np.zeros(64, np.uint8)
            tag = (b"/ramx_box_%d_%s" % (os.getpid(), os.urandom(8).hex().encode()))[:63]
            mine[:len(tag)] = np.frombuffer(tag, np.uint8)
            name = bytes(all_gather_bytes(mine.tobytes())[0]).split(b"\0", 1)[0]
            ok = 1
            try:
                if rank == 0:
                    ok = 1 if self._L.ramx_dev_hostbox_attach(self._h, name, rank, world) >= 0 else 0
                barrier()
                if rank != 0:
                    ok = 1 if self._L.ramx_dev_hostbox_attach(self._h, name, rank, world) >= 0 else 0
                barrier()
                ok = selftest(ok)
            finally:
                if rank == 0:
                    self._L.ramx_hostbox_unlink(name)
            if ok == 1:
                self._L.ramx_dev_peer_enable(self._h, 1)
                self.peer_kind = "host"
                return True
        self._L.ramx_dev_peer_enable(self._h, 0)
        return False
```

Measured before the change: 17.75 billion.

## Offload long-running leader flanks to a dedicated service block via handoff slots

Adds a service block to the persistent packed kernel. A flank that stays a lean-mode leader for many consecutive rows can be handed to this block through atomic claim, answer, ready and release slots. The service block then computes that flank's band rows with wave-wide DPP scans, and the owning block drops it from its own work and vote contributions. The aim is to stop one straggler flank from keeping a whole block in non-lean mode. The cost is an extra block in the grid, more cross-block handshakes and spin waits, extra slot memsets per segment, and correctness risk in the handoff protocol.

```diff
diff --git a/include/ramx.h b/include/ramx.h
--- a/include/ramx.h
+++ b/include/ramx.h
@@ -144,6 +144,8 @@
 
 int ramx_dev_peek_state(ramx_dev *d, int32_t flank, int32_t *cells, int32_t *high, int32_t *pos);
 
+int ramx_dev_served_rows(ramx_dev *d);
+
 int ramx_dev_peek_family_state(ramx_dev *d, int32_t flank, int32_t *cells);
 
 typedef void (*ramx_row_trace_cb)(int32_t row, int32_t besta, const int8_t *codes ,
diff --git a/repeatafterme_amd/_lib.py b/repeatafterme_amd/_lib.py
--- a/repeatafterme_amd/_lib.py
+++ b/repeatafterme_amd/_lib.py
@@ -11,7 +11,7 @@
 EXPORTS = [
     "ramx_set_runtime", "ramx_extend_alignment", "ramx_extend_flat", "ramx_invalidate_library", "ramx_preload_library", "ramx_resolve_flanks", "ramx_last_error", "ramx_device_count",
     "ramx_dev_create", "ramx_dev_destroy", "ramx_dev_load_library", "ramx_dev_begin_direction",
-    "ramx_dev_run_direction", "ramx_dev_download", "ramx_dev_peek_state", "ramx_dev_peek_family_state", "ramx_dev_set_row_trace", "ramx_dev_run_families", "ramx_extend_batch", "ramx_comm_unique_id",
+    "ramx_dev_run_direction", "ramx_dev_download", "ramx_dev_peek_state", "ramx_dev_served_rows", "ramx_dev_peek_family_state", "ramx_dev_set_row_trace", "ramx_dev_run_families", "ramx_extend_batch", "ramx_comm_unique_id",
     "ramx_dev_comm_init", "ramx_dev_comm_size", "ramx_dev_set_allreduce_cb", "ramx_dev_peer_export", "ramx_dev_peer_import",
     "ramx_dev_peer_selftest", "ramx_dev_peer_enable", "ramx_dev_hostbox_attach", "ramx_hostbox_unlink", "ramx_get_matrix", "ramx_get_matrix_using_gap_penalties",
     "ramx_get_repeatscout_matrix", "ramx_free_scoring_system", "ramx_calculate_lambda",
@@ -90,6 +90,9 @@
         L.ramx_dev_download.argtypes = [C.c_void_p, C.c_void_p, C.c_int32, C.c_void_p, C.c_void_p]
         L.ramx_dev_peek_state.argtypes = [C.c_void_p, C.c_int32, C.c_void_p, C.POINTER(C.c_int32),
                                           C.POINTER(C.c_int32)]
+        if hasattr(L, "ramx_dev_served_rows"):
+            L.ramx_dev_served_rows.argtypes = [C.c_void_p]
+            L.ramx_dev_served_rows.restype = C.c_int
         L.ramx_dev_peek_family_state.argtypes = [C.c_void_p, C.c_int32, C.c_void_p]
         L.ramx_comm_unique_id.argtypes = [C.c_void_p]
         L.ramx_dev_comm_init.argtypes = [C.c_void_p, C.c_void_p, C.c_int, C.c_int]
diff --git a/repeatafterme_amd/csrc/ramx_device.hip b/repeatafterme_amd/csrc/ramx_device.hip
--- a/repeatafterme_amd/csrc/ramx_device.hip
+++ b/repeatafterme_amd/csrc/ramx_device.hip
@@ -70,7 +70,9 @@
   ramx_flank *d_flanks; unsigned *d_bases; int2 *d_bounds; int4 *d_state[2]; int2 *d_trim;
   long long *d_sums; RamxCtl *d_ctl; signed char *d_cons;
   PShard *d_vote; unsigned *d_err;
+  PkSlot *d_slots;
   int last_persistent;
+  unsigned last_served;
   size_t cap_flanks, cap_bases, cap_state, cap_cons, cap_bounds, cap_trim, cap_fam, cap_famctl;
   void *d_fam; RamxCtl *d_famctl;
   RamxCtl *h_ctl;
@@ -139,6 +141,7 @@
   CRCHK(hipMalloc((void **)&d->d_ctl, 2 * sizeof(RamxCtl)));
   CRCHK(hipMalloc((void **)&d->d_vote, PRK_NSETS * NSHARD * sizeof(PShard)));
   CRCHK(hipMalloc((void **)&d->d_err, 64));
+  CRCHK(hipMalloc((void **)&d->d_slots, PK_NSLOT * sizeof(PkSlot)));
 
   for (int i = 0; i < 2; i++) CRCHK(hipEventCreate(&d->ev_chk[i]));
   CRCHK(hipEventCreate(&d->ev_begin));
@@ -165,7 +168,7 @@
   (void)hipFree(d->d_pk_nstart); (void)hipFree(d->d_pk_nlen); (void)hipFree(d->d_flank_win);
   (void)hipFree(d->d_lib); (void)hipFree(d->d_flanks); (void)hipFree(d->d_bases); (void)hipFree(d->d_bounds);
   (void)hipFree(d->d_state[0]); if (d->d_state[1] != d->d_state[0]) (void)hipFree(d->d_state[1]); (void)hipFree(d->d_trim); (void)hipFree(d->d_sums);
-  (void)hipFree(d->d_ctl); (void)hipFree(d->d_cons); (void)hipFree(d->d_vote); (void)hipFree(d->d_err);
+  (void)hipFree(d->d_ctl); (void)hipFree(d->d_cons); (void)hipFree(d->d_vote); (void)hipFree(d->d_err); (void)hipFree(d->d_slots);
   if (d->h_ctl) (void)hipHostFree(d->h_ctl);
   if (d->h_stage) (void)hipHostFree(d->h_stage);
   if (d->hostbox_map)
@@ -788,6 +791,12 @@
       int cap = 0;
       if (ramx_pk_capacity(W, pk_block, &cap) == RAMX_OK && pk_blocks + 1 <= cap) ka.xblock = pk_blocks;
     }
+    ka.slots = d->d_slots; ka.served = d->d_err + 1; ka.svc = 0;
+    if (ka.nranks <= 1 && W <= 40 && pa.lean_p >= 0 && pa.leader_max > 0 && getenv("RAMX_NO_PK_SERVICE") == NULL)
+    {
+      int cap = 0;
+      if (ramx_pk_capacity(W, pk_block, &cap) == RAMX_OK && pk_blocks + 1 <= cap) ka.svc = 1;
+    }
     ka.Np = d->Np; ka.Nx = d->Nx; ka.L = L; ka.go = a.go; ka.ge = a.ge; ka.cap = a.cap; ka.minimp = a.minimp;
     ka.when_to_stop = a.when_to_stop; ka.nblocks = pk_blocks;
     memcpy(ka.tab, a.tab, sizeof(ka.tab));
@@ -816,6 +825,7 @@
         d->packed_kw = words_for(r1);
       }
       HIPCHK(hipMemsetAsync(d->d_vote, 0, PRK_NSETS * NSHARD * sizeof(PShard), d->stream));
+      if (ka.svc) HIPCHK(hipMemsetAsync(d->d_slots, 0, PK_NSLOT * sizeof(PkSlot), d->stream));
       ka.r0 = r; ka.Lseg = r1; ka.sums_in = sums_in;
       ka.sums_next = r1 < L ? sbuf[nextbuf] : NULL;
       if (r1 < L) HIPCHK(hipMemsetAsync(sbuf[nextbuf], 0, (size_t)NSHARD * 4 * sizeof(long long), d->stream));
@@ -1348,6 +1358,7 @@
 {
   if (!d || !d->ready) { ramx_set_error("ramx_dev_run_direction: begin_direction has not been called"); return RAMX_ERR_STATE; }
   HIPCHK(hipSetDevice(d->ordinal));
+  d->last_served = 0;
   const ramx_params &p = d->p;
   const int L = p.L;
   KArgs a;
@@ -1652,6 +1663,7 @@
       if ((drc = d2h_small(d, c0, d->d_ctl, sizeof(c0))) != RAMX_OK) return drc;
       if ((drc = d2h_small(d, &ew, d->d_err, sizeof(ew))) != RAMX_OK) return drc;
       errw = (unsigned)ew;
+      d->last_served = (unsigned)(ew >> 32);
     }
     rt_mark("after the launch: control blocks, error word");
     if (c0[0].pad != 0 || c0[1].pad != 0 || errw != 0)
@@ -1663,6 +1675,7 @@
       fprintf(stderr, "ramx: device-wide barrier of the persistent launch timed out (bounded spin); repeating the direction with "
                       "per-column launches\n");
       persistent = false;
+      d->last_served = 0;
       HIPCHK(hipMemsetAsync(d->d_sums, 0, 3 * NSHARD * 4 * sizeof(long long), d->stream));
       a.r = -1; a.S_in = d->d_state[0]; a.S_out = d->d_state[1]; a.ctl_in = d->d_ctl; a.ctl_out = d->d_ctl + 1;
       a.sums_in = slot(0); a.sums_out = slot(0); a.sums_zero = slot(1); a.nshards_in = NSHARD;
@@ -1807,6 +1820,12 @@
   return RAMX_OK;
 }
 
+extern "C" int ramx_dev_served_rows(ramx_dev *d)
+{
+  if (!d) { ramx_set_error("ramx_dev_served_rows: bad argument"); return RAMX_ERR_ARG; }
+  return d->last_served > 0x7fffffffu ? 0x7fffffff : (int)d->last_served;
+}
+
 extern "C" int ramx_dev_peek_state(ramx_dev *d, int32_t flank, int32_t *cells, int32_t *high, int32_t *pos)
 {
   if (!d || !d->ready || flank < 0 || flank >= d->Nx) { ramx_set_error("ramx_dev_peek_state: bad argument"); return RAMX_ERR_ARG; }
diff --git a/repeatafterme_amd/csrc/ramx_kernels_packed.h b/repeatafterme_amd/csrc/ramx_kernels_packed.h
--- a/repeatafterme_amd/csrc/ramx_kernels_packed.h
+++ b/repeatafterme_amd/csrc/ramx_kernels_packed.h
@@ -233,6 +233,220 @@
   const int stp = d2 >= a.when_to_stop ? 1 : 0;
   if (lane == 0) { st[0] = (int)mx; st[1] = (int)(mx >> 32); st[2] = mr; st[3] = ov; }
   return bw | (nm << 2) | (stp << 3) | (fl << 4);
+}
+
+#ifndef PK_ADOPT_RUN
+#define PK_ADOPT_RUN 64
+#endif
+#define PK_RELEASE_MARGIN 6
+
+__device__ __forceinline__ int pkb_scan_max64(int v)
+{
+#define PKB_SCAN_STEP(ctrl) asm("s_nop 1\n\tv_max_i32_dpp %0, %0, %0 " ctrl : "+v"(v))
+  PKB_SCAN_STEP("row_shr:1 row_mask:0xf bank_mask:0xf"); PKB_SCAN_STEP("row_shr:2 row_mask:0xf bank_mask:0xf");
+  PKB_SCAN_STEP("row_shr:4 row_mask:0xf bank_mask:0xf"); PKB_SCAN_STEP("row_shr:8 row_mask:0xf bank_mask:0xf");
+  PKB_SCAN_STEP("row_bcast:15 row_mask:0xa bank_mask:0xf"); PKB_SCAN_STEP("row_bcast:31 row_mask:0xc bank_mask:0xf");
+#undef PKB_SCAN_STEP
+  return v;
+}
+
+template <int W, int BLOCK>
+__device__ __forceinline__ void pkb_service(const PKArgs &a, const PkTabs &pt, long long (&tot)[2][4], int (&word)[2][2], int *st)
+{
+  constexpr int B = PkCfg<W>::B, NP = PkCfg<W>::NP;
+  const int lane = threadIdx.x & 63, wave = threadIdx.x >> 6;
+  const int shard = blockIdx.x % NSHARD;
+  const bool has_slot = wave < PK_NSLOT;
+  PkSlot *sl = a.slots + (has_slot ? wave : 0);
+  const int j0 = lane, j1 = lane + 64;
+  int state = 0;
+  int T = 0, T2 = 0, fn = 0, bdy = 0, high = 0, pos = 0, failed = 0;
+  int m0 = NEG, m1 = NEG, e0 = NEG, e1 = NEG;
+  int cls0 = 0, cls1 = 0;
+  unsigned rows = 0;
+  auto cls_of = [&](int rr, int j) __attribute__((always_inline)) -> int
+  {
+    const int g = rr + 8 + j;
+    return (int)((a.bases[(size_t)(g >> 3) * a.Np + fn] >> (4 * (g & 7))) & 15u);
+  };
+  __syncthreads();
+  for (int r = a.r0; r < a.Lseg; r++)
+  {
+    PShard *vb = a.vote;
+    asm volatile("" : "+s"(vb));
+    const int par = r & 1, npar = (r + 1) & 1;
+    const bool hand_over = r == a.Lseg - 1 && a.Lseg < a.L;
+    if (state == 2 && T2 != 0 && r == T2)
+    {
+      if (lane == 0)
+      {
+        __hip_atomic_store(&sl->answer, 0u, __ATOMIC_RELAXED, __HIP_MEMORY_SCOPE_AGENT);
+        __hip_atomic_store(&sl->ready, 0u, __ATOMIC_RELAXED, __HIP_MEMORY_SCOPE_AGENT);
+        __hip_atomic_store(&sl->release, 0u, __ATOMIC_RELAXED, __HIP_MEMORY_SCOPE_AGENT);
+        __hip_atomic_store(&sl->claim, 0u, __ATOMIC_RELEASE, __HIP_MEMORY_SCOPE_AGENT);
+      }
+      state = 0; T2 = 0;
+    }
+    if (has_slot && state == 0)
+    {
+      unsigned c = 0;
+      if (lane == 0) c = __hip_atomic_load(&sl->claim, __ATOMIC_RELAXED, __HIP_MEMORY_SCOPE_AGENT);
+      c = (unsigned)__builtin_amdgcn_readfirstlane((int)c);
+      if (c != 0)
+      {
+        fn = (int)c - 1; T = r + 3; state = 1;
+        const int2 bd = a.bounds[fn];
+        bdy = bd.x > bd.y ? -0x40000000 : bd.y;
+        if (lane == 0) __hip_atomic_store(&sl->answer, (unsigned)(T + 1), __ATOMIC_RELAXED, __HIP_MEMORY_SCOPE_AGENT);
+        __builtin_amdgcn_fence(__ATOMIC_RELEASE, "agent");
+      }
+    }
+    if (state == 1 && r == T)
+    {
+      unsigned spins = 0;
+      int ok = 0;
+      for (;;)
+      {
+        unsigned f = 0;
+        if (lane == 0) f = __hip_atomic_load(&sl->ready, __ATOMIC_RELAXED, __HIP_MEMORY_SCOPE_AGENT);
+        if (__builtin_amdgcn_readfirstlane((int)f) != 0) { ok = 1; break; }
+        if (++spins > PRK_SPIN_LIMIT || ((spins & 1023u) == 0 && __hip_atomic_load(a.err, __ATOMIC_RELAXED, __HIP_MEMORY_SCOPE_AGENT) != 0)) break;
+        __builtin_amdgcn_s_sleep(1);
+      }
+      __builtin_amdgcn_fence(__ATOMIC_ACQUIRE, "agent");
+      if (!ok)
+      {
+        if (lane == 0) __hip_atomic_fetch_max(a.err, 1u, __ATOMIC_RELAXED, __HIP_MEMORY_SCOPE_AGENT);
+        state = 3;
+      }
+      else
+      {
+        const int lbase = __hip_atomic_load(&sl->pbase, __ATOMIC_RELAXED, __HIP_MEMORY_SCOPE_AGENT);
+        high = __hip_atomic_load(&sl->high, __ATOMIC_RELAXED, __HIP_MEMORY_SCOPE_AGENT);
+        pos = __hip_atomic_load(&sl->pos, __ATOMIC_RELAXED, __HIP_MEMORY_SCOPE_AGENT);
+        const int jprev = bdy - (r - 1);
+        auto cell = [&](int j, int &m, int &e) __attribute__((always_inline))
+        {
+          m = NEG; e = NEG;
+          if (j < B && j <= jprev)
+          {
+            const int mw = __hip_atomic_load(&sl->row[j >> 1], __ATOMIC_RELAXED, __HIP_MEMORY_SCOPE_AGENT);
+            const int ew = __hip_atomic_load(&sl->row[NP + ((j + 1) >> 1)], __ATOMIC_RELAXED, __HIP_MEMORY_SCOPE_AGENT);
+            m = lbase + ((j & 1) ? (mw >> 16) : (int)(short)mw);
+            e = lbase + ((j & 1) ? (int)(short)ew : (ew >> 16));
+          }
+        };
+        cell(j0, m0, e0); cell(j1, m1, e1);
+        cls0 = j0 < B ? cls_of(r, j0) : 0; cls1 = j1 < B ? cls_of(r, j1) : 0;
+        state = 2;
+      }
+    }
+    state = __builtin_amdgcn_readfirstlane(state);
+    int ncls0 = 0, ncls1 = 0;
+    if (state == 2) { ncls0 = j0 < B ? cls_of(r + 1, j0) : 0; ncls1 = j1 < B ? cls_of(r + 1, j1) : 0; }
+
+    if (wave == 0)
+    {
+      long long v[4];
+      const int nv = a.nblocks + 1;
+      prk_wait_vote(a, vb, a.sums_in, r == a.r0 ? (a.r0 == 0 ? 1 : 2) : 0, r, lane, (nv - (lane & (NSHARD - 1)) + NSHARD - 1) / NSHARD, failed, v, false);
+      const int fl = __any(failed) ? 1 : 0;
+      const int dword = pkb_stop_rule(a, r, v, fl, st, lane);
+      if (lane == 0)
+      {
+        word[par][0] = dword;
+        if (fl) __hip_atomic_fetch_max(a.err, 1u, __ATOMIC_RELAXED, __HIP_MEMORY_SCOPE_AGENT);
+      }
+    }
+    __syncthreads();
+    const int dw = __builtin_amdgcn_readfirstlane(word[par][0]);
+    if (dw & 16) break;
+    const int bw = dw & 3;
+    const bool last_col = ((dw >> 3) & 1) || r == a.L - 1;
+
+    if (state == 2)
+    {
+      const int jhi = bdy - r;
+      const bool in0 = j0 < B && j0 <= jhi, in1 = j1 < B && j1 <= jhi;
+      const int sub0 = m0 + (int)(short)pt.tp[bw][cls0], sub1 = m1 + (int)(short)pt.tp[bw][cls1];
+      const int eup0 = __shfl_down(e0, 1, 64), eup1 = __shfl_down(e1, 1, 64), e1first = __builtin_amdgcn_readlane(e1, 0);
+      const int del0 = j0 == B - 1 ? NEG : (lane == 63 ? e1first : eup0);
+      const int del1 = (j1 >= B - 1 || lane == 63) ? NEG : eup1;
+      const int x0 = in0 ? imax(sub0 + a.go, del0) + a.ge - j0 * a.ge : NEG;
+      const int x1 = in1 ? imax(sub1 + a.go, del1) + a.ge - j1 * a.ge : NEG;
+      const int p0 = pkb_scan_max64(x0);
+      const int p1 = imax(pkb_scan_max64(x1), __builtin_amdgcn_readlane(p0, 63));
+      const int en0 = p0 + j0 * a.ge, en1 = p1 + j1 * a.ge;
+      const int edn0 = __shfl_up(en0, 1, 64), edn1 = __shfl_up(en1, 1, 64), en0last = __builtin_amdgcn_readlane(en0, 63);
+      const int ins0 = lane == 0 ? NEG : edn0, ins1 = lane == 0 ? en0last : edn1;
+      m0 = in0 ? imax3(sub0, del0, ins0) : NEG; e0 = in0 ? en0 : NEG;
+      m1 = in1 ? imax3(sub1, del1, ins1) : NEG; e1 = in1 ? en1 : NEG;
+      const int bf = wave_max_i32_dpp(imax(m0, m1));
+      const unsigned long long hit0 = __ballot(in0 && m0 == bf), hit1 = __ballot(in1 && m1 == bf);
+      const int jb = hit0 ? __builtin_ctzll(hit0) : (hit1 ? 64 + __builtin_ctzll(hit1) : 0);
+      const int bestF = jhi < 0 ? SENT : bf;
+      if (bestF > high) { high = bestF; pos = r + jb - W; }
+      const bool c0 = in0 && j0 + 1 <= jhi, c1 = in1 && j1 + 1 <= jhi;
+      int me = NEG;
+      if (in0 && j0 >= 1) me = e0;
+      if (in1) me = imax(me, e1);
+      const int mx = wave_max_i32_dpp(me);
+      const int capv = high + a.cap;
+      long long mine = 0;
+#pragma unroll
+      for (int c = 0; c < 4; c++)
+      {
+        const int t0 = c0 ? m0 + (int)(short)pt.tp[c][ncls0] : NEG, t1 = c1 ? m1 + (int)(short)pt.tp[c][ncls1] : NEG;
+        int b = imax(wave_max_i32_dpp(imax(t0, t1)), mx);
+        b = b < 0 ? 0 : b;
+        b = b >= capv ? b : capv;
+        if (lane == c) mine = b;
+      }
+      if (lane < 4 && !last_col) asm volatile("ds_add_u64 %0, %1" : : "v"(pkb_lds_off(&tot[npar][lane])), "v"(mine) : "memory");
+      if ((dw & 4) && lane == 0) a.trim[fn] = make_int2(high, pos);
+      cls0 = ncls0; cls1 = ncls1;
+      rows++;
+      if (T2 == 0 && !last_col)
+      {
+        const long long bl = bestF, capfl = capv > 0 ? capv : 0, P = a.lean_p;
+        if (bl + (2 + PK_RELEASE_MARGIN) * P <= capfl && bl + (1 + PK_RELEASE_MARGIN) * P <= (long long)high)
+        {
+          T2 = r + 4;
+          if (lane == 0)
+          {
+            __hip_atomic_store(&sl->rel_pos, pos, __ATOMIC_RELAXED, __HIP_MEMORY_SCOPE_AGENT);
+            __hip_atomic_store(&sl->release, (unsigned)(T2 + 1), __ATOMIC_RELEASE, __HIP_MEMORY_SCOPE_AGENT);
+          }
+          __builtin_amdgcn_fence(__ATOMIC_RELEASE, "agent");
+        }
+      }
+    }
+    if (last_col) break;
+    asm volatile("s_waitcnt lgkmcnt(0)\n\ts_barrier" ::: "memory");
+    if (wave == 0 && lane < 4)
+    {
+      long long t;
+      asm volatile("ds_read_b64 %0, %1\n\ts_waitcnt lgkmcnt(0)" : "=v"(t) : "v"(pkb_lds_off(&tot[npar][lane])) : "memory");
+      asm volatile("ds_write_b64 %0, %1" : : "v"(pkb_lds_off(&tot[npar][lane])), "v"(0LL) : "memory");
+      if (hand_over) __hip_atomic_fetch_add(&a.sums_next[shard * 4 + lane], t, __ATOMIC_RELAXED, __HIP_MEMORY_SCOPE_AGENT);
+      else
+      {
+        PShard *sh = vb + (size_t)((r + 1) & (PRK_NSETS - 1)) * NSHARD + shard;
+        __hip_atomic_fetch_add(&sh->word[lane], (unsigned long long)t + PRK_BIAS + PRK_TICKET, __ATOMIC_RELAXED, __HIP_MEMORY_SCOPE_AGENT);
+      }
+    }
+    if (hand_over) break;
+  }
+  if (has_slot && state >= 2)
+  {
+    if (lane == 0)
+    {
+      __hip_atomic_store(&sl->fin_high, high, __ATOMIC_RELAXED, __HIP_MEMORY_SCOPE_AGENT);
+      __hip_atomic_store(&sl->fin_pos, pos, __ATOMIC_RELAXED, __HIP_MEMORY_SCOPE_AGENT);
+      __hip_atomic_store(&sl->done, 1u, __ATOMIC_RELEASE, __HIP_MEMORY_SCOPE_AGENT);
+      if (rows) __hip_atomic_fetch_add(a.served, rows, __ATOMIC_RELAXED, __HIP_MEMORY_SCOPE_AGENT);
+    }
+  }
 }
 
 #ifdef RAMX_PRK_TIMING
@@ -301,6 +515,11 @@
   const bool skip = stopped || failed || a.r0 >= a.Lseg;
   if (threadIdx.x == 0) { sm.st[0] = (int)max_ext; sm.st[1] = (int)(max_ext >> 32); sm.st[2] = max_row; sm.st[3] = ovf; }
 
+  if (blockIdx.x == a.nblocks && a.svc)
+  {
+    if (!(stopped || failed || a.r0 >= a.Lseg)) pkb_service<W, BLOCK>(a, sm.pt, sm.tot[1], sm.word, sm.st);
+    return;
+  }
   if (blockIdx.x == a.nblocks)
   {
     if (wave != 0 || stopped || failed || a.r0 >= a.Lseg) return;
@@ -403,9 +622,13 @@
   unsigned long long tsum[6] = { 0, 0, 0, 0, 0, 0 }, tlast = wall_clock64();
 #endif
   int spec = 0, guess = 0;
+  int ad = 0;
+  unsigned relw = 0;
   for (int r = a.r0; r < a.Lseg; r++)
   {
     PKB_TICK(5);
+    const bool adopted = (ad >> 12) != 0 && ((ad & 0x80) != 0 || r >= (ad >> 12) - 1);
+    unsigned long long lead_last = 0;
     PShard *vb = a.vote;
     asm volatile("" : "+s"(vb));
     if (((r + 8) & 7) == 0 && r > a.r0)
@@ -430,7 +653,7 @@
         long long v[4];
         int lv = lane;
         asm volatile("" : "+v"(lv));
-        prk_wait_vote(a, vb, a.sums_in, r == a.r0 ? (a.r0 == 0 ? 1 : 2) : 0, r, lv, (a.nblocks - (lv & (NSHARD - 1)) + NSHARD - 1) / NSHARD, failed, v, blockIdx.x == a.xblock);
+        prk_wait_vote(a, vb, a.sums_in, r == a.r0 ? (a.r0 == 0 ? 1 : 2) : 0, r, lv, (a.nblocks + a.svc - (lv & (NSHARD - 1)) + NSHARD - 1) / NSHARD, failed, v, blockIdx.x == a.xblock);
         const int fl = __any(failed) ? 1 : 0;
         const int dword = pkb_stop_rule(a, r, v, fl, sm.st, lane);
         const int bw = dword & 3;
@@ -548,15 +771,16 @@
       unsigned long long leaders = 0;
       if (live && a.lean_p >= 0)
       {
-        const unsigned long long keep = __ballot((n < a.Nx) && !((prevBest + 2 * a.lean_p <= capfloor) && (prevBest + a.lean_p <= high)));
+        const unsigned long long keep = __ballot((n < a.Nx) && !adopted && !((prevBest + 2 * a.lean_p <= capfloor) && (prevBest + a.lean_p <= high)));
         if (keep == 0) { lean = true; early = true; }
         else if (__popcll(keep) <= a.leader_max) { lean = true; leaders = keep; }
       }
       if (!live) early = true;
+      lead_last = leaders;
       const bool send = pass_spec || !last_col;
       if (early && send)
       {
-        const long long t = wave_sum_nonneg31((live && n < a.Nx) ? capfloor : 0);
+        const long long t = wave_sum_nonneg31((live && n < a.Nx && !adopted) ? capfloor : 0);
         arrive(set, t, t, t, t);
       }
       PKB_TICK(3);
@@ -626,7 +850,7 @@
         }
         prevBest = bestF;
         if (bestF > high) { high = bestF; pos = r + jbest - W; }
-        if (n < a.Nx)
+        if (n < a.Nx && !adopted)
         {
           const int capv = high + a.cap;
 #pragma unroll
@@ -692,9 +916,9 @@
     }
     if (gave_up) break;
 #ifndef PKB_PROBE_NO_TRIM
-    if (new_max && live)
+    if (new_max && live && !adopted)
 #else
-    if (new_max && live && r < 0)
+    if (new_max && live && !adopted && r < 0)
 #endif
     {
       int nn = n;
@@ -702,6 +926,56 @@
       a.trim[nn] = make_int2(high, pos);
     }
     if (last_col || hand_over) break;
+    if (a.svc && (lead_last != 0 || __any(ad != 0)))
+    {
+      const bool isl = live && ((lead_last >> lane) & 1) != 0;
+      int run = ad & 0x7f;
+      run = isl ? (run < 127 ? run + 1 : 127) : 0;
+      ad = (ad & ~0x7f) | run;
+      const int myslot = (ad >> 8) & 15;
+      if (isl && run >= PK_ADOPT_RUN && myslot == 0)
+      {
+        constexpr int NSL = WPB < PK_NSLOT ? WPB : PK_NSLOT;
+        int got = 0;
+        for (int s_ = 0; s_ < NSL; s_++)
+        {
+          unsigned expect = 0;
+          if (__hip_atomic_compare_exchange_strong(&a.slots[s_].claim, &expect, (unsigned)(n + 1), __ATOMIC_ACQUIRE, __ATOMIC_RELAXED, __HIP_MEMORY_SCOPE_AGENT)) { got = s_ + 1; break; }
+        }
+        if (got) ad |= got << 8;
+        else ad &= ~0x7f;
+      }
+      else if (myslot >= 1 && myslot <= PK_NSLOT && (ad >> 12) == 0)
+      {
+        const unsigned ans = __hip_atomic_load(&a.slots[myslot - 1].answer, __ATOMIC_RELAXED, __HIP_MEMORY_SCOPE_AGENT);
+        if (ans != 0)
+        {
+          ad |= (int)ans << 12;
+          if (r + 2 > (int)ans) __hip_atomic_fetch_max(a.err, 1u, __ATOMIC_RELAXED, __HIP_MEMORY_SCOPE_AGENT);
+        }
+      }
+      if ((ad >> 12) != 0 && (ad & 0x80) == 0 && r >= (ad >> 12) - 1)
+      {
+        const unsigned rw = relw;
+        relw = __hip_atomic_load(&a.slots[myslot - 1].release, __ATOMIC_RELAXED, __HIP_MEMORY_SCOPE_AGENT);
+        if (rw != 0)
+        {
+          __builtin_amdgcn_fence(__ATOMIC_ACQUIRE, "agent");
+          pos = __hip_atomic_load(&a.slots[myslot - 1].rel_pos, __ATOMIC_RELAXED, __HIP_MEMORY_SCOPE_AGENT);
+          ad = (ad & 0xfff) | 0x80 | ((int)rw << 12);
+          if (r + 2 > (int)rw) __hip_atomic_fetch_max(a.err, 1u, __ATOMIC_RELAXED, __HIP_MEMORY_SCOPE_AGENT);
+        }
+      }
+      if ((ad & 0x80) != 0 && r == (ad >> 12) - 2) { ad = 0; relw = 0; }
+      if ((ad >> 12) != 0 && (ad & 0x80) == 0 && r == (ad >> 12) - 2)
+      {
+        PkSlot *sl = a.slots + (myslot - 1);
+        static_for([&](auto kc) __attribute__((always_inline)) { constexpr int k = decltype(kc)::value; sl->row[k] = R[k]; sl->row[NP + k] = E[k]; },
+                   std::make_integer_sequence<int, NP>{});
+        sl->pbase = pbase; sl->high = high; sl->pos = pos;
+        __hip_atomic_store(&sl->ready, 1u, __ATOMIC_RELEASE, __HIP_MEMORY_SCOPE_AGENT);
+      }
+    }
     if constexpr (SPEC)
     {
       if (confirmed_arrival)
@@ -724,6 +998,24 @@
   }
 #endif
 
+  if (a.svc && (ad >> 12) != 0 && ((ad & 0x80) != 0 || rows_done >= (ad >> 12)))
+  {
+    PkSlot *sl = a.slots + (((ad >> 8) & 15) - 1);
+    unsigned spins = 0;
+    bool ok = true;
+    while (__hip_atomic_load(&sl->done, __ATOMIC_RELAXED, __HIP_MEMORY_SCOPE_AGENT) == 0)
+    {
+      if (++spins > PRK_SPIN_LIMIT || ((spins & 1023u) == 0 && __hip_atomic_load(a.err, __ATOMIC_RELAXED, __HIP_MEMORY_SCOPE_AGENT) != 0)) { ok = false; break; }
+      __builtin_amdgcn_s_sleep(1);
+    }
+    __builtin_amdgcn_fence(__ATOMIC_ACQUIRE, "agent");
+    if (ok)
+    {
+      high = __hip_atomic_load(&sl->fin_high, __ATOMIC_RELAXED, __HIP_MEMORY_SCOPE_AGENT);
+      pos = __hip_atomic_load(&sl->fin_pos, __ATOMIC_RELAXED, __HIP_MEMORY_SCOPE_AGENT);
+    }
+    else __hip_atomic_fetch_max(a.err, 1u, __ATOMIC_RELAXED, __HIP_MEMORY_SCOPE_AGENT);
+  }
   if (live && rows_done > a.r0)
   {
     int bz = bdy;
@@ -755,7 +1047,8 @@
     RamxCtl o;
     o.max_ext = ((long long)sm.st[1] << 32) | (long long)(unsigned)sm.st[0]; o.max_row = sm.st[2]; o.stopped = stopped; o.rows_done = rows_done;
     o.overflow = sm.st[3];
-    o.besta = ((carried & 0xffff) + lean_rows) | ((((carried >> 16) & 0xffff) + wrong_rows) << 16);
+    const int nl = (carried & 0xffff) + lean_rows, nw = ((carried >> 16) & 0xffff) + wrong_rows;
+    o.besta = (nl > 0xffff ? 0xffff : nl) | ((nw > 0xffff ? 0xffff : nw) << 16);
     o.pad = failed;
     *a.ctl_out = o;
   }
diff --git a/repeatafterme_amd/csrc/ramx_packed.hip b/repeatafterme_amd/csrc/ramx_packed.hip
--- a/repeatafterme_amd/csrc/ramx_packed.hip
+++ b/repeatafterme_amd/csrc/ramx_packed.hip
@@ -89,7 +89,7 @@
 template <int W>
 static int pk_launch(hipStream_t st, int block, int blocks, const PKArgs &a)
 {
-  const int grid = blocks + (a.xblock != 0 ? 1 : 0);
+  const int grid = blocks + ((a.xblock != 0 || a.svc) ? 1 : 0);
   if (block == 256) hipLaunchKernelGGL((ramx_packed_kernel<W, 256>), dim3(grid), dim3(256), 0, st, a);
   else if (block == 320)
   {
diff --git a/repeatafterme_amd/csrc/ramx_pk_api.h b/repeatafterme_amd/csrc/ramx_pk_api.h
--- a/repeatafterme_amd/csrc/ramx_pk_api.h
+++ b/repeatafterme_amd/csrc/ramx_pk_api.h
@@ -6,6 +6,20 @@
 
 struct PShard;
 struct PeerBox;
+
+#define PK_NSLOT 8
+struct PkSlot
+{
+  unsigned claim;
+  unsigned answer;
+  unsigned ready;
+  unsigned done;
+  unsigned release;
+  int pbase, high, pos, fin_high, fin_pos;
+  int rel_pos;
+  int pad[5];
+  int row[112];
+};
 
 struct PKArgs
 {
@@ -34,6 +48,9 @@
   int rebase;
   int spec_on;
   int test_wrong_every;
+  PkSlot *slots;
+  int svc;
+  unsigned *served;
   unsigned long long *dbg;
 };
 
diff --git a/repeatafterme_amd/device.py b/repeatafterme_amd/device.py
--- a/repeatafterme_amd/device.py
+++ b/repeatafterme_amd/device.py
@@ -75,6 +75,9 @@
                    "ramx_dev_peek_state")
         return cells[:2 * B].reshape(B, 2).copy(), hi.value, po.value
 
+    def served_rows(self) -> int:
+        return _lib.check(self._L.ramx_dev_served_rows(self._h), "ramx_dev_served_rows")
+
     def unique_id(self) -> np.ndarray:
         uid = np.zeros(128, np.uint8)
         _lib.check(self._L.ramx_comm_unique_id(uid.ctypes.data), "ramx_comm_unique_id")
```

After: 17.80 billion (median of 4 runs). About the same (+0.3%).
